# StanfordASL/pmpc

Hardware: AMD Instinct MI355X
Metric: SCP iterations/sec (M particles x N horizon) (higher is better)
Workload: dtype f64; 1 GPU; quadrotor x12 u4 M=4096 N=50 Nc=1 box-u, full SCP iteration (on-device linearise + c_lqp_solve-equivalent + residual), BASELINE config D; timed window = SCP iterations 6..2477 from the cold start X_prev = x0, U_prev = U_ref (the active-set round count falls as the SCP loop converges, so the rate depends on the window); particles_per_gpu=4096, parallelism=particle-shard x1, scp_loop=library (pmpc_scp_loop_device), ipm_warm_start=True

## Files before the change

include/pmpc_abi.h:

```cpp
#ifndef PMPC_ABI_H
#define PMPC_ABI_H

#include <stddef.h>

#ifdef __cplusplus
extern "C" {
#endif


void c_lqp_solve(double *X_out, double *U_out, size_t xdim, size_t udim, size_t N, size_t M, long long Nc,
                 double *x0, double *f, double *fx, double *fu, double *X_prev, double *U_prev, double *Q,
                 double *R, double *X_ref, double *U_ref, double *lx, double *ux, double *lu, double *uu,
                 double reg_x, double reg_u, double *slew_reg, double *slew_reg0, double *slew_um1,
                 long long verbose);

void c_lcone_solve(double *X_out, double *U_out, size_t xdim, size_t udim, size_t N, size_t M, long long Nc,
                   double *x0, double *f, double *fx, double *fu, double *X_prev, double *U_prev, double *Q,
                   double *R, double *X_ref, double *U_ref, double *lx, double *ux, double *lu, double *uu,
                   double reg_x, double reg_u, double *slew_reg, double *slew_reg0, double *slew_um1,
                   long long verbose, double smooth_alpha, char *solver);

void pmpc_lqp_solve_host(double *X_out, double *U_out, size_t xdim, size_t udim, size_t N, size_t M, long long Nc,
                         double *x0, double *f, double *fx, double *fu, double *X_prev, double *U_prev, double *Q,
                         double *R, double *X_ref, double *U_ref, double *lx, double *ux, double *lu, double *uu,
                         double reg_x, double reg_u, double *slew_reg, double *slew_reg0, double *slew_um1,
                         long long verbose, unsigned rowmajor);
void pmpc_lcone_solve_host(double *X_out, double *U_out, size_t xdim, size_t udim, size_t N, size_t M, long long Nc,
                           double *x0, double *f, double *fx, double *fu, double *X_prev, double *U_prev, double *Q,
                           double *R, double *X_ref, double *U_ref, double *lx, double *ux, double *lu, double *uu,
                           double reg_x, double reg_u, double *slew_reg, double *slew_reg0, double *slew_um1,
                           long long verbose, double smooth_alpha, unsigned rowmajor, long long cone_k);
void pmpc_lcone_solve_host_ex(double *X_out, double *U_out, size_t xdim, size_t udim, size_t N, size_t M, long long Nc, double *x0, double *f,
                              double *fx, double *fu, double *X_prev, double *U_prev, double *Q, double *R, double *X_ref, double *U_ref, double *lx,
                              double *ux, double *lu, double *uu, double reg_x, double reg_u, double *slew_reg, double *slew_reg0, double *slew_um1,
                              long long verbose, double smooth_alpha, unsigned rowmajor, long long cone_k, int smooth_cstr, double smooth_beta);


#define PMPC_HAS_XBOUNDS 1u
#define PMPC_HAS_UBOUNDS 2u
#define PMPC_HAS_SLEW 4u
#define PMPC_HAS_SLEW0 8u
#define PMPC_FORCE_GENERIC 16u
#define PMPC_SYMMETRIC_COST 32u

#define PMPC_COLD_START 64u
#define PMPC_STATIC_CONS_BOUNDS 128u
#define PMPC_PREV_IS_LAST_SOLUTION 256u

#define PMPC_CONE_OBJECTIVE 1024u
#define PMPC_F32_MATRICES 512u

typedef struct pmpc_problem {
  size_t xdim, udim, N, M;
  long long Nc;
  unsigned flags;
  double reg_x, reg_u;
  const double *x0, *f, *fx, *fu, *X_prev, *U_prev, *Q, *R, *X_ref, *U_ref;
  const double *lx, *ux, *lu, *uu;
  const double *slew_reg, *slew_reg0, *slew_um1;
  double *X_out, *U_out;
  const double *weights;
  double barrier_mu;
  size_t soc_q;
  const double *soc_W, *soc_w0, *soc_v;
  double soc_v0;
  const double *soc_u_interior;
  size_t cone_count;
  const int *cone_sizes;
  const double *cone_A, *cone_c;
  int cone_per_stage;
  long long cone_k;
  int smooth_cstr;
  double smooth_beta;
} pmpc_problem;

typedef struct pmpc_info {
  int status;
  int ipm_iters;
  int structured_solves;
  int fast_path;
  double mu;
  double slack_res;
  double max_violation;
  int outer_solves;
  int active_set_rounds;
} pmpc_info;

typedef struct pmpc_ctx pmpc_ctx;

int pmpc_create(pmpc_ctx **ctx, int device);
void pmpc_destroy(pmpc_ctx *ctx);
int pmpc_set_option(pmpc_ctx *ctx, const char *key, double value);
int pmpc_get_option(pmpc_ctx *ctx, const char *key, double *value);
void *pmpc_stream(pmpc_ctx *ctx);
void pmpc_sync(pmpc_ctx *ctx);

int pmpc_lqp_solve_device(pmpc_ctx *ctx, const pmpc_problem *prob, pmpc_info *info, int verbose);

int pmpc_lcone_solve_device(pmpc_ctx *ctx, const pmpc_problem *prob, double smooth_alpha, pmpc_info *info, int verbose);

int pmpc_lsoc_solve_device(pmpc_ctx *ctx, const pmpc_problem *prob, pmpc_info *info, int verbose);

int pmpc_particle_costs_device(pmpc_ctx *ctx, const pmpc_problem *prob, const double *X, const double *U, double *J_out);

int pmpc_comm_unique_id(void *unique_id_128);
int pmpc_comm_init(pmpc_ctx *ctx, int rank, int world, const void *unique_id_128);
int pmpc_comm_init_mock(pmpc_ctx *ctx, int rank, int world, int group);
int pmpc_comm_rank(pmpc_ctx *ctx);
int pmpc_comm_world(pmpc_ctx *ctx);

int pmpc_linearize_device(pmpc_ctx *ctx, int model, size_t N, size_t M, const double *x0, const double *X_prev,
                          const double *U_prev, const double *params, double *f, double *fx, double *fu);

int pmpc_linearize_device_f32(pmpc_ctx *ctx, int model, size_t N, size_t M, const double *x0, const double *X_prev,
                              const double *U_prev, const double *params, double *f, float *fx, float *fu);

int pmpc_rollout_device(pmpc_ctx *ctx, int model, size_t N, size_t M, const double *x0, const double *U, const double *params, double *X);

int pmpc_shift_plan_device(pmpc_ctx *ctx, int model, size_t N, size_t M, size_t s, const double *X, const double *U,
                           const double *params, const double *U_tail, double *X_new, double *U_new, double *um1_new);

int pmpc_shift_active_set_device(pmpc_ctx *ctx, size_t N, size_t M, size_t udim, long long Nc, size_t s, const double *U,
                                 const double *U_tail, const int *act, const double *lo, const double *hi, double *U_new, int *act_new);

int pmpc_warm_shift_device(pmpc_ctx *ctx, size_t N, size_t M, size_t udim, long long Nc, size_t s, const double *U, const double *U_tail,
                           const double *lo, const double *hi, double *U_new, int *shifted);

int pmpc_warm_set_read_device(pmpc_ctx *ctx, int *act_out, size_t n);

int pmpc_linearize_compact_device(pmpc_ctx *ctx, int model, size_t N, size_t M, const double *x0, const double *X_prev,
                                  const double *U_prev, const double *params, double *f, double *jc);
int pmpc_expand_jac_device(pmpc_ctx *ctx, int model, size_t N, size_t M, const double *jc, double *fx, double *fu, int orient);
long long pmpc_jac_compact_doubles(int model, size_t N, size_t M);
int pmpc_jac_live_mask(int model, unsigned char *fx_mask, unsigned char *fu_mask);

int pmpc_as_sweep_variant(int sweep, int xdim, int udim, int M, int Nc, unsigned flags, const int *knobs, int *out);

int pmpc_as_sweep_launches(int sweep, unsigned long long *out, int n, int reset);
void pmpc_as_sweep_knobs(int *out);

int pmpc_scp_residual_device(pmpc_ctx *ctx, size_t xdim, size_t udim, size_t N, size_t M, const double *X, const double *X_prev,
                             const double *U, const double *U_prev, double *out);

int pmpc_scp_loop_device(pmpc_ctx *ctx, int model, const double *params, const pmpc_problem *p, double *f2, double *fx2, double *fu2,
                         int steps, int first_cold, double *res, pmpc_info *infos, int *last_in_out);

int pmpc_ref_shift_device(pmpc_ctx *ctx, size_t dim, size_t rows, const double *A, const double *c, const double *ref, double *out);
long long pmpc_ref_shift_bad_pivots(pmpc_ctx *ctx, int reset);

typedef struct pmpc_scp_cost {
  int kind;
  int K, pos_dim;
  int pos_idx[3];
  int per_stage;
  const double *centres, *sigma, *w;
} pmpc_scp_cost;
size_t pmpc_abi_scp_cost_size(void);

int pmpc_obstacle_cost_grad_device(pmpc_ctx *ctx, const pmpc_scp_cost *cost, size_t xdim, size_t N, size_t M, const double *X_prev,
                                   double *cx);
int pmpc_obstacle_ref_shift_device(pmpc_ctx *ctx, const pmpc_scp_cost *cost, size_t xdim, size_t N, size_t M, const double *X_prev,
                                   const double *Q, const double *X_ref, double *out);

int pmpc_scp_loop_device_cost(pmpc_ctx *ctx, int model, const double *params, const pmpc_problem *p, double *f2, double *fx2,
                              double *fu2, int steps, int first_cold, double *res, pmpc_info *infos, int *last_in_out,
                              const pmpc_scp_cost *cost);

typedef struct pmpc_scp_cstr {
  int kind;
  int K, pos_dim;
  int pos_idx[3];
  long long centre_stride_particle, centre_stride_stage;
  const double *centres, *radius;
} pmpc_scp_cstr;
size_t pmpc_abi_scp_cstr_size(void);

int pmpc_keepout_augment_device(pmpc_ctx *ctx, const pmpc_scp_cstr *cstr, size_t xdim, size_t udim, size_t N, size_t M,
                                const double *X_prev, const double *f, const double *fx, const double *fu, const double *X_ref,
                                double *f_aug, double *fx_aug, double *fu_aug, double *X_prev_aug, double *X_ref_aug, double *xu_aug);

int pmpc_keepout_strip_residual_device(pmpc_ctx *ctx, size_t xdim, int K, size_t udim, size_t N, size_t M, const double *X_aug, double *X,
                                       const double *X_prev, const double *U, const double *U_prev, double *out);

typedef struct pmpc_scp_aug {
  const double *Q, *x0, *lx;
  double *f[2], *fx[2], *fu[2], *X_prev[2], *X_ref[2], *xu[2];
  double *X_out;
} pmpc_scp_aug;
size_t pmpc_abi_scp_aug_size(void);

int pmpc_scp_loop_device_cstr(pmpc_ctx *ctx, int model, const double *params, const pmpc_problem *p, double *f2, double *fx2,
                              double *fu2, int steps, int first_cold, double *res, pmpc_info *infos, int *last_in_out,
                              const pmpc_scp_cost *cost, const pmpc_scp_cstr *cstr, const pmpc_scp_aug *aug);
void pmpc_scp_loop_follow_ups(unsigned long long *out2, int reset);

void pmpc_profile_enable(pmpc_ctx *ctx, int level);
void pmpc_profile_read(pmpc_ctx *ctx, double *ms4, long long *n4);
void pmpc_profile_read_partial(pmpc_ctx *ctx, double *ms, long long *n);
void pmpc_profile_read_all(pmpc_ctx *ctx, double *ms, long long *launches, int count);

void pmpc_restart_stats(pmpc_ctx *ctx, unsigned long long *out4, int reset);

const char *pmpc_version(void);
void pmpc_abi_struct_sizes(size_t *problem, size_t *info);

#ifdef __cplusplus
}
#endif
#endif
```

pmpc_amd/_lib.py:

```python
from __future__ import annotations

import ctypes
import os
from pathlib import Path

import numpy as np

_HERE = Path(__file__).resolve().parent
LIB_PATH = Path(os.environ["PMPC_HIP_LIB"]) if os.environ.get("PMPC_HIP_LIB") else _HERE / "libpmpc_hip.so"
_lib = None

c_dp = ctypes.POINTER(ctypes.c_double)

HAS_XBOUNDS, HAS_UBOUNDS, HAS_SLEW, HAS_SLEW0, FORCE_GENERIC, SYMMETRIC_COST, COLD_START, STATIC_CONS_BOUNDS, PREV_IS_LAST_SOLUTION, F32_MATRICES, CONE_OBJECTIVE = 1, 2, 4, 8, 16, 32, 64, 128, 256, 512, 1024

ABI_SYMBOLS = [
    "c_lqp_solve", "c_lcone_solve", "pmpc_lqp_solve_host", "pmpc_lcone_solve_host", "pmpc_create", "pmpc_destroy", "pmpc_stream", "pmpc_sync", "pmpc_lqp_solve_device",
    "pmpc_comm_unique_id", "pmpc_comm_init", "pmpc_comm_rank", "pmpc_comm_world", "pmpc_linearize_device",
    "pmpc_profile_enable", "pmpc_profile_read", "pmpc_version", "pmpc_lcone_solve_device", "pmpc_particle_costs_device", "pmpc_lsoc_solve_device", "pmpc_comm_init_mock",
    "pmpc_scp_residual_device", "pmpc_profile_read_partial", "pmpc_profile_read_all", "pmpc_scp_loop_device", "pmpc_linearize_device_f32",
    "pmpc_set_option", "pmpc_get_option", "pmpc_abi_struct_sizes", "pmpc_lcone_solve_host_ex", "pmpc_restart_stats",
    "pmpc_linearize_compact_device", "pmpc_expand_jac_device", "pmpc_jac_compact_doubles", "pmpc_jac_live_mask",
    "pmpc_as_sweep_variant", "pmpc_as_sweep_launches", "pmpc_as_sweep_knobs",
    "pmpc_ref_shift_device", "pmpc_ref_shift_bad_pivots", "pmpc_obstacle_cost_grad_device", "pmpc_obstacle_ref_shift_device",
    "pmpc_scp_loop_device_cost", "pmpc_abi_scp_cost_size",
    "pmpc_rollout_device", "pmpc_shift_plan_device",
    "pmpc_keepout_augment_device", "pmpc_abi_scp_cstr_size",
    "pmpc_keepout_strip_residual_device", "pmpc_scp_loop_device_cstr", "pmpc_abi_scp_aug_size", "pmpc_scp_loop_follow_ups",
    "pmpc_shift_active_set_device", "pmpc_warm_shift_device", "pmpc_warm_set_read_device",
]


class PmpcProblem(ctypes.Structure):
    _fields_ = (
        [(k, ctypes.c_size_t) for k in ("xdim", "udim", "N", "M")]
        + [("Nc", ctypes.c_longlong), ("flags", ctypes.c_uint), ("reg_x", ctypes.c_double), ("reg_u", ctypes.c_double)]
        + [(k, ctypes.c_void_p) for k in ("x0", "f", "fx", "fu", "X_prev", "U_prev", "Q", "R", "X_ref", "U_ref",
                                          "lx", "ux", "lu", "uu", "slew_reg", "slew_reg0", "slew_um1", "X_out", "U_out", "weights")]
        + [("barrier_mu", ctypes.c_double), ("soc_q", ctypes.c_size_t), ("soc_W", ctypes.c_void_p), ("soc_w0", ctypes.c_void_p),
           ("soc_v", ctypes.c_void_p), ("soc_v0", ctypes.c_double), ("soc_u_interior", ctypes.c_void_p),
           ("cone_count", ctypes.c_size_t), ("cone_sizes", ctypes.POINTER(ctypes.c_int)), ("cone_A", ctypes.c_void_p), ("cone_c", ctypes.c_void_p),
           ("cone_per_stage", ctypes.c_int), ("cone_k", ctypes.c_longlong), ("smooth_cstr", ctypes.c_int), ("smooth_beta", ctypes.c_double)]
    )


class PmpcInfo(ctypes.Structure):
    _fields_ = [("status", ctypes.c_int), ("ipm_iters", ctypes.c_int), ("structured_solves", ctypes.c_int),
                ("fast_path", ctypes.c_int), ("mu", ctypes.c_double), ("slack_res", ctypes.c_double),
                ("max_violation", ctypes.c_double), ("outer_solves", ctypes.c_int), ("active_set_rounds", ctypes.c_int)]


class PmpcScpCost(ctypes.Structure):
    _fields_ = [("kind", ctypes.c_int), ("K", ctypes.c_int), ("pos_dim", ctypes.c_int), ("pos_idx", ctypes.c_int * 3), ("per_stage", ctypes.c_int),
                ("centres", ctypes.c_void_p), ("sigma", ctypes.c_void_p), ("w", ctypes.c_void_p)]


class PmpcScpCstr(ctypes.Structure):
    _fields_ = [("kind", ctypes.c_int), ("K", ctypes.c_int), ("pos_dim", ctypes.c_int), ("pos_idx", ctypes.c_int * 3),
                ("centre_stride_particle", ctypes.c_longlong), ("centre_stride_stage", ctypes.c_longlong),
                ("centres", ctypes.c_void_p), ("radius", ctypes.c_void_p)]


class PmpcScpAug(ctypes.Structure):
    _fields_ = ([(k, ctypes.c_void_p) for k in ("Q", "x0", "lx")] + [(k, ctypes.c_void_p * 2) for k in ("f", "fx", "fu", "X_prev", "X_ref", "xu")]
                + [("X_out", ctypes.c_void_p)])


def load():
    global _lib
    if _lib is not None:
        return _lib
    if not LIB_PATH.exists():
        raise ImportError(
            f"{LIB_PATH} is missing: build the HIP extension first (python -c 'import __graft_entry__ as g; g.build()' "
            "or make -C pmpc_amd/csrc). pmpc_amd has no CPU fallback.")
    lib = ctypes.CDLL(str(LIB_PATH), mode=ctypes.RTLD_GLOBAL)
    sz, ll, dbl, vp = ctypes.c_size_t, ctypes.c_longlong, ctypes.c_double, ctypes.c_void_p
    common = [c_dp, c_dp, sz, sz, sz, sz, ll] + [c_dp] * 14 + [dbl, dbl] + [c_dp] * 3 + [ll]
    lib.c_lqp_solve.argtypes = common
    lib.c_lqp_solve.restype = None
    lib.c_lcone_solve.argtypes = common + [dbl, ctypes.c_char_p]
    lib.c_lcone_solve.restype = None
    lib.pmpc_lqp_solve_host.argtypes = common + [ctypes.c_uint]
    lib.pmpc_lqp_solve_host.restype = None
    lib.pmpc_lcone_solve_host.argtypes = common + [dbl, ctypes.c_uint, ll]
    lib.pmpc_lcone_solve_host.restype = None
    lib.pmpc_lcone_solve_host_ex.argtypes = common + [dbl, ctypes.c_uint, ll, ctypes.c_int, dbl]
    lib.pmpc_lcone_solve_host_ex.restype = None
    lib.pmpc_create.argtypes = [ctypes.POINTER(vp), ctypes.c_int]
    lib.pmpc_create.restype = ctypes.c_int
    lib.pmpc_destroy.argtypes = [vp]
    lib.pmpc_destroy.restype = None
    lib.pmpc_set_option.argtypes = [vp, ctypes.c_char_p, ctypes.c_double]
    lib.pmpc_set_option.restype = ctypes.c_int
    lib.pmpc_get_option.argtypes = [vp, ctypes.c_char_p, c_dp]
    lib.pmpc_get_option.restype = ctypes.c_int
    lib.pmpc_stream.argtypes = [vp]
    lib.pmpc_stream.restype = vp
    lib.pmpc_sync.argtypes = [vp]
    lib.pmpc_sync.restype = None
    lib.pmpc_lqp_solve_device.argtypes = [vp, ctypes.POINTER(PmpcProblem), ctypes.POINTER(PmpcInfo), ctypes.c_int]
    lib.pmpc_lqp_solve_device.restype = ctypes.c_int
    lib.pmpc_lcone_solve_device.argtypes = [vp, ctypes.POINTER(PmpcProblem), dbl, ctypes.POINTER(PmpcInfo), ctypes.c_int]
    lib.pmpc_lcone_solve_device.restype = ctypes.c_int
    lib.pmpc_lsoc_solve_device.argtypes = [vp, ctypes.POINTER(PmpcProblem), ctypes.POINTER(PmpcInfo), ctypes.c_int]
    lib.pmpc_lsoc_solve_device.restype = ctypes.c_int
    lib.pmpc_particle_costs_device.argtypes = [vp, ctypes.POINTER(PmpcProblem), vp, vp, vp]
    lib.pmpc_particle_costs_device.restype = ctypes.c_int
    lib.pmpc_comm_unique_id.argtypes = [vp]
    lib.pmpc_comm_unique_id.restype = ctypes.c_int
    lib.pmpc_comm_init.argtypes = [vp, ctypes.c_int, ctypes.c_int, vp]
    lib.pmpc_comm_init.restype = ctypes.c_int
# ... 7 lines not shown
    lib.pmpc_linearize_device.restype = ctypes.c_int
    lib.pmpc_linearize_device_f32.argtypes = [vp, ctypes.c_int, sz, sz] + [vp] * 7
    lib.pmpc_linearize_device_f32.restype = ctypes.c_int
    if hasattr(lib, "pmpc_jac_live_mask"):
        lib.pmpc_linearize_compact_device.argtypes = [vp, ctypes.c_int, sz, sz] + [vp] * 6
        lib.pmpc_linearize_compact_device.restype = ctypes.c_int
        lib.pmpc_expand_jac_device.argtypes = [vp, ctypes.c_int, sz, sz, vp, vp, vp, ctypes.c_int]
        lib.pmpc_expand_jac_device.restype = ctypes.c_int
        lib.pmpc_jac_compact_doubles.argtypes = [ctypes.c_int, sz, sz]
        lib.pmpc_jac_compact_doubles.restype = ctypes.c_longlong
        lib.pmpc_jac_live_mask.argtypes = [ctypes.c_int, vp, vp]
        lib.pmpc_jac_live_mask.restype = ctypes.c_int
    if hasattr(lib, "pmpc_as_sweep_variant"):
        lib.pmpc_as_sweep_variant.argtypes = [ctypes.c_int] * 5 + [ctypes.c_uint, ctypes.POINTER(ctypes.c_int), ctypes.POINTER(ctypes.c_int)]
        lib.pmpc_as_sweep_variant.restype = ctypes.c_int
    if hasattr(lib, "pmpc_as_sweep_launches"):
        lib.pmpc_as_sweep_launches.argtypes = [ctypes.c_int, ctypes.POINTER(ctypes.c_ulonglong), ctypes.c_int, ctypes.c_int]
        lib.pmpc_as_sweep_launches.restype = ctypes.c_int
        lib.pmpc_as_sweep_knobs.argtypes = [ctypes.POINTER(ctypes.c_int)]
        lib.pmpc_as_sweep_knobs.restype = None
    lib.pmpc_scp_residual_device.argtypes = [vp, sz, sz, sz, sz] + [vp] * 5
    lib.pmpc_scp_residual_device.restype = ctypes.c_int
    lib.pmpc_profile_enable.argtypes = [vp, ctypes.c_int]
    lib.pmpc_profile_enable.restype = None
    lib.pmpc_profile_read.argtypes = [vp, c_dp, ctypes.POINTER(ctypes.c_longlong)]
    lib.pmpc_profile_read.restype = None
    lib.pmpc_profile_read_partial.argtypes = [vp, ctypes.POINTER(ctypes.c_double), ctypes.POINTER(ctypes.c_longlong)]
    lib.pmpc_profile_read_partial.restype = None
    lib.pmpc_restart_stats.argtypes = [vp, ctypes.POINTER(ctypes.c_ulonglong), ctypes.c_int]
    lib.pmpc_restart_stats.restype = None
    lib.pmpc_profile_read_all.argtypes = [vp, c_dp, ctypes.POINTER(ctypes.c_longlong), ctypes.c_int]
    lib.pmpc_profile_read_all.restype = None
    lib.pmpc_scp_loop_device.argtypes = [vp, ctypes.c_int, vp, ctypes.POINTER(PmpcProblem), vp, vp, vp, ctypes.c_int, ctypes.c_int, vp,
                                         ctypes.POINTER(PmpcInfo), ctypes.POINTER(ctypes.c_int)]
    lib.pmpc_scp_loop_device.restype = ctypes.c_int
    if hasattr(lib, "pmpc_scp_loop_device_cost"):
        lib.pmpc_ref_shift_device.argtypes = [vp, sz, sz, vp, vp, vp, vp]
        lib.pmpc_ref_shift_device.restype = ctypes.c_int
        lib.pmpc_ref_shift_bad_pivots.argtypes = [vp, ctypes.c_int]
        lib.pmpc_ref_shift_bad_pivots.restype = ctypes.c_longlong
        lib.pmpc_obstacle_cost_grad_device.argtypes = [vp, ctypes.POINTER(PmpcScpCost), sz, sz, sz, vp, vp]
        lib.pmpc_obstacle_cost_grad_device.restype = ctypes.c_int
        lib.pmpc_obstacle_ref_shift_device.argtypes = [vp, ctypes.POINTER(PmpcScpCost), sz, sz, sz, vp, vp, vp, vp]
        lib.pmpc_obstacle_ref_shift_device.restype = ctypes.c_int
        lib.pmpc_scp_loop_device_cost.argtypes = lib.pmpc_scp_loop_device.argtypes + [ctypes.POINTER(PmpcScpCost)]
        lib.pmpc_scp_loop_device_cost.restype = ctypes.c_int
        lib.pmpc_abi_scp_cost_size.argtypes = []
        lib.pmpc_abi_scp_cost_size.restype = sz
        if lib.pmpc_abi_scp_cost_size() != ctypes.sizeof(PmpcScpCost):
            raise ImportError(f"{LIB_PATH} and pmpc_amd/_lib.py disagree on pmpc_scp_cost: library {lib.pmpc_abi_scp_cost_size()} bytes, "
                              f"binding {ctypes.sizeof(PmpcScpCost)}: rebuild the library")
    if hasattr(lib, "pmpc_shift_plan_device"):
        lib.pmpc_rollout_device.argtypes = [vp, ctypes.c_int, sz, sz, vp, vp, vp, vp]
        lib.pmpc_rollout_device.restype = ctypes.c_int
        lib.pmpc_shift_plan_device.argtypes = [vp, ctypes.c_int, sz, sz, sz] + [vp] * 7
        lib.pmpc_shift_plan_device.restype = ctypes.c_int
    if hasattr(lib, "pmpc_keepout_augment_device"):
        lib.pmpc_keepout_augment_device.argtypes = [vp, ctypes.POINTER(PmpcScpCstr), sz, sz, sz, sz] + [vp] * 11
        lib.pmpc_keepout_augment_device.restype = ctypes.c_int
        lib.pmpc_abi_scp_cstr_size.argtypes = []
        lib.pmpc_abi_scp_cstr_size.restype = sz
        if lib.pmpc_abi_scp_cstr_size() != ctypes.sizeof(PmpcScpCstr):
            raise ImportError(f"{LIB_PATH} and pmpc_amd/_lib.py disagree on pmpc_scp_cstr: library {lib.pmpc_abi_scp_cstr_size()} bytes, "
                              f"binding {ctypes.sizeof(PmpcScpCstr)}: rebuild the library")
    if hasattr(lib, "pmpc_scp_loop_device_cstr"):
        lib.pmpc_keepout_strip_residual_device.argtypes = [vp, sz, ctypes.c_int, sz, sz, sz] + [vp] * 6
        lib.pmpc_keepout_strip_residual_device.restype = ctypes.c_int
        lib.pmpc_scp_loop_device_cstr.argtypes = lib.pmpc_scp_loop_device_cost.argtypes + [ctypes.POINTER(PmpcScpCstr), ctypes.POINTER(PmpcScpAug)]
        lib.pmpc_scp_loop_device_cstr.restype = ctypes.c_int
        lib.pmpc_scp_loop_follow_ups.argtypes = [ctypes.POINTER(ctypes.c_ulonglong), ctypes.c_int]
        lib.pmpc_scp_loop_follow_ups.restype = None
        lib.pmpc_abi_scp_aug_size.argtypes = []
        lib.pmpc_abi_scp_aug_size.restype = sz
        if lib.pmpc_abi_scp_aug_size() != ctypes.sizeof(PmpcScpAug):
            raise ImportError(f"{LIB_PATH} and pmpc_amd/_lib.py disagree on pmpc_scp_aug: library {lib.pmpc_abi_scp_aug_size()} bytes, "
                              f"binding {ctypes.sizeof(PmpcScpAug)}: rebuild the library")
    if hasattr(lib, "pmpc_warm_shift_device"):
        lib.pmpc_shift_active_set_device.argtypes = [vp, sz, sz, sz, ll, sz] + [vp] * 7
        lib.pmpc_shift_active_set_device.restype = ctypes.c_int
        lib.pmpc_warm_shift_device.argtypes = [vp, sz, sz, sz, ll, sz] + [vp] * 5 + [ctypes.POINTER(ctypes.c_int)]
        lib.pmpc_warm_shift_device.restype = ctypes.c_int
        lib.pmpc_warm_set_read_device.argtypes = [vp, vp, sz]
        lib.pmpc_warm_set_read_device.restype = ctypes.c_int
    lib.pmpc_version.argtypes = []
    lib.pmpc_version.restype = ctypes.c_char_p
    if not hasattr(lib, "pmpc_abi_struct_sizes"):
        raise ImportError(f"{LIB_PATH} predates this binding (no pmpc_abi_struct_sizes): rebuild it (make -C pmpc_amd/csrc)")
    lib.pmpc_abi_struct_sizes.argtypes = [ctypes.POINTER(sz), ctypes.POINTER(sz)]
    lib.pmpc_abi_struct_sizes.restype = None
    sp, si = sz(0), sz(0)
    lib.pmpc_abi_struct_sizes(ctypes.byref(sp), ctypes.byref(si))
    if (sp.value, si.value) != (ctypes.sizeof(PmpcProblem), ctypes.sizeof(PmpcInfo)):
        raise ImportError(f"{LIB_PATH} ({lib.pmpc_version().decode()}) and pmpc_amd/_lib.py disagree on the ABI structs: library "
                          f"{sp.value}/{si.value} bytes, binding {ctypes.sizeof(PmpcProblem)}/{ctypes.sizeof(PmpcInfo)}: rebuild the library")
    _lib = lib
    return lib


def jac_live_mask(model: int, x: int, u: int):
    lib = load()
    mx, mu = np.zeros(x * x, dtype=np.uint8), np.zeros(x * u, dtype=np.uint8)
    got = lib.pmpc_jac_live_mask(int(model), mx.ctypes.data, mu.ctypes.data)
    if got < 0:
        raise ValueError(f"model {model} is not a built-in model")
    if got != 100 * x + u:
        raise ValueError(f"model {model}: compact records are for dims {got // 100} x {got % 100}, not {x} x {u}")
    return mx.reshape(x, x).T.astype(bool), mu.reshape(u, x).T.astype(bool)


AS_SWEEP_FLAGS = ("defect", "as_settled_in", "mat32", "cone_H", "xb_D", "as_uraw", "as_T")


def as_sweep_variant(sweep: str, x: int, u: int, M: int, Nc: int, flags: int, knobs=None):
    lib = load()
    out = (ctypes.c_int * 8)()
    kn = (ctypes.c_int * 3)(*knobs) if knobs is not None else None
    got = lib.pmpc_as_sweep_variant({"bwd": 0, "fwd": 1}[sweep], x, u, M, Nc, flags, kn, out)
    if got < 0:
        raise ValueError(f"({x}, {u}) is not a compiled pair of the active-set sweeps")
    return tuple(out[:5]), bool(got), tuple(bool(v) for v in out[5:8])


def as_sweep_code(sweep: str, variant) -> int:
    a, b, c, d, e = (int(v) for v in variant)
    if sweep == "bwd":
        return a + 3 * (b + 2 * (c + 2 * (d + 3 * e)))
    return a + 2 * b + 4 * c + 8 * d + 16 * e


def as_sweep_launches(sweep: str, reset: bool = False):
    lib = load()
    sw = {"bwd": 0, "fwd": 1}[sweep]
    n = lib.pmpc_as_sweep_launches(sw, None, 0, 0)
    out = (ctypes.c_ulonglong * n)()
    lib.pmpc_as_sweep_launches(sw, out, n, int(reset))
    return [int(v) for v in out]


def scp_loop_follow_ups(reset: bool = False):
    out = (ctypes.c_ulonglong * 2)()
    load().pmpc_scp_loop_follow_ups(out, int(reset))
    return int(out[0]), int(out[1])


def as_sweep_knobs():
    out = (ctypes.c_int * 3)()
    load().pmpc_as_sweep_knobs(out)
    return tuple(out)


def dptr(a: np.ndarray):
    assert a.dtype == np.float64 and a.flags["C_CONTIGUOUS"]
    return a.ctypes.data_as(c_dp)
```

pmpc_amd/csrc/kernels_as.hip:

```cpp
#include <atomic>
#include <type_traits>

#include "fast_common.h"
#include "as_ctl_dev.h"
#include "as_variant.h"
#include "../../include/pmpc_abi.h"
#include "jac_compact.h"

#ifdef PMPC_STAGE_TIMELINE
#define PMPC_TL_STAMPS 10
__device__ unsigned long long pmpc_tl[3][128][PMPC_TL_STAMPS];
#define TL_DECL(kind) unsigned long long tl_[PMPC_TL_STAMPS] = {}; const int tl_kind = (kind); const bool tl_on = blockIdx.x == gridDim.x / 2
#define TL(k) do { __builtin_amdgcn_sched_barrier(0); tl_[k] = __builtin_amdgcn_s_memtime(); __builtin_amdgcn_sched_barrier(0); } while (0)
#define TL_FLUSH(j) do { if (tl_on && threadIdx.x == 0 && (j) < 128) { for (int k_ = 0; k_ < PMPC_TL_STAMPS; k_++) pmpc_tl[tl_kind][j][k_] = tl_[k_]; } } while (0)
#else
#define TL_DECL(kind)
#define TL(k)
#define TL_FLUSH(j)
#endif

#ifndef PMPC_AS_LEAN_WAVES
#define PMPC_AS_LEAN_WAVES 4
#endif
#ifndef PMPC_AS_DEEP_WAVES
// ... 5 lines not shown

namespace {

template <int XD, int UD, int MODE, bool SKIP, bool DEFECT, int EX = 0, class MT = double>
__global__ void __launch_bounds__(64, MODE == 2 ? 2 : (MODE == 1 ? PMPC_AS_DEEP_WAVES : PMPC_AS_LEAN_WAVES)) k_bwd_as(LQArgs a) {
  constexpr bool CONE = EX == 1, XBOX = EX == 2;
  typedef Lane<XD, UD> LT;
  constexpr int KS = LT::KS, XP = LT::XP;
  constexpr bool PADX = (XD != XP);
  constexpr long long D8 = sizeof(double);
  constexpr bool DEEP = MODE != 0, SCHOL = !DEEP;
  constexpr long long MB = sizeof(MT);
  if (a.done && *a.done) return;
  const int lane = threadIdx.x;
  const int N = a.N, Nc = a.Nc, i = a.as_perm ? __builtin_amdgcn_readfirstlane(a.as_perm[blockIdx.x]) : (int)blockIdx.x;
  if (SKIP && a.as_settled_in[i]) {
    const int nc = Nc * UD;
    if (lane < nc) {
      const double *H = a.Hc_part + (size_t)i * nc * nc;
      double acc = 0.0;
      for (int cc = 0; cc < nc; cc++) acc = fma(H[(lane < cc ? lane : cc) + nc * (lane < cc ? cc : lane)], a.as_delta[cc], acc);
      a.gc_part[(size_t)i * nc + lane] += acc;
    }
    return;
  }
  const LT L(lane);
  const int g = L.g, c = L.c;
  const size_t pbase = (size_t)i * N;
  const bool own0 = (i == 0 && a.owner);
  const bool gu = g < UD;
  const double *Z = a.zeros;
  const double pwt = a.pw ? a.pw[i] : 1.0;
  const double regx = pwt * a.reg_x, regu = pwt * a.reg_u;
  const double *Xb = DEFECT ? a.X_prev : a.Xb, *Ub = DEFECT ? a.U_prev : a.Ub;
  constexpr int CKS = 64 * KS + 32;
  int jtop = N - 1, ck_k = 0;
  if (SKIP && a.as_ck) {
    const int jh = a.as_jhi[i];
    const int lo = jh > Nc ? jh : (Nc > 1 ? Nc : 1);
    const int k = lo <= PMPC_AS_CK_FIRST ? 0 : 32 - __builtin_clz((unsigned)(lo - 1) >> PMPC_AS_CK_LOG);
    if (k < a.ck_slots) { ck_k = __builtin_amdgcn_readfirstlane(k + 1); jtop = PMPC_AS_CK_FIRST << (ck_k - 1); }
    if (lane == 0 && a.ck_stat) {
      atomicAdd(a.ck_stat + (ck_k ? 0 : 2), 1ull);
      atomicAdd(a.ck_stat + (ck_k ? 1 : 3), (unsigned long long)(jtop + 1));
    }
  }
  const double *ck_ = a.as_ck ? ubase(a.as_ck, (long long)i * a.ck_slots * (long long)(CKS * sizeof(double))) : nullptr;

  const bool fF = L.cxv || L.cu;
  const MT *pF = L.cxv ? (const MT *)a.fx + (pbase + jtop) * (XD * XD) + XD * L.oc + L.row0
                       : (L.cu ? (const MT *)a.fu + (pbase + jtop) * (XD * UD) + XD * L.cb + L.row0 : (const MT *)Z);
  int sF = fF ? -(int)MB * (L.cxv ? XD * XD : XD * UD) : 0;
  typedef typename jacc::SpecFor<XD, UD>::list JSpecs;
  if constexpr (JSpecs::COUNT > 0 && std::is_same<MT, double>::value) {
    if (a.jac_compact) {
      const jacc::LaneSel js = jacc::select(JSpecs{}, a.jac_compact, lane);
      const int m = js.bwd;
      if (m != jacc::NONE) {
        pF = m >= 0 ? (const MT *)a.fx + (pbase + jtop) * js.rec + m : (const MT *)a.fx + (size_t)a.M * N * js.rec + (size_t)i * js.pool + (-1 - m);
        sF = m >= 0 ? -(int)MB * js.rec : 0;
      }
    }
  }
  const unsigned lQ = (unsigned)((L.cxv ? XD * L.oc + L.row0 : 0) * MB);
  const double pwt_x = L.cxv ? pwt : 0.0;
  const bool fR = L.cu && gu;
  const unsigned lR = (unsigned)((fR ? g + UD * L.cb : 0) * MB), lRd = (unsigned)((fR ? g + UD * L.cb : 0) * D8);
  const unsigned lxr = (unsigned)(L.row0 * D8), lxc = (unsigned)((L.cxv ? L.oc : 0) * D8);
  const unsigned lug = (unsigned)((gu ? g : 0) * D8);
  const double regx_c = L.cxv ? regx : 0.0;
  const bool umask = L.cu && g == L.cb;
  const double umask_d = umask ? 1.0 : 0.0;
  const bool diag_x = L.cxv && ((c & 3) == g);
  bool dmask[KS];
#pragma unroll
  for (int r = 0; r < KS; r++) dmask[r] = diag_x && (c >> 2) == r;
  const long long px = (long long)(pbase * XD) * D8, pu = (long long)(pbase * UD) * D8;
  const double *Xb_ = ubase(Xb, px), *Xr_ = ubase(a.X_ref, px), *Xp_ = ubase(a.X_prev, px), *f_ = ubase(a.f, px);
  const double *kff_ = ubase(a.kff, pu);
  const void *Q_ = ubase_v(a.Q, (long long)(pbase * (XD * XD)) * MB), *R_ = ubase_v(a.R, (long long)(pbase * (UD * UD)) * MB);
  const void *K_ = ubase_v(a.K, (long long)(pbase * 64) * MB);
  auto xoff = [&](int jj) { return (long long)(jj * (int)(XD * D8)); };
  auto uoff = [&](int jj) { return (long long)(jj * (int)(UD * D8)); };
  auto ld_Q = [&](int jj, double *dst) {
    const void *q = ubase_v(Q_, (long long)(jj * (int)(XD * XD * MB)));
#pragma unroll
    for (int r = 0; r < KS; r++) {
      const bool rv = !PADX || (L.row0 + r < XD);
      const double v = ldom<MT>(q, rv ? lQ + r * (unsigned)MB : 0u);
      dst[r] = rv ? v : 0.0;
    }
  };
  auto ld_xm = [&](int jj, double *dst) {
    const double *xb = ubase(Xb_, xoff(jj)), *xr = ubase(Xr_, xoff(jj));
#pragma unroll
    for (int r = 0; r < KS; r++) {
      const bool rv = !PADX || (L.row0 + r < XD);
      const unsigned o = rv ? lxr + r * 8u : 0u;
      const double v = pwt * (ldo(xb, o) - ldo(xr, o));
      dst[r] = rv ? v : 0.0;
    }
  };
  auto ld_gx = [&](int jj) -> double {
    if (DEFECT) return 0.0;
    return regx_c * (ldo(ubase(Xb_, xoff(jj)), lxc) - ldo(ubase(Xp_, xoff(jj)), lxc));
  };
  const char *pC = (const char *)Z;
  int sC = 0;
  if (gu && c == XP) { pC = (const char *)(Ub + (pbase + jtop) * UD + g); sC = -UD * (int)D8; }
  else if (gu && c == XP + 1) { pC = (const char *)(a.U_ref + (pbase + jtop) * UD + g); sC = -UD * (int)D8; }
  else if (gu && c == XP + 2) { pC = (const char *)(a.as_act + (pbase + jtop) * UD + g); sC = -UD * (int)sizeof(int); }
  else if (CONE && gu && c == XP + 3) { pC = (const char *)(a.cone_g + (pbase + jtop) * UD + g); sC = -UD * (int)D8; }
  else if (!DEFECT && g < 2 && 15 - XP - c >= 0 && 15 - XP - c < UD) {
    pC = (const char *)((g == 0 ? Ub : a.U_prev) + (pbase + jtop) * UD + (15 - XP - c));
    sC = -UD * (int)D8;
  }
  const double regu_s = (L.cu && g < 2) ? (g == 0 ? regu : -regu) : 0.0;
  auto ld_R = [&](int jj) -> double {
    const double v = ldom<MT>(ubase_v(R_, (long long)(jj * (int)(UD * UD * MB))), lR);
    return fR ? v : 0.0;
  };
  const double *CH_ = CONE ? ubase(a.cone_H, (long long)(pbase * (UD * UD)) * D8) : Z;
  auto ld_CH = [&](int jj) -> double {
    const double v = ldo(ubase(CH_, (long long)(jj * (int)(UD * UD * D8))), lRd);
    return fR ? v : 0.0;
  };
  const bool frec = (L.cxv || L.cu) && gu;
  const unsigned lrec = (unsigned)(lane * MB);
  auto st_rec = [&](int jj, double v) {
    gstom<MT>(ubase_v(K_, (long long)(jj * (int)(64 * MB))), lrec, v);
  };

  struct PipeCone { double ch; };
  struct PipeXbox { double xd, xg; };
  struct PipeNone {};
  struct Pipe : std::conditional_t<CONE, PipeCone, std::conditional_t<XBOX, PipeXbox, PipeNone>> { double F[KS], R, ctl, f, Q[KS], xb, xr, xp; };
  const double *XD_ = XBOX ? ubase(a.xb_D, px) : Z, *XG_ = XBOX ? ubase(a.xb_g, px) : Z;
  int jF = jtop;
  auto fetch_early = [&](int jj, Pipe &q) {
    if (jj < jF) { pF = (const MT *)((const char *)pF + sF); pC += sC; jF = jj; }
#pragma unroll
    for (int r = 0; r < KS; r++) q.F[r] = (!PADX || L.row0 + r < XD || (const void *)pF == (const void *)Z) ? gldm<MT>(pF + r) : 0.0;
    q.R = ld_R(jj);
    q.ctl = gld(pC);
    if (DEFECT) q.f = ldo(ubase(f_, xoff(jj)), lxc);
    if constexpr (CONE) q.ch = ld_CH(jj);
  };
  auto fetch_late = [&](int jj, int jbelow, Pipe &q) {
    ld_Q(jbelow, q.Q);
    q.xb = ldo(ubase(Xb_, xoff(jbelow)), lxc);
    q.xr = ldo(ubase(Xr_, xoff(jbelow)), lxc);
    if (!DEFECT) q.xp = ldo(ubase(Xp_, xoff(jbelow)), lxc);
    if constexpr (XBOX) {
      q.xd = ldo(ubase(XD_, xoff(jbelow)), lxc);
      q.xg = ldo(ubase(XG_, xoff(jbelow)), lxc);
    }
  };

  double S[KS], s_row[KS], s_col;
  bool bad = false;
  TL_DECL(SKIP ? 1 : 0);
  if (SKIP && ck_k > 0) {
    const double *ck = ubase(ck_, (long long)(ck_k - 1) * (long long)(CKS * D8));
#pragma unroll
    for (int r = 0; r < KS; r++) S[r] = ldo(ck, (unsigned)((lane + 64 * r) * D8));
    const double s_ck = ldo(ck, (unsigned)(64 * KS * D8) + lxc), x_ck = ldo(ck, (unsigned)((64 * KS + 16) * D8) + lxc);
    const double dx_col = L.cxv ? ldo(ubase(Xb_, xoff(jtop)), lxc) - x_ck : 0.0;
    double dx_row[KS], part = 0.0;
    col_to_row<KS>(dx_col, g, dx_row);
#pragma unroll
    for (int r = 0; r < KS; r++) part = fma(S[r], dx_row[r], part);
    part = grp_allsum(part);
    s_col = L.cxv ? s_ck + part : 0.0;
    col_to_row<KS>(s_col, g, s_row);
  } else
  {
    double Q0[KS], xm0[KS], part = 0.0;
    ld_Q(N - 1, Q0);
    ld_xm(N - 1, xm0);
#pragma unroll
    for (int r = 0; r < KS; r++) {
      part = fma(Q0[r], xm0[r], part);
      S[r] = fma(pwt_x, Q0[r], dmask[r] ? regx : 0.0);
    }
    part = grp_allsum(part);
    if constexpr (XBOX) {
      const double d0 = ldo(ubase(XD_, xoff(N - 1)), lxc);
      part += ldo(ubase(XG_, xoff(N - 1)), lxc);
#pragma unroll
      for (int r = 0; r < KS; r++) S[r] += dmask[r] ? d0 : 0.0;
    }
    s_col = L.cxv ? part + ld_gx(N - 1) : 0.0;
    col_to_row<KS>(s_col, g, s_row);
  }
  double xb_carry = DEFECT ? ldo(ubase(Xb_, xoff(N - 1)), lxc) : 0.0;

  auto stage = [&](auto main_tag, const int j, const Pipe &cur, Pipe &nxt) {
    constexpr bool MAIN = decltype(main_tag)::value;
    TL(0);
    if (MAIN && ck_ && (j & (j - 1)) == 0 && j >= PMPC_AS_CK_FIRST) {
      const double *ck = ubase(ck_, (long long)(__builtin_ctz((unsigned)j) - PMPC_AS_CK_LOG) * (long long)(CKS * D8));
#pragma unroll
      for (int r = 0; r < KS; r++) gsto(ck, (unsigned)((lane + 64 * r) * D8), S[r]);
      const double xj = DEFECT ? xb_carry : ldo(ubase(Xb_, xoff(j)), lxc);
      if (g == 0 && L.cxv) {
        gsto(ck, (unsigned)(64 * KS * D8) + lxc, s_col);
        gsto(ck, (unsigned)((64 * KS + 16) * D8) + lxc, xj);
      }
    }
    const bool cons = MAIN ? false : j < Nc;
    const bool below = MAIN ? true : j > 0;
    double Fr[KS], Qc[KS], xm_row[KS], gx_c, Du_c;
#pragma unroll
    for (int r = 0; r < KS; r++) Fr[r] = (!MAIN && j == 0 && L.cxv) ? 0.0 : cur.F[r];
    const double Rc = cur.R;
    const double um_g = pwt * (dpp_d<0x00>(cur.ctl) - dpp_d<0x55>(cur.ctl));
    const int act_g = __builtin_amdgcn_mov_dpp(__double2loint(cur.ctl), 0xAA, 0xF, 0xF, true);
    Du_c = (umask && act_g) ? a.as_big : 0.0;
    const double gu_c0 = DEFECT ? 0.0 : regu_s * dpp_d<0x140>(cur.ctl);
    const bool cone_here = CONE && (MAIN || !cons || own0);
    double gu_c = gu_c0;
    if constexpr (CONE) gu_c = fma(dpp_d<0xFF>(cur.ctl), cone_here ? umask_d : 0.0, gu_c0);
    double Hcone = 0.0;
    if constexpr (CONE) Hcone = cone_here ? cur.ch : 0.0;
    const double df_c = (DEFECT && L.cxv) ? cur.f - xb_carry : 0.0;
    if (DEFECT) xb_carry = cur.xb;
    gx_c = DEFECT ? 0.0 : regx_c * (cur.xb - cur.xp);
    if constexpr (XBOX) gx_c += cur.xg;
    col_to_row<KS>(pwt_x * (cur.xb - cur.xr), g, xm_row);
#pragma unroll
    for (int r = 0; r < KS; r++) Qc[r] = cur.Q[r];
    auto late_pf = [&]() { if (below) fetch_late(j - 1, j >= 2 ? j - 2 : 0, nxt); };
    TL(1);
    if (MODE == 1) late_pf();
// ... 119 lines not shown
      stage(std::true_type{}, j - 2, P2, P2);
      __builtin_amdgcn_sched_barrier(0);
    }
    for (; j >= 0; j--) {
      fetch(j - 2, P2);
      if (j >= jmin) stage(std::true_type{}, j, P0, P0);
      else stage(std::false_type{}, j, P0, P0);
      P0 = P1;
      P1 = P2;
    }
  } else {
    Pipe A, B;
    fetch_early(jtop, A);
    fetch_late(jtop, jtop >= 1 ? jtop - 1 : 0, A);
    for (; j >= jmin; j--) {
      stage(std::true_type{}, j, A, B);
      A = B;
    }
    if (j >= jmin) {
      stage(std::true_type{}, j, A, B);
      A = B;
      j--;
    }
    for (; j >= 0; j--) {
      stage(std::false_type{}, j, A, B);
      A = B;
    }
  }
  if (bad && lane == 0) *a.fail = 2;
}

template <int XD, int UD, bool DEFECT, bool PF2, bool CONE = false, class MT = double, bool SENS = false>
__global__ void __launch_bounds__(64, 4) k_fwd_as(LQArgs a) {
  typedef Lane<XD, UD> LT;
  constexpr int KS = LT::KS;
  constexpr bool PADX = (XD != LT::XP);
  constexpr long long D8 = sizeof(double);
  if (a.done && *a.done) return;
  const int lane = threadIdx.x;
  const LT L(lane);
  const int N = a.N, Nc = a.Nc, i = a.as_perm ? __builtin_amdgcn_readfirstlane(a.as_perm[blockIdx.x]) : (int)blockIdx.x, g = L.g, c = L.c;
  const size_t pbase = (size_t)i * N;
  const bool gu = g < UD;
  const double *Z = a.zeros;
  constexpr int MB = (int)sizeof(MT);
  const char *pA = (const char *)Z, *pB = (const char *)Z;
  int sAr = 0, sAj = 0, sBj = 0;
  if (L.cxv) {
    pA = (const char *)((const MT *)a.fx + pbase * (XD * XD) + (size_t)XD * (KS * g) + L.oc);
    sAr = XD * MB; sAj = XD * XD * MB;
    if (gu) { pB = (const char *)((const MT *)a.fu + pbase * (XD * UD) + (size_t)XD * g + L.oc); sBj = XD * UD * MB; }
  } else if (L.cu) {
    pA = (const char *)((const MT *)a.K + pbase * 64 + 16 * L.cb + g);
    sAr = 4 * MB; sAj = 64 * MB;
  }
  typedef typename jacc::SpecFor<XD, UD>::list JSpecs;
  if constexpr (JSpecs::COUNT > 0 && std::is_same<MT, double>::value) {
    if (a.jac_compact && L.cxv) {
      const jacc::LaneSel js = jacc::select(JSpecs{}, a.jac_compact, lane);
      const double *rec = a.fx + pbase * js.rec, *pool = a.fx + (size_t)a.M * N * js.rec + (size_t)i * js.pool;
      const int mA = js.fwdA, mB = js.fwdB;
      pA = (const char *)(mA >= 0 ? rec + mA : pool + (-1 - mA));
      sAr = MB; sAj = mA >= 0 ? js.rec * MB : 0;
      if (gu) { pB = (const char *)(mB >= 0 ? rec + mB : pool + (-1 - mB)); sBj = mB >= 0 ? js.rec * MB : 0; }
    }
  }
  bool vA[KS];
#pragma unroll
  for (int r = 0; r < KS; r++) vA[r] = !L.cxv || !PADX || (KS * g + r < XD);
  const double *Xb = DEFECT ? a.X_prev : a.Xb, *Ub = DEFECT ? a.U_prev : a.Ub;
  const double pwi = a.pw ? a.pw[i] : 1.0;
  const double tol_l = (a.as_ctl ? a.as_ctl->tol_l : a.as_tol_l) * pwi;
  const unsigned lug = (unsigned)((gu ? g : 0) * D8);
  const bool own_x = c < KS && (!PADX || L.row0 + c < XD);
  const unsigned lx1 = own_x ? (unsigned)((L.row0 + c) * D8) : 0u;
  const long long px = (long long)(pbase * XD) * D8, pu = (long long)(pbase * UD) * D8;
  const double *Xb_ = ubase(Xb, px), *f_ = ubase(a.f, px), *Xo_ = ubase(a.Xo, px);
  const double *act_ = ubase((const double *)a.as_act, pu >> 1);
  const double *T_ = SENS ? ubase(a.as_T, (long long)(pbase * 64) * D8) : Z;
  const unsigned lT = (unsigned)((((c - 4) & 3) * 16 + 4 * g) * D8);
  auto xoff = [&](int jj) { return (long long)(jj * (int)(XD * D8)); };
  auto uoff = [&](int jj) { return (long long)(jj * (int)(UD * D8)); };
  const char *pG = (const char *)Z;
  int sG = 0;
  if (gu && c < 4) {
    const double *arr = c == 0 ? Ub : (c == 1 ? a.kff : (c == 2 ? a.as_lo : a.as_hi));
    pG = (const char *)(arr + pbase * UD + g);
    sG = UD * (int)D8;
  } else if (gu && c == 7) {
    pG = (const char *)(a.as_act + pbase * UD + g);
    sG = UD * (int)sizeof(int);
  }
  char *pS = (char *)((c == 1 ? a.kff : ((CONE && c == 2) ? a.as_uraw : a.Uo)) + pbase * UD + (gu ? g : 0));
  const bool st_lane = gu && c < (CONE ? 3 : 2);
  const bool store_u = (c == 0) && gu;
  struct Pipe { double T[KS + 1], grp, xb, f; };
  int jF = 0;
  auto fetch = [&](int jj, Pipe &q) {
    if (jj > jF) { pA += sAj; pB += sBj; pG += sG; jF = jj; }
#pragma unroll
    for (int r = 0; r < KS; r++) {
      const double t = gldm<MT>(pA + (vA[r] ? r * sAr : 0));
      q.T[r] = vA[r] ? t : 0.0;
    }
    q.T[KS] = gldm<MT>(pB);
    q.grp = gld(pG);
    q.xb = ldo(ubase(Xb_, xoff(jj)), lx1);
    if (DEFECT) q.f = ldo(ubase(f_, xoff(jj)), lx1);
  };

  double V[KS];
#pragma unroll
  for (int r = 0; r < KS; r++) V[r] = 0.0;
  int nrel = 0, nadd = 0, nbad = 0;
  int jh = -1;
  double vworst = 0.0;
  double dcap = 0.0;
  const bool elem = SENS && !DEFECT && a.as_settled_in && a.as_settled_in[i];
  TL_DECL(2);
  double dcons = 0.0;
  bool frozen = false;
  if (a.cons_G) {
    constexpr int nH = UD * UD, E = nH + UD;
    double a0 = 0.0, a1 = 0.0, a2 = 0.0, a3 = 0.0;
    if (lane < E) {
      const double *src = lane < nH ? a.cons_tH + lane : a.cons_tg + (lane - nH);
      const int stride = lane < nH ? nH : UD;
      int k = 0;
      for (; k + 3 < a.cons_G; k += 4) {
        a0 += src[(size_t)k * stride];
        a1 += src[(size_t)(k + 1) * stride];
        a2 += src[(size_t)(k + 2) * stride];
        a3 += src[(size_t)(k + 3) * stride];
      }
      for (; k < a.cons_G; k++) a0 += src[(size_t)k * stride];
    }
    const double acc = (a0 + a1) + (a2 + a3);
    double Lm[UD][UD], y[UD];
    bool cbad = false;
#pragma unroll
    for (int q = 0; q < UD; q++) {
      double d = readlane_d(acc, q + UD * q);
#pragma unroll
      for (int k = 0; k < q; k++) d -= Lm[q][k] * Lm[q][k];
      cbad |= !(d > 0.0);
      d = sqrt(cbad ? 1.0 : d);
      Lm[q][q] = d;
#pragma unroll
      for (int p = q + 1; p < UD; p++) {
        double v = readlane_d(acc, q + UD * p);
#pragma unroll
        for (int k = 0; k < q; k++) v -= Lm[p][k] * Lm[q][k];
        Lm[p][q] = v / d;
      }
    }
#pragma unroll
    for (int p = 0; p < UD; p++) {
      double v = -readlane_d(acc, nH + p);
#pragma unroll
      for (int k = 0; k < p; k++) v -= Lm[p][k] * y[k];
      y[p] = v / Lm[p][p];
    }
#pragma unroll
    for (int p = UD - 1; p >= 0; p--) {
      double v = y[p];
#pragma unroll
      for (int k = p + 1; k < UD; k++) v -= Lm[k][p] * y[k];
      y[p] = v / Lm[p][p];
    }
    if (CONE && a.as_freeze_tol > 0.0) {
      const int *act0 = a.as_act + pbase * UD;
      const double *ub0 = Ub + pbase * UD;
      double ym = 0.0;
      bool asks_release = false;
#pragma unroll
      for (int p = 0; p < UD; p++) {
        if (act0[p] == 0) ym = fmax(ym, fabs(y[p]) / fmax(1.0, fabs(ub0[p])));
        else asks_release |= (act0[p] == 1 ? -a.as_big * y[p] : a.as_big * y[p]) < -tol_l;
      }
      frozen = ym <= a.as_freeze_tol && !asks_release;
      if (frozen) {
#pragma unroll
// ... 56 lines not shown
    nrel += (cnt_here && release) ? 1 : 0;
    nadd += (cnt_here && (vlo || vhi)) ? 1 : 0;
    jh = (cnt_here && (release || vlo || vhi)) ? j : jh;
    {
      const double pv = (vlo ? loc - zt : (vhi ? zt - hic : 0.0)) * __builtin_amdgcn_rcp(fmax(1.0, fabs(vlo ? loc : hic)));
      const double dv = release ? -lam * inv_dual : 0.0;
      vworst = fmax(vworst, cnt_here ? fmax(pv, dv) : 0.0);
    }
    TL(3);
    const double du_q = dpp_d<0x00>(dug);
    if (SENS && !MAIN && j < Nc) dcap = dug;
    const double knew = actc ? -draw : 0.0;
    if (MAIN || j >= Nc) {
      const double k1 = dpp_d<0x00>(knew);
      const double z1 = CONE ? dpp_d<0x00>(zt) : 0.0;
      if (st_lane) gst(pS, (c == 0) ? unew : ((CONE && c == 2) ? z1 : k1));
    } else {
      const double z1 = CONE ? dpp_d<0x00>(zt) : 0.0;
      if (store_u || (CONE && gu && c == 2)) gst(pS, (c == 0) ? unew : z1);
      if (store_u && i == 0) a.as_delta[j * UD + g] = dug;
    }
    pS += UD * (int)D8;
    if (store_u) gsto_i(ubase(act_, uoff(j) >> 1), lug >> 1, anew);
    TL(4);
    D[KS] = 0.0;
    double bop = (c < 4 && gu) ? du_q : 0.0;
    if (SENS) {
      const bool sc = c >= 4 && c < 4 + UD && gu;
      const double bs = (!MAIN && j < Nc) ? ((g == c - 4) ? 1.0 : 0.0) : -raw;
      bop = sc ? bs : bop;
    }
    D = mfma(cur.T[KS], bop, D);
    if (SENS) {
      if (c >= 4 && c < 4 + UD) {
        typedef double v2dd __attribute__((ext_vector_type(2)));
        const v2dd lo2 = {D[0], KS > 1 ? D[KS > 1 ? 1 : 0] : 0.0}, hi2 = {KS > 2 ? D[KS > 2 ? 2 : 0] : 0.0, gu ? bop : 0.0};
        __attribute__((address_space(1))) char *t = (__attribute__((address_space(1))) char *)(unsigned long long)ubase(T_, (long long)(j * (int)(64 * D8))) + lT;
        *(v2dd __attribute__((address_space(1))) *)t = lo2;
        *(v2dd __attribute__((address_space(1))) *)(t + 16) = hi2;
      }
    }
    if (DEFECT) {
      const double dfo = own_x ? cur.f - cur.xb : 0.0;
      D[0] += dpp_d<0x00>(dfo);
      if (KS > 1) D[1] += dpp_d<0x55>(dfo);
      if (KS > 2) D[2] += dpp_d<0xAA>(dfo);
    }
    if (own_x) {
      double mine = D[0];
#pragma unroll
      for (int r = 1; r < KS; r++) mine = (c == r) ? D[r] : mine;
      gsto(ubase(Xo_, xoff(j)), lx1, cur.xb + mine);
    }
#pragma unroll
    for (int r = 0; r < KS; r++) V[r] = (c < (SENS ? 4 + UD : 4)) ? D[r] : 0.0;
    TL(5);
    TL_FLUSH(j);
  };

  int nrel_e = 0, nadd_e = 0, nbad_e = 0, jh_e = -1;
  auto settled_update = [&](int j0) {
    double dl[UD];
#pragma unroll
    for (int k = 0; k < UD; k++) dl[k] = readlane_d(dcap, 16 * k);
    const int s16 = lane & 15, q4 = lane >> 4, gs = s16 >> 2, rs = s16 & 3;
    const bool is_x = rs < KS && KS * gs + rs < XD, is_u = rs == 3 && gs < UD;
    const size_t xo = (size_t)(is_x ? KS * gs + rs : 0), uo = (size_t)(is_u ? gs : 0);
    constexpr int SB = 4;
    for (int j4 = j0; j4 < N; j4 += 4 * SB) {
      double dv[SB], xv[SB], ub[SB], kf[SB], lo[SB], hi[SB];
      int act[SB];
#pragma unroll
      for (int q = 0; q < SB; q++) {
        const int jj = j4 + 4 * q + q4, jc = jj < N ? jj : N - 1;
        const double *t = a.as_T + (pbase + jc) * 64 + s16;
        double acc = 0.0;
#pragma unroll
        for (int k = 0; k < UD; k++) acc = fma(gld(t + 16 * k), dl[k], acc);
        dv[q] = acc;
        xv[q] = is_x ? gld(Xb + (pbase + jc) * XD + xo) : 0.0;
        const size_t e = (pbase + jc) * UD + uo;
        ub[q] = is_u ? gld(Ub + e) : 0.0;
        kf[q] = is_u ? gld(a.kff + e) : 0.0;
        lo[q] = is_u ? gld(a.as_lo + e) : 0.0;
        hi[q] = is_u ? gld(a.as_hi + e) : 0.0;
        act[q] = is_u ? a.as_act[e] : 0;
      }
#pragma unroll
      for (int q = 0; q < SB; q++) {
        const int jj = j4 + 4 * q + q4;
        const bool live = jj < N;
        if (is_x && live) gst(a.Xo + (pbase + jj) * XD + xo, xv[q] + dv[q]);
        if (is_u && live) {
          const size_t e = (pbase + jj) * UD + uo;
          if (act[q] == 0) {
            const double zt = ub[q] + dv[q];
            const bool vlo = zt < lo[q] - a.as_tol_p * fmax(1.0, fabs(lo[q])), vhi = !vlo && zt > hi[q] + a.as_tol_p * fmax(1.0, fabs(hi[q]));
            nadd_e += (vlo || vhi) ? 1 : 0;
            nbad_e |= !(zt == zt) ? 1 : 0;
            gst(a.Uo + e, zt);
            if (CONE) gst(a.as_uraw + e, zt);
          } else {
            const double kn = kf[q] - dv[q];
            const double lam = act[q] == 1 ? a.as_big * kn : -a.as_big * kn;
            const bool release = lam < -tol_l;
            nrel_e += release ? 1 : 0;
            jh_e = (release && jj > jh_e) ? jj : jh_e;
            nbad_e |= !(kn == kn) ? 1 : 0;
            gst(a.kff + e, kn);
            if (release) a.as_act[e] = 0;
            if (a.Uo != Ub) gst(a.Uo + e, ub[q]);
            if (CONE) gst(a.as_uraw + e, ub[q] + dv[q]);
          }
        }
      }
    }
  };

  auto finish = [&]() {
    double r = grp_allsum((double)nrel), d = grp_allsum((double)nadd), b = grp_allsum((double)nbad);
    if (SENS && elem) {
      r += grp_allsum(row_allsum((double)nrel_e)); d += grp_allsum(row_allsum((double)nadd_e)); b += grp_allsum(row_allsum((double)nbad_e));
      int m = jh_e;
#pragma unroll
      for (int o = 32; o > 0; o >>= 1) { const int v = __shfl_xor(m, o, 64); m = v > m ? v : m; }
      jh = m > jh ? m : jh;
    }
    if (a.as_viol) {
      double p01, p23, q0, q1;
      swap32_d(vworst, p01, p23);
      const double m = fmax(p01, p23);
      swap16_d(m, q0, q1);
      if (lane == 0) a.as_viol[i] = fmax(q0, q1);
    }
    if (a.as_jhi) {
      int m = jh;
#pragma unroll
      for (int k = 1; k < 4; k++) { const int o = __builtin_amdgcn_readlane(jh, 16 * k); m = o > m ? o : m; }
      if (lane == 0) a.as_jhi[i] = m;
    }
    if (lane == 0) {
      a.as_cnt[3 * i + 0] = (int)r;
      a.as_cnt[3 * i + 1] = (int)d;
      a.as_cnt[3 * i + 2] = b > 0.0 ? 1 : 0;
      if (a.as_settled_out) a.as_settled_out[i] = (r == 0.0 && d == 0.0 && !(b > 0.0)) ? 1 : 0;
      if (CONE) a.as_open[i] = 0;
    }
  };

  const int jmin = Nc > 1 ? Nc : 1;
  auto clampN = [&](int jj) { return jj < N ? jj : N - 1; };
  int j = 0;
  if constexpr (SENS && !DEFECT) if (elem) {
    Pipe P;
    fetch(0, P);
    stage(std::false_type{}, 0, P);
    settled_update(1);
    finish();
    return;
  }
  if (PF2) {
    Pipe P0, P1, P2;
    fetch(0, P0);
    fetch(clampN(1), P1);
    for (; j < jmin && j < N; j++) {
      fetch(clampN(j + 2), P2);
      stage(std::false_type{}, j, P0);
      P0 = P1;
      P1 = P2;
    }
    for (; j + 2 < N; j += 3) {
      fetch(clampN(j + 2), P2);
      stage(std::true_type{}, j, P0);
      fetch(clampN(j + 3), P0);
      stage(std::true_type{}, j + 1, P1);
      fetch(clampN(j + 4), P1);
      stage(std::true_type{}, j + 2, P2);
    }
    if (j < N) { stage(std::true_type{}, j, P0); j++; }
    if (j < N) { stage(std::true_type{}, j, P1); j++; }
  } else {
    Pipe A, B;
    fetch(0, A);
    for (; j < jmin && j < N; j++) {
      fetch(clampN(j + 1), B);
      stage(std::false_type{}, j, A);
      A = B;
    }
    for (; j < N; j++) {
      fetch(clampN(j + 1), B);
      stage(std::true_type{}, j, A);
      A = B;
    }
  }
  finish();
}

__global__ void k_as_begin(AsCtl *ctl, int *fail, int max_rounds, double dual_scale, int stall_limit) {
  if (threadIdx.x == 0) {
    *fail = 0;
    AsCtl h = {};
    h.max_rounds = max_rounds;
    h.stall_limit = stall_limit;
    h.last_changes = 0x7fffffff;
    h.dual_scale = dual_scale;
    h.tol_l = dual_scale * 1e-11;
    *ctl = h;
  }
}

__global__ void __launch_bounds__(1024) k_as_ctl(AsCtl *ctl, const int *cnt_part, int M, const int *fail, int reduce, int decide, int last_of_batch,
                                                 AsCtl *mirror, unsigned long long *mirror_seq, unsigned long long seq, double *tail, const double *viol,
                                                 const int *open_part) {
  as_ctl_block(ctl, cnt_part, M, fail, reduce, decide, last_of_batch, mirror, mirror_seq, seq, tail, viol, open_part);
}

__global__ void __launch_bounds__(1024) k_as_perm(const int *settled, int M, int *perm, const int *done) {
  if (done && *done) return;
  as_perm_block(settled, M, perm);
}

template <class F>
void lift(bool v, F &&f) {
  if (v) f(std::true_type{}); else f(std::false_type{});
}
template <class F>
void lift3(int v, F &&f) {
  if (v == 0) f(std::integral_constant<int, 0>{}); else if (v == 1) f(std::integral_constant<int, 1>{}); else f(std::integral_constant<int, 2>{});
}
[[noreturn]] void no_such_variant(const char *sweep, int x, int u) {
  fprintf(stderr, "pmpc_hip: %s: the selected variant is not compiled for xdim %d, udim %d (as_variant.h)\n", sweep, x, u);
  throw PmpcHipError{-1, sweep, __FILE__, __LINE__};
}
const AsSweepKnobs &as_sweep_knobs() {
  static const AsSweepKnobs k = {getenv("PMPC_AS_DEEP2_MAXM") ? atoi(getenv("PMPC_AS_DEEP2_MAXM")) : PMPC_AS_DEEP2_MAXM,
                                 getenv("PMPC_AS_DEEP_MAXM") ? atoi(getenv("PMPC_AS_DEEP_MAXM")) : PMPC_AS_DEEP_WAVES * 1024,
                                 getenv("PMPC_AS_FWD_PF2_MAXM") ? atoi(getenv("PMPC_AS_FWD_PF2_MAXM")) : (1 << 30)};
  return k;
}
std::atomic<unsigned long long> as_bwd_launches[AS_BWD_CODES], as_fwd_launches[AS_FWD_CODES];

template <int XD, int UD>
void launch_bwd_as_t(const LQArgs &a, hipStream_t s) {
  const BwdAsVariant v = select_bwd_as(a.M, a.defect, a.as_settled_in, a.mat32, a.cone_H, a.xb_D, as_sweep_knobs());
  bool launched = false;
  lift3(v.mode, [&](auto MODE) { lift(v.skip, [&](auto SKIP) { lift(v.defect, [&](auto DEFECT) { lift3(v.ex, [&](auto EX) { lift(v.f32, [&](auto F32) {
    if constexpr (bwd_as_compiled(BwdAsVariant{MODE, SKIP, DEFECT, EX, F32}, XD, UD)) {
      hipLaunchKernelGGL((k_bwd_as<XD, UD, MODE, SKIP, DEFECT, EX, std::conditional_t<F32, float, double>>), dim3(a.M), dim3(64), 0, s, a);
      as_bwd_launches[bwd_as_code(v)].fetch_add(1, std::memory_order_relaxed);
      launched = true;
    }
  }); }); }); }); });
  if (!launched) no_such_variant("factor sweep of an active-set round", XD, UD);
}
template <int XD, int UD>
void launch_fwd_as_t(const LQArgs &a, hipStream_t s) {
  const FwdAsVariant v = select_fwd_as(a.M, a.Nc, a.defect, a.mat32, a.as_uraw, a.as_T, as_sweep_knobs());
  bool launched = false;
  lift(v.defect, [&](auto DEFECT) { lift(v.pf2, [&](auto PF2) { lift(v.cone, [&](auto CONE) { lift(v.f32, [&](auto F32) { lift(v.sens, [&](auto SENS) {
    if constexpr (fwd_as_compiled(FwdAsVariant{DEFECT, PF2, CONE, F32, SENS}, XD, UD)) {
      hipLaunchKernelGGL((k_fwd_as<XD, UD, DEFECT, PF2, CONE, std::conditional_t<F32, float, double>, SENS>), dim3(a.M), dim3(64), 0, s, a);
      as_fwd_launches[fwd_as_code(v)].fetch_add(1, std::memory_order_relaxed);
      launched = true;
    }
  }); }); }); }); });
  if (!launched) no_such_variant("forward sweep of an active-set round", XD, UD);
}

}

#ifdef PMPC_STAGE_TIMELINE
extern "C" int pmpc_debug_timeline_read(unsigned long long *out) {
  return (int)hipMemcpyFromSymbol(out, HIP_SYMBOL(pmpc_tl), sizeof(unsigned long long) * 3 * 128 * PMPC_TL_STAMPS);
}
#endif
static bool as_dims_compiled(int x, int u) {
#define X(xd, ud) if (x == xd && u == ud) return true;
  PMPC_FAST_DIMS(X)
#undef X
  return false;
}
bool f32_as_dims_supported(int x, int u) { return as_dims_compiled(x, u) && as_f32_dims(x, u); }
bool xbox_as_dims_supported(int x, int u) { return as_dims_compiled(x, u) && as_xbox_dims(x, u); }
bool cone_as_dims_supported(int x, int u) { return as_dims_compiled(x, u) && as_cone_dims(x, u); }
int pmpc_as_sweep_variant(int sweep, int xdim, int udim, int M, int Nc, unsigned flags, const int *knobs, int *out) {
  if ((sweep != 0 && sweep != 1) || !as_dims_compiled(xdim, udim) || !out) return -1;
  const AsSweepKnobs k = knobs ? AsSweepKnobs{knobs[0], knobs[1], knobs[2]} : AsSweepKnobs{PMPC_AS_DEEP2_MAXM, PMPC_AS_DEEP_WAVES * 1024, 1 << 30};
  const bool defect = flags & 1, settled_in = flags & 2, mat32 = flags & 4, cone_H = flags & 8, xb_D = flags & 16, as_uraw = flags & 32, as_T = flags & 64;
  out[5] = f32_as_dims_supported(xdim, udim); out[6] = cone_as_dims_supported(xdim, udim); out[7] = xbox_as_dims_supported(xdim, udim);
  if (sweep == 0) {
    const BwdAsVariant v = select_bwd_as(M, defect, settled_in, mat32, cone_H, xb_D, k);
    out[0] = v.mode; out[1] = v.skip; out[2] = v.defect; out[3] = v.ex; out[4] = v.f32;
    return bwd_as_compiled(v, xdim, udim);
  }
  const FwdAsVariant v = select_fwd_as(M, Nc, defect, mat32, as_uraw, as_T, k);
  out[0] = v.defect; out[1] = v.pf2; out[2] = v.cone; out[3] = v.f32; out[4] = v.sens;
  return fwd_as_compiled(v, xdim, udim);
}
int pmpc_as_sweep_launches(int sweep, unsigned long long *out, int n, int reset) {
  if (sweep != 0 && sweep != 1) return -1;
  std::atomic<unsigned long long> *t = sweep == 0 ? as_bwd_launches : as_fwd_launches;
  const int codes = sweep == 0 ? AS_BWD_CODES : AS_FWD_CODES;
  for (int c = 0; c < codes; c++) {
    const unsigned long long v = reset ? t[c].exchange(0, std::memory_order_relaxed) : t[c].load(std::memory_order_relaxed);
    if (out && c < n) out[c] = v;
  }
  return codes;
}
void pmpc_as_sweep_knobs(int *out) {
  const AsSweepKnobs &k = as_sweep_knobs();
  out[0] = k.deep2_maxm; out[1] = k.deep_maxm; out[2] = k.fwd_pf2_maxm;
}
void launch_bwd_as(const LQArgs &a, hipStream_t s) {
#define X(xd, ud) if (a.x == xd && a.u == ud) { launch_bwd_as_t<xd, ud>(a, s); return; }
  PMPC_FAST_DIMS(X)
#undef X
  no_such_variant("factor sweep of an active-set round", a.x, a.u);
}
void launch_fwd_as(const LQArgs &a, hipStream_t s) {
#define X(xd, ud) if (a.x == xd && a.u == ud) { launch_fwd_as_t<xd, ud>(a, s); return; }
  PMPC_FAST_DIMS(X)
#undef X
  no_such_variant("forward sweep of an active-set round", a.x, a.u);
}
void launch_as_ctl(AsCtl *ctl, const int *cnt_part, int M, const int *fail, int reduce, int decide, int last_of_batch, AsCtl *mirror,
                   unsigned long long *mirror_seq, unsigned long long seq, hipStream_t s, double *tail, const double *viol, const int *open_part) {
  hipLaunchKernelGGL(k_as_ctl, dim3(1), dim3(1024), 0, s, ctl, cnt_part, M, fail, reduce, decide, last_of_batch, mirror, mirror_seq, seq, tail, viol,
                     open_part);
}
void launch_as_perm(const int *settled, int M, int *perm, const int *done, hipStream_t s) {
  hipLaunchKernelGGL(k_as_perm, dim3(1), dim3(1024), 0, s, settled, M, perm, done);
}
void launch_as_begin(AsCtl *ctl, int *fail, int max_rounds, double dual_scale, hipStream_t s, int stall_limit) {
  hipLaunchKernelGGL(k_as_begin, dim3(1), dim3(64), 0, s, ctl, fail, max_rounds, dual_scale, stall_limit);
}
```

pmpc_amd/csrc/pmpc_dev.h:

```cpp
#pragma once
#include <hip/hip_runtime.h>
#include <cstdint>
#include <cstdio>
#include <cstdlib>

struct PmpcHipError {
  int code;
  const char *what, *file;
  int line;
};
#define HIP_CHECK(expr)                                                                       \
  do {                                                                                        \
    hipError_t _e = (expr);                                                                   \
    if (_e != hipSuccess) {                                                                   \
      fprintf(stderr, "pmpc_hip: HIP error %s at %s:%d (%s)\n", hipGetErrorString(_e), __FILE__, \
              __LINE__, #expr);                                                               \
      throw PmpcHipError{(int)_e, #expr, __FILE__, __LINE__};                                 \
    }                                                                                         \
  } while (0)
#define HIP_WARN(expr)                                                                        \
  do {                                                                                        \
    hipError_t _e = (expr);                                                                   \
    if (_e != hipSuccess)                                                                     \
      fprintf(stderr, "pmpc_hip: HIP error %s at %s:%d (%s)\n", hipGetErrorString(_e), __FILE__, __LINE__, #expr); \
  } while (0)

struct AsCtl {
  int done;
  int status;
  int round;
  int max_rounds, last_changes, stalls;
  int stall_limit;
  int open;
  int cnt[4];
  int hist[16][2];
  double tol_l;
  double dual_scale;
  double worst[16];
};

#ifndef PMPC_AS_CK_LOG
#define PMPC_AS_CK_LOG 2
#endif
#define PMPC_AS_CK_FIRST (1 << PMPC_AS_CK_LOG)

struct LQArgs {
  int x, u, N, M, Nc;
  int w;
  int n;
  double reg_x, reg_u;
  const double *pw;
  const double *cons_w;
  const double *f, *fx, *fu, *Q, *R, *X_prev, *U_prev, *X_ref, *U_ref;
  const double *slew, *slew0, *um1;
  const double *X, *U;
  const double *Dx, *Du, *wx, *wu;
  int du_full;
  double *xm, *xd, *um, *ud;
  const double *zeros;
  double *K;
  double *Hinv;
  double *kff;
  double *gc_part;
  double *Hc_part;
  int cost_lds;
  double *Hc_grp;
  double *scratch;
  const double *duc;
  double *dX, *dU;
  int *as_act;
  const double *as_lo, *as_hi;
  int *as_cnt;
  double *as_viol;
  const double *defect;
  const int *as_settled_in;
  int *as_settled_out;
  const int *as_perm;
  double *as_ck;
  int *as_jhi;
  int ck_slots;
  unsigned long long *ck_stat;
  double as_big, as_tol_p, as_tol_l;
  double as_freeze_tol;
  const double *Xb, *Ub;
  double *Xo, *Uo;
  double *as_delta;
  const AsCtl *as_ctl;
  const int *done;
  int as_merge;
  const double *cons_tH, *cons_tg;
  int cons_G;
  const double *cone_H, *cone_g;
  double *as_uraw;
  int *as_open;
  double *as_T;
  const double *xb_D, *xb_g;
  int mat32;
  int jac_compact;
  int owner;
  int any_slew;
  int sym_cost;
  int *fail;
};

struct Slab {
  long long count;
  int d, N, Nc;
  int is_u;
  int owner;
  const double *lo, *hi;
  double *z, *dz;
  const double *dz2;
  double *tl, *tu, *ll, *lu, *cl, *cu, *D, *w;
};

struct SlabEx {
  Slab s;
  int bounded;
  const double *ref, *prev;
  double *gm, *gd;
  double reg;
  const double *pw;
  long long per;
};

struct IpmScal {
  double comp_sum;
  double cnt;
  double muaff_sum;
  double pad0;
  double res_max;
  double viol_max;
  unsigned long long amin_bits;
  unsigned long long pad1;
  double mu, sigma, sigmu, alpha_aff, alpha, nu;
  int iter, status;
  double mu_target;
  double dev_max;
  double *part_dev;
};

#define PMPC_RED_BLOCKS 1024

size_t lq_generic_lds_bytes(const LQArgs &a);
void launch_rollout(const LQArgs &a, const double *U, double *X, hipStream_t s);
void launch_bwd_generic(const LQArgs &a, bool factor, hipStream_t s);
void launch_fwd_generic(const LQArgs &a, hipStream_t s);
void launch_reduce_particles_hg(const double *Hc_part, const double *gc_part, double *tmp, double *Hg, int M, int nc, hipStream_t s, int MH = -1);
void launch_reduce_particles(const double *src, double *tmp, double *dst, int M, int E, hipStream_t s);
struct AsCtlCall {
  AsCtl *ctl;
  const int *cnt_part;
  int M;
  const int *fail;
  AsCtl *mirror;
  unsigned long long *mirror_seq;
  unsigned long long seq;
  const double *viol;
  const int *open_part;
  const int *settled;
  int *perm;
};
int launch_cons_partials(const double *Hc_part, const double *gc_part, int M, int nc, double *tmp, const AsCtlCall &pend,
                         hipStream_t s);
void launch_cons_small(const double *Hc_part, const double *gc_part, int M, int nc, bool with_H, double *Hg, double *tmp, bool solve_now,
                       double *Lc, double *duc, int *fail, hipStream_t s);
void launch_cons_solve(double *Hc, double *Lc, const double *gc, double *duc, int nc, bool factor, int *fail,
                       hipStream_t s);
void launch_epi_check(const double *lam, const double *J, const double *user, int M, double cap, double *out, hipStream_t s, double *mirror = nullptr,
                      unsigned long long *mirror_seq = nullptr, unsigned long long seq = 0);
void launch_cons_scale(const double *Hc_part, const double *gc_part, const double *w, int M, int nc, bool with_H, double *outH, double *outg,
                       const int *as_act, double as_big, const double *Du, const double *wu, int u, int owner, hipStream_t s);

bool lq_fast_supported(const LQArgs &a);
void launch_bwd_fast(const LQArgs &a, bool factor, hipStream_t s);
void launch_fwd_fast(const LQArgs &a, hipStream_t s);
int cond_fast_groups(int M);
void launch_cond_fast(const LQArgs &a, hipStream_t s);
void launch_rollout_fast(const LQArgs &a, const double *U, double *X, hipStream_t s);
void launch_grad_prep(const LQArgs &a, hipStream_t s);
void launch_as_publish(int *counters, const int *fail, int *mirror_cnt, unsigned long long *mirror_seq, unsigned long long seq, hipStream_t s);
void launch_particle_cost(const LQArgs &a, const double *X, const double *U, double *J, hipStream_t s);

void launch_bwd_as(const LQArgs &a, hipStream_t s);
void launch_fwd_as(const LQArgs &a, hipStream_t s);
void launch_as_perm(const int *settled, int M, int *perm, const int *done, hipStream_t s);
void launch_as_begin(AsCtl *ctl, int *fail, int max_rounds, double dual_scale, hipStream_t s, int stall_limit = 2);
void launch_as_ctl(AsCtl *ctl, const int *cnt_part, int M, const int *fail, int reduce, int decide, int last_of_batch, AsCtl *mirror,
                   unsigned long long *mirror_seq, unsigned long long seq, hipStream_t s, double *tail = nullptr, const double *viol = nullptr,
                   const int *open_part = nullptr);

struct ConeArgs {
  int M, N, u, q, Nc, owner;
  const double *U, *Uraw;
  const double *A, *c;
  int ncones, qs[4], rows, per_stage;
  const double *R;
  int r32;
  double reg_u, rho_scale;
  double *z, *rec;
  double *H, *g;
  int *cnt, *settled, *open;
  int *jhi;
  const int *done;
  const AsCtl *ctl;
  int finish;
  double tol_step, tol_phi, dual_scale;
};
#define PMPC_CONE_REC 12
bool cone_as_supported(int u, int q);
bool cone_as_dims_supported(int x, int u);
void launch_cone_step(const ConeArgs &a, hipStream_t s);
void launch_cone_drop_redundant_lo(double *lo, const double *A, const double *c, int q, long long rows, int u, hipStream_t s);

struct XboxArgs {
  int M, N, x;
  const double *X;
  const double *lo, *hi;
  const double *Q, *pw;
  double reg_x, rho_scale;
  double *qmax;
  double *z;
  int *st;
  double *D, *g;
  int *cnt, *settled, *open;
  int *jhi;
  const int *done;
  const AsCtl *ctl;
  int finish;
  double tol, dual_scale;
  double z_tol;
  int keep_on_clamp;
  double act_frac;
  int ctrl_from;
};
bool xbox_as_dims_supported(int x, int u);
void launch_xbox_step(const XboxArgs &a, hipStream_t s);
void launch_xbox_from_ipm(const struct Slab &sx, int *st, double *z, hipStream_t s);

void launch_block_transpose(const double *in, double *out, int rows, int cols, long long n, hipStream_t s);
void launch_host_checks(const double *lx, const double *ux, long long nx, const double *lu, const double *uu, long long nu,
                        const double *Q, long long nq, int x, const double *R, long long nr, int u, int *flags, hipStream_t s);
void launch_axpy(double *y, const double *xv, double alpha, long long n, hipStream_t s);
void launch_fill(double *y, double v, long long n, hipStream_t s);
void launch_cons_bounds(double *lo, double *hi, int M, int N, int u, int Nc, hipStream_t s);
void launch_init_base(double *U, const double *U_prev, int M, int N, int u, int Nc, hipStream_t s);
void launch_violation(const Slab &sl, double *part_max, hipStream_t s);
void launch_violation_sum(const Slab &sl, const double *za, const double *zb, double *part_max, hipStream_t s);
void launch_ipm_clip(const Slab &sl, hipStream_t s);
void launch_as_setup(const Slab &sl, int from_ipm, int keep_base, int *act, double *ztry, double big, hipStream_t s);
void launch_as_check(const Slab &sl, int *act, const double *ztry, double big, double tol_p, double tol_l, int *counters,
                     unsigned long long *worst_bits, hipStream_t s);
void launch_as_accept_all(const Slab &sl, const int *act, const double *ztry, double *Uout, const double *xtry, const double *dx,
                          long long nx, double *Xws, double *Xout, hipStream_t s);
void launch_ipm_init_slack(const Slab &sl, double mu0, hipStream_t s, double thr_frac = 1e-2);
void launch_ipm_prepare(const Slab &sl, int corrector, const IpmScal *sc, double *part_sum, double *part_cnt,
                        double *part_max, hipStream_t s);
void launch_ipm_step(const Slab &sl, int corrector, IpmScal *sc, double *part_s1, double *part_s2, hipStream_t s);
void launch_ipm_advance(const SlabEx &X, const SlabEx &U, int do_update, const IpmScal *sc, double *part_sum, double *part_cnt,
                        double *part_max, hipStream_t s);
void launch_ipm_exchange(int phase, bool pack, bool unpack, IpmScal *sc, const int *fail, double *xch, int rank, int world,
                         const double *part_sum, const double *part_cnt, const double *part_max, int nblocks, hipStream_t s,
                         double mu_target = 0.0, double *part_dev = nullptr,
                         IpmScal *mirror = nullptr, unsigned long long *mirror_seq = nullptr, unsigned long long seq = 0);

struct SocArgs {
  int M, N, u, Nc, q, owner;
  const double *U, *dU, *dU2;
  int corr;
  double *cl, *cu, *cc;
  const double *lo, *hi;
  const double *W, *w0, *v;
  double v0, mu, sigmu;
// ... 56 lines not shown
```

pmpc_amd/csrc/solver.hip:

```cpp
#include <dlfcn.h>

#include "solver_internal.h"
#include "cost_lin.h"
#include "keepout.h"
#include <atomic>

namespace {

struct Rccl {
  void *h = nullptr;
  ncclResult_t (*GetUniqueId)(ncclUniqueId *) = nullptr;
  ncclResult_t (*CommInitRank)(ncclComm_t *, int, ncclUniqueId, int) = nullptr;
  ncclResult_t (*CommDestroy)(ncclComm_t) = nullptr;
  ncclResult_t (*AllReduce)(const void *, void *, size_t, ncclDataType_t, ncclRedOp_t, ncclComm_t, hipStream_t) = nullptr;
  ncclResult_t (*Broadcast)(const void *, void *, size_t, ncclDataType_t, int, ncclComm_t, hipStream_t) = nullptr;
  bool load() {
    if (h) return true;
    const char *names[] = {"librccl.so", "librccl.so.1", "/opt/rocm/lib/librccl.so"};
    for (const char *n : names)
      if ((h = dlopen(n, RTLD_NOW | RTLD_GLOBAL))) break;
    if (!h) return false;
    GetUniqueId = (decltype(GetUniqueId))dlsym(h, "ncclGetUniqueId");
    CommInitRank = (decltype(CommInitRank))dlsym(h, "ncclCommInitRank");
    CommDestroy = (decltype(CommDestroy))dlsym(h, "ncclCommDestroy");
// ... 129 lines not shown
  IpmScal *sc = (IpmScal *)w.sc.p;
  const int B2 = 2 * PMPC_RED_BLOCKS;
  c->seq++;
  if (!c->multi()) {
    launch_ipm_exchange(phase, true, true, sc, (const int *)w.fail.p, w.xch.d(), 0, 1, w.part_sum.d(), w.part_cnt.d(),
                        w.part_max.d(), B2, c->stream, 0.0, nullptr, &c->mirror_dev->sc, &c->mirror_dev->seq, c->seq);
    return;
  }
  launch_ipm_exchange(phase, true, false, sc, (const int *)w.fail.p, w.xch.d(), c->rank, c->world, w.part_sum.d(),
                      w.part_cnt.d(), w.part_max.d(), B2, c->stream);
  allreduce(c, w.xch.p, (size_t)c->world * 8, ncclFloat64, ncclSum);
  launch_ipm_exchange(phase, false, true, sc, (const int *)w.fail.p, w.xch.d(), c->rank, c->world, w.part_sum.d(),
                      w.part_cnt.d(), w.part_max.d(), B2, c->stream, 0.0, nullptr, &c->mirror_dev->sc, &c->mirror_dev->seq, c->seq);
}

void structured_solve(pmpc_ctx *c, LQArgs &a, bool factor, bool fast, bool prep_done) {
  hipStream_t s = c->stream;
  Workspace &w = c->ws;
  const int nc = a.Nc * a.u;
  if (fast && factor && !prep_done) launch_grad_prep(a, s);
  {
    ProfScope ps(c, factor ? ((fast && a.as_settled_in) ? 4 : 0) : 1);
    if (fast && a.as_act) launch_bwd_as(a, s);
    else if (fast) launch_bwd_fast(a, factor, s);
    else launch_bwd_generic(a, factor, s);
  }
  if (nc > 0) {
    ProfScope ps(c, 3);
    double *Hc = w.Hg.d(), *gc = w.Hg.d() + (size_t)nc * nc;
    const bool grouped = fast && factor && a.Nc > 1 && nc * nc + nc > 32 && !a.as_act && !a.as_settled_in && !a.cons_w && c->opt[OPT_COND_GROUPED] != 0.0;
    a.Hc_grp = nullptr;
    if (grouped) {
      w.Hc_grp.ensure((size_t)cond_fast_groups(a.M) * nc * nc * sizeof(double));
      a.Hc_grp = w.Hc_grp.d();
    }
    if (fast && factor) launch_cond_fast(a, s);
    const size_t tail = (a.as_merge && factor) ? 5 : 0;
    double *tl = Hc + (size_t)nc * nc + nc;
    auto merged_exchange = [&]() {
      if (a.as_merge == 2) launch_as_ctl(const_cast<AsCtl *>(a.as_ctl), a.as_cnt, a.M, (const int *)w.fail.p, 1, 0, 0, nullptr, nullptr, 0, s, tl, nullptr, a.as_open);
      else if (a.as_merge == 1) HIP_CHECK(hipMemsetAsync(tl, 0, 5 * sizeof(double), s));
      if (factor) allreduce(c, Hc, (size_t)nc * nc + nc + tail, ncclFloat64, ncclSum);
      else allreduce(c, gc, nc, ncclFloat64, ncclSum);
      if (a.as_merge == 2)
        launch_as_ctl(const_cast<AsCtl *>(a.as_ctl), nullptr, a.M, (const int *)w.fail.p, 0, 1, 0, &c->mirror_dev->ctl, &c->mirror_dev->as_seq, c->as_seq, s, tl);
    };
    const bool wave_solve = c->opt[OPT_AS_WAVE_CONS] != 0.0;
    a.cons_G = 0;
    const double *HcP = a.Hc_part, *gcP = a.gc_part;
    if (a.cons_w) {
      w.Hc_w.ensure((size_t)a.M * nc * nc * sizeof(double)); w.gc_w.ensure((size_t)a.M * nc * sizeof(double));
      launch_cons_scale(a.Hc_part, a.gc_part, a.cons_w, a.M, nc, factor, w.Hc_w.d(), w.gc_w.d(), a.as_act, a.as_big, a.as_act ? nullptr : a.Du,
                        a.as_act ? nullptr : a.wu, a.u, a.owner, s);
      HcP = factor ? w.Hc_w.d() : a.Hc_part; gcP = w.gc_w.d();
    }
    if (fast && a.as_act && factor && !c->multi() && a.Nc == 1 && wave_solve) {
      a.cons_G = launch_cons_partials(HcP, gcP, a.M, nc, w.red_tmp.d(), c->as_pend, s);
      c->as_pend.ctl = nullptr;
      a.cons_tH = w.red_tmp.d();
      a.cons_tg = w.red_tmp.d() + (size_t)64 * nc * nc;
    } else if (nc * nc + nc <= 32) {
      const bool solve_now = !c->multi();
      launch_cons_small(HcP, gcP, a.M, nc, factor, Hc, w.red_tmp.d(), solve_now, w.Lc.d(), w.duc.d(), (int *)w.fail.p, s);
      if (!solve_now) {
        merged_exchange();
        if (fast && a.as_act && factor && a.Nc == 1 && wave_solve) {
          a.cons_G = 1; a.cons_tH = Hc; a.cons_tg = gc;
        } else {
          launch_cons_solve(Hc, w.Lc.d(), gc, w.duc.d(), nc, factor, (int *)w.fail.p, s);
        }
      }
    } else {
      if (factor && grouped) launch_reduce_particles_hg(a.Hc_grp, gcP, w.red_tmp.d(), Hc, a.M, nc, s, cond_fast_groups(a.M));
      else if (factor) launch_reduce_particles_hg(HcP, gcP, w.red_tmp.d(), Hc, a.M, nc, s);
      else launch_reduce_particles(gcP, w.red_tmp.d(), gc, a.M, nc, s);
      merged_exchange();
      launch_cons_solve(Hc, w.Lc.d(), gc, w.duc.d(), nc, factor, (int *)w.fail.p, s);
    }
  }
  ProfScope ps(c, 2);
  if (fast && a.as_act) launch_fwd_as(a, s);
  else if (fast) launch_fwd_fast(a, s);
  else launch_fwd_generic(a, s);
}

int fail_after_error(pmpc_ctx *c, const pmpc_problem *p, pmpc_info *info) {
  Workspace &w = c->ws;
  w.as_key = w.warm_key = w.soc_key = w.cons_key = w.xb_block_key = w.su_key = -1;
  w.as_U_valid = false;
  w.xb_warm_backoff = w.xb_warm_fails = 0;
  c->cone_rw_key = -1;
  c->xb_ctrl_from = -1;
  c->as_pend.ctl = nullptr;
  c->staged.clear();
  (void)hipGetLastError();
  try {
    if (p && p->X_out && p->U_out) {
      const double nan = std::numeric_limits<double>::quiet_NaN();
      launch_fill(p->X_out, nan, (long long)p->M * p->N * p->xdim, c->stream);
      launch_fill(p->U_out, nan, (long long)p->M * p->N * p->udim, c->stream);
    }
    HIP_WARN(hipStreamSynchronize(c->stream));
  } catch (...) {
  }
  if (info) {
    memset(info, 0, sizeof(*info));
    info->status = 2;
  }
  return 2;
}

void fill_nan_outputs(pmpc_ctx *c, const pmpc_problem *p) {
  const double nan = std::numeric_limits<double>::quiet_NaN();
  launch_fill(p->X_out, nan, (long long)p->M * p->N * p->xdim, c->stream);
  launch_fill(p->U_out, nan, (long long)p->M * p->N * p->udim, c->stream);
  HIP_CHECK(hipStreamSynchronize(c->stream));
}

}

extern "C" {

const char *pmpc_version(void) { return "pmpc_hip 0.4 (gfx950)"; }
void pmpc_abi_struct_sizes(size_t *problem, size_t *info) { *problem = sizeof(pmpc_problem); *info = sizeof(pmpc_info); }
size_t pmpc_abi_scp_cost_size(void) { return sizeof(pmpc_scp_cost); }

int pmpc_create(pmpc_ctx **out, int device) {
  int ndev = 0;
  if (hipGetDeviceCount(&ndev) != hipSuccess || ndev <= device) {
    fprintf(stderr, "pmpc_hip: no HIP device %d available (found %d) — this library has no CPU path\n", device, ndev);
    return 1;
  }
  pmpc_ctx *c = new pmpc_ctx();
  c->device = device;
  for (int k = 0; k < OPT_COUNT; k++) {
    const char *e = getenv(kPmpcOptions[k].env);
    c->opt[k] = (e && *e) ? atof(e) : kPmpcOptions[k].dflt;
  }
  try {
    HIP_CHECK(hipSetDevice(device));
    HIP_CHECK(hipStreamCreateWithFlags(&c->stream, hipStreamNonBlocking));
    c->sc_host = (IpmScal *)calloc(1, sizeof(IpmScal));
    c->fail_host = (int *)calloc(1, sizeof(int));
    HIP_CHECK(hipHostMalloc((void **)&c->mirror, sizeof(pmpc_ctx::ScMirror), hipHostMallocMapped | hipHostMallocCoherent));
    memset(c->mirror, 0, sizeof(pmpc_ctx::ScMirror));
    HIP_CHECK(hipHostGetDevicePointer((void **)&c->mirror_dev, c->mirror, 0));
  } catch (const PmpcHipError &) {
    free(c->sc_host);
    free(c->fail_host);
    delete c;
    return 1;
  }
  *out = c;
  return 0;
}

int pmpc_set_option(pmpc_ctx *c, const char *key, double value) {
  if (!c || !key) return -1;
  for (int k = 0; k < OPT_COUNT; k++)
    if (!strcmp(key, kPmpcOptions[k].key)) {
      c->opt[k] = value;
      c->fp_key = -1;
      c->ws.as_key = c->ws.warm_key = c->cone_rw_key = c->cone_lam_key = c->ws.es_key = -1;
      return 0;
    }
  return -1;
// ... 332 lines not shown
static int solve_impl(pmpc_ctx *c, const pmpc_problem *p, pmpc_info *info, int verbose, bool soc) {
  try {
    int st = solve_impl_body(c, p, info, verbose, soc);
    if (st == PMPC_NEEDS_F64) {
      const pmpc_problem q = widened_f32_problem(c, p);
      if (verbose) printf("pmpc_hip: fp32-storage problem: widened for the fp64 kernels\n");
      st = solve_impl_body(c, &q, info, verbose, soc);
    }
    HIP_CHECK(hipGetLastError());
    return st;
  } catch (const PmpcHipError &) {
    return fail_after_error(c, p, info);
  }
}

int pmpc_lqp_solve_device(pmpc_ctx *c, const pmpc_problem *p, pmpc_info *info, int verbose) {
  return solve_impl(c, p, info, verbose, false);
}
int pmpc_lsoc_solve_device(pmpc_ctx *c, const pmpc_problem *p, pmpc_info *info, int verbose) {
  return solve_impl(c, p, info, verbose, true);
}

bool slew_increment_form_applies(const pmpc_ctx *c, const pmpc_problem *p, bool soc) {
  if (soc || !(p->flags & (PMPC_HAS_SLEW | PMPC_HAS_SLEW0)) || (p->flags & PMPC_FORCE_GENERIC) || !(p->flags & PMPC_SYMMETRIC_COST))
    return false;
  if (p->N < 2) return false;
  const bool with_boxes = c->opt[OPT_SLEW_INCREMENT_BOXES] != 0.0 && c->opt[OPT_XBOX_AS] != 0.0;
  if ((p->flags & (PMPC_HAS_XBOUNDS | PMPC_HAS_UBOUNDS)) && !(with_boxes && xbox_as_dims_supported((int)(p->xdim + p->udim), (int)p->udim))) return false;
  if ((p->flags & (PMPC_HAS_XBOUNDS | PMPC_HAS_UBOUNDS)) && p->barrier_mu > 0.0) return false;
  LQArgs t;
  memset(&t, 0, sizeof(t));
  t.x = (int)(p->xdim + p->udim); t.u = (int)p->udim; t.N = (int)p->N; t.M = (int)p->M; t.sym_cost = 1;
  return lq_fast_supported(t);
}

void build_slew_increment_problem(pmpc_ctx *c, const pmpc_problem *p, pmpc_problem &q, SlewAug &g) {
  HIP_CHECK(hipSetDevice(c->device));
  hipStream_t s = c->stream;
  Workspace &w = c->ws;
  const int x = (int)p->xdim, u = (int)p->udim, N = (int)p->N, M = (int)p->M, n = x + u;
  const int Nc = p->Nc < 0 ? N : (int)p->Nc;
  const bool has_xb = p->flags & PMPC_HAS_XBOUNDS, has_ub = p->flags & PMPC_HAS_UBOUNDS;
  const bool has_slew = p->flags & PMPC_HAS_SLEW, has_slew0 = p->flags & PMPC_HAS_SLEW0;
  const size_t rows = (size_t)M * N, D8 = sizeof(double);
  w.sa_f.ensure(rows * n * D8); w.sa_fx.ensure(rows * n * n * D8); w.sa_fu.ensure(rows * n * u * D8);
  w.sa_Xp.ensure(rows * n * D8); w.sa_Up.ensure(rows * u * D8); w.sa_Q.ensure(rows * n * n * D8); w.sa_R.ensure(rows * u * u * D8);
  w.sa_Xr.ensure(rows * n * D8); w.sa_Ur.ensure(rows * u * D8); w.sa_Xo.ensure(rows * n * D8); w.sa_Uo.ensure(rows * u * D8);
  const bool boxes = has_xb || has_ub;
  if (boxes) { w.sa_lo.ensure(rows * n * D8); w.sa_hi.ensure(rows * n * D8); }
  if (w.zslew.bytes < (size_t)M * D8 || w.zum1.bytes < (size_t)M * u * D8) {
    w.zslew.ensure((size_t)M * D8); w.zslew0.ensure((size_t)M * D8); w.zum1.ensure((size_t)M * u * D8);
    HIP_CHECK(hipMemsetAsync(w.zslew.p, 0, (size_t)M * D8, s));
    HIP_CHECK(hipMemsetAsync(w.zslew0.p, 0, (size_t)M * D8, s));
    HIP_CHECK(hipMemsetAsync(w.zum1.p, 0, (size_t)M * u * D8, s));
  }
  memset(&g, 0, sizeof(g));
  g.x = x; g.u = u; g.N = N; g.M = M; g.Nc = Nc; g.has_xb = has_xb; g.has_ub = has_ub;
  g.has_um1 = (has_slew0 && Nc >= 1) ? 1 : 0;
  const double reg = std::min(p->reg_x, p->reg_u);
  g.dx = p->reg_x - reg; g.du = p->reg_u - reg;
  g.f = p->f; g.fx = p->fx; g.fu = p->fu; g.Xp = p->X_prev; g.Up = p->U_prev; g.Q = p->Q; g.R = p->R; g.Xr = p->X_ref; g.Ur = p->U_ref;
  g.lx = p->lx; g.ux = p->ux; g.lu = p->lu; g.uu = p->uu;
  g.slew = has_slew ? p->slew_reg : w.zslew.d();
  g.slew0 = has_slew0 ? p->slew_reg0 : w.zslew0.d();
  g.um1 = has_slew0 ? p->slew_um1 : w.zum1.d();
  if (has_ub && Nc > 0) {
    const size_t nc = (size_t)Nc * u;
    w.sa_cl.ensure(nc * D8); w.sa_ch.ensure(nc * D8);
    HIP_CHECK(hipMemcpyAsync(w.sa_cl.p, p->lu, nc * D8, hipMemcpyDeviceToDevice, s));
    HIP_CHECK(hipMemcpyAsync(w.sa_ch.p, p->uu, nc * D8, hipMemcpyDeviceToDevice, s));
    if (c->multi()) {
      broadcast(c, w.sa_cl.p, nc, ncclFloat64, 0);
      broadcast(c, w.sa_ch.p, nc, ncclFloat64, 0);
    }
    g.cons_lo = w.sa_cl.d(); g.cons_hi = w.sa_ch.d();
  }
  g.af = w.sa_f.d(); g.afx = w.sa_fx.d(); g.afu = w.sa_fu.d(); g.aXp = w.sa_Xp.d(); g.aUp = w.sa_Up.d();
  g.aQ = w.sa_Q.d(); g.aR = w.sa_R.d(); g.aXr = w.sa_Xr.d(); g.aUr = w.sa_Ur.d();
  g.alo = boxes ? w.sa_lo.d() : nullptr; g.ahi = boxes ? w.sa_hi.d() : nullptr;
  launch_slew_augment(g, s);

  q = *p;
  q.xdim = (size_t)n;
  q.flags &= ~(PMPC_HAS_SLEW | PMPC_HAS_SLEW0 | PMPC_HAS_UBOUNDS | PMPC_HAS_XBOUNDS | PMPC_PREV_IS_LAST_SOLUTION | PMPC_STATIC_CONS_BOUNDS);
  if (boxes) q.flags |= PMPC_HAS_XBOUNDS;
  q.reg_x = reg;
  q.reg_u = 0.0;
  q.f = g.af; q.fx = g.afx; q.fu = g.afu; q.X_prev = g.aXp; q.U_prev = g.aUp; q.Q = g.aQ; q.R = g.aR; q.X_ref = g.aXr; q.U_ref = g.aUr;
  q.lx = g.alo; q.ux = g.ahi; q.lu = q.uu = nullptr;
  q.slew_reg = q.slew_reg0 = q.slew_um1 = nullptr;
  q.X_out = w.sa_Xo.d(); q.U_out = w.sa_Uo.d();
}

int solve_slew_increment_form(pmpc_ctx *c, const pmpc_problem *p, pmpc_info *info, int verbose) {
  hipStream_t s = c->stream;
  Workspace &w = c->ws;
  const int x = (int)p->xdim, u = (int)p->udim, N = (int)p->N, M = (int)p->M;
  const int Nc = p->Nc < 0 ? N : (int)p->Nc;
  const size_t rows = (size_t)M * N;
  pmpc_problem q;
  SlewAug g;
  build_slew_increment_problem(c, p, q, g);
  pmpc_info inf;
  memset(&inf, 0, sizeof(inf));
  c->xb_ctrl_from = x;
  int st;
  try {
    st = solve_impl_body(c, &q, &inf, verbose, false);
  } catch (...) {
    c->xb_ctrl_from = -1;
    throw;
  }
  c->xb_ctrl_from = -1;
  if (st == 0) launch_slew_split(w.sa_Xo.d(), w.sa_Uo.d(), p->X_out, p->U_out, (long long)rows, x, u, N, (M > 1 || c->multi()) ? Nc : 0, g.cons_lo, g.cons_hi, s);
  else fill_nan_outputs(c, p);
  if (info) *info = inf;
  return st;
}


static std::atomic<unsigned long long> g_follow_ups[2];
void pmpc_scp_loop_follow_ups(unsigned long long *out2, int reset) {
  for (int k = 0; k < 2; k++) {
    if (out2) out2[k] = g_follow_ups[k].load();
    if (reset) g_follow_ups[k].store(0);
  }
}
size_t pmpc_abi_scp_aug_size(void) { return sizeof(pmpc_scp_aug); }

int pmpc_scp_loop_device(pmpc_ctx *c, int model, const double *params, const pmpc_problem *p0, double *f2, double *fx2, double *fu2,
                         int steps, int first_cold, double *res, pmpc_info *infos, int *last_in_out) {
  return pmpc_scp_loop_device_cstr(c, model, params, p0, f2, fx2, fu2, steps, first_cold, res, infos, last_in_out, nullptr, nullptr, nullptr);
}
int pmpc_scp_loop_device_cost(pmpc_ctx *c, int model, const double *params, const pmpc_problem *p0, double *f2, double *fx2, double *fu2,
                              int steps, int first_cold, double *res, pmpc_info *infos, int *last_in_out, const pmpc_scp_cost *cost) {
  return pmpc_scp_loop_device_cstr(c, model, params, p0, f2, fx2, fu2, steps, first_cold, res, infos, last_in_out, cost, nullptr, nullptr);
}
static bool scp_aug_complete(const pmpc_scp_aug *g) {
  if (!g || !g->Q || !g->x0 || !g->lx || !g->X_out) return false;
  for (int k = 0; k < 2; k++)
    if (!g->f[k] || !g->fx[k] || !g->fu[k] || !g->X_prev[k] || !g->X_ref[k] || !g->xu[k]) return false;
  return true;
}
int pmpc_scp_loop_device_cstr(pmpc_ctx *c, int model, const double *params, const pmpc_problem *p0, double *f2, double *fx2, double *fu2,
                              int steps, int first_cold, double *res, pmpc_info *infos, int *last_in_out, const pmpc_scp_cost *cost,
                              const pmpc_scp_cstr *cstr, const pmpc_scp_aug *aug) {
  pmpc_problem p = *p0;
  const int x = (int)p0->xdim, u = (int)p0->udim, N = (int)p0->N, M = (int)p0->M;
  const bool with_cost = cost != nullptr && cost->kind != 0;
  double *Xr[2] = {nullptr, nullptr};
  unsigned *cost_bad = nullptr;
  auto shift = [&](int set, const double *X) {
    if (!with_cost) return;
    launch_obstacle_ref_shift(*cost, x, N, M, X, p0->Q, p0->X_ref, Xr[set], cost_bad, c->stream);
  };
  double *XA = const_cast<double *>(p0->X_prev), *UA = const_cast<double *>(p0->U_prev), *XB = p0->X_out, *UB = p0->U_out;
  double *F[2][3] = {{const_cast<double *>(p0->f), const_cast<double *>(p0->fx), const_cast<double *>(p0->fu)}, {f2, fx2, fu2}};
  const bool with_cstr = cstr != nullptr && cstr->kind != 0;
  const int K = with_cstr ? cstr->K : 0;
  auto augment = [&](int set, const double *X) {
    if (!with_cstr) return;
    launch_keepout_augment(*cstr, x, u, N, M, X, F[set][0], F[set][1], F[set][2], with_cost ? Xr[set] : p0->X_ref, aug->f[set], aug->fx[set], aug->fu[set], aug->X_prev[set],
                           aug->X_ref[set], aug->xu[set], c->stream);
  };
  const bool soc = p0->soc_u_interior != nullptr || p0->cone_count > 0;
  const bool cone_obj = (p0->flags & PMPC_CONE_OBJECTIVE) != 0;
  const int jac32 = (p0->flags & PMPC_F32_MATRICES) ? 1 : 0;
  static const bool lin_compact_env = !(getenv("PMPC_LIN_COMPACT") && atoi(getenv("PMPC_LIN_COMPACT")) == 0);
  const bool compact_ok = lin_compact_env && !with_cstr && !cone_obj && !jac32 && !c->multi() && p0->Nc >= 0 && p0->Nc <= 1 &&
                          jac_compact_dims(model, x, u) && (p0->flags & PMPC_SYMMETRIC_COST) &&
                          !(p0->flags & (PMPC_HAS_SLEW | PMPC_HAS_SLEW0 | PMPC_FORCE_GENERIC | PMPC_COLD_START)) &&
                          ((p0->flags & PMPC_HAS_UBOUNDS) || soc) && !(p0->barrier_mu > 0.0) && c->opt[OPT_AS_DEFECT] != 0.0 &&
                          c->opt[OPT_AS_WARM] != 0.0 && c->opt[OPT_POLISH_MU] > 0.0;
  bool compact_set[2] = {false, false};
  int done = 0, cur = 0;
  const bool cstr_refused = with_cstr && (!keepout_cstr_valid(cstr, x) || !keepout_strip_dims_valid(p0->xdim, K, p0->udim) || !scp_aug_complete(aug) || soc ||
                                          (p0->flags & (PMPC_HAS_SLEW | PMPC_HAS_SLEW0)) || jac32 || c->multi() || p0->smooth_cstr == 1);
  if (!model_known(model) || (with_cost && (jac32 || !obstacle_cost_valid(cost, x))) || cstr_refused) {
    if (infos && steps > 0) { memset(&infos[0], 0, sizeof(pmpc_info)); infos[0].status = 2; }
    if (last_in_out) *last_in_out = 0;
    return 0;
  }
  bool lin_ready = false;
  try {
    HIP_CHECK(hipSetDevice(c->device));
    HIP_CHECK(hipMemsetAsync(res, 0, (size_t)steps * sizeof(double), c->stream));
    if (with_cost) {
      for (DevBuf &b : c->ws.cost_ref) b.ensure((size_t)p0->M * p0->N * p0->xdim * sizeof(double));
      Xr[0] = c->ws.cost_ref[0].d(); Xr[1] = c->ws.cost_ref[1].d();
      cost_bad = cost_bad_counter(c);
    }
    for (; done < steps; done++) {
      double *Xp = (done & 1) ? XB : XA, *Up = (done & 1) ? UB : UA, *Xo = (done & 1) ? XA : XB, *Uo = (done & 1) ? UA : UB;
      if (!lin_ready) {
        ProfScope ps(c, 6);
        compact_set[cur] = compact_ok && (done > 0 || !first_cold);
        if (compact_set[cur])
          launch_linearize_compact(model, N, M, p0->x0, Xp, Up, params, F[cur][0], F[cur][1], nullptr, nullptr, nullptr, nullptr, 0, 0, nullptr, c->stream);
        else
          launch_linearize(model, N, M, p0->x0, Xp, Up, params, F[cur][0], F[cur][1], F[cur][2], c->stream, jac32);
        shift(cur, Xp);
        augment(cur, Xp);
      }
      p.f = F[cur][0]; p.fx = F[cur][1]; p.fu = F[cur][2];
      if (with_cost) p.X_ref = Xr[cur];
      c->jac_compact_fx = compact_set[cur] ? F[cur][1] : nullptr;
      c->jac_compact_model = model;
      p.X_prev = Xp; p.U_prev = Up; p.X_out = Xo; p.U_out = Uo;
      p.flags = p0->flags | PMPC_STATIC_CONS_BOUNDS;
      if (done > 0 || !first_cold) p.flags |= PMPC_PREV_IS_LAST_SOLUTION;
      else p.flags &= ~(unsigned)PMPC_PREV_IS_LAST_SOLUTION;
      if (with_cstr) {
        p.xdim = (size_t)(x + K);
        p.f = aug->f[cur]; p.fx = aug->fx[cur]; p.fu = aug->fu[cur]; p.X_prev = aug->X_prev[cur];
        p.X_ref = (with_cost || p0->X_ref) ? aug->X_ref[cur] : nullptr;
        p.Q = aug->Q; p.x0 = aug->x0; p.lx = aug->lx; p.ux = aug->xu[cur]; p.X_out = aug->X_out;
        p.flags = (p.flags | PMPC_HAS_XBOUNDS) & ~(unsigned)PMPC_PREV_IS_LAST_SOLUTION;
      }
      bool res_dirty = false;
      auto follow_up = [&, Xp, Up, Xo, Uo](bool with_next_lin) {
        const bool next = with_next_lin && done + 1 < steps;
        if (with_cstr) {
          {
            ProfScope ps(c, 7);
            launch_keepout_strip_residual(aug->X_out, Xo, Xp, Uo, Up, (long long)M * (long long)N, x, K, u, res + done, c->stream, res_dirty);
            res_dirty = true;
          }
          if (next) {
            ProfScope ps(c, 6);
            compact_set[cur ^ 1] = false;
            launch_linearize(model, N, M, p0->x0, Xo, Uo, params, F[cur ^ 1][0], F[cur ^ 1][1], F[cur ^ 1][2], c->stream, jac32);
            shift(cur ^ 1, Xo);
            augment(cur ^ 1, Xo);
          }
          return;
        }
        if (next && !res_dirty && !c->multi()) {
          ProfScope ps(c, 6);
          compact_set[cur ^ 1] = compact_ok;
          if (compact_ok)
            launch_linearize_compact(model, N, M, p0->x0, Xo, Uo, params, F[cur ^ 1][0], F[cur ^ 1][1], Xo, Xp, Uo, Up, x, u, res + done, c->stream);
          else
            launch_linearize_with_residual(model, N, M, p0->x0, Xo, Uo, params, F[cur ^ 1][0], F[cur ^ 1][1], F[cur ^ 1][2], Xo, Xp, Uo, Up, x, u,
                                           res + done, c->stream, jac32);
          shift(cur ^ 1, Xo);
          res_dirty = true;
          return;
        }
        {
          ProfScope ps(c, 7);
          launch_scp_residual(Xo, Xp, Uo, Up, (long long)M * (long long)N, x, u, res + done, c->stream, res_dirty);
          res_dirty = true;
        }
        if (c->multi()) allreduce(c, res + done, 1, ncclFloat64, ncclMax);
        if (next) {
          ProfScope ps(c, 6);
          compact_set[cur ^ 1] = compact_ok;
          if (compact_ok)
            launch_linearize_compact(model, N, M, p0->x0, Xo, Uo, params, F[cur ^ 1][0], F[cur ^ 1][1], nullptr, nullptr, nullptr, nullptr, 0, 0, nullptr, c->stream);
          else
            launch_linearize(model, N, M, p0->x0, Xo, Uo, params, F[cur ^ 1][0], F[cur ^ 1][1], F[cur ^ 1][2], c->stream, jac32);
          shift(cur ^ 1, Xo);
        }
      };
      c->spec_fired = c->spec_ok = false;
      c->post_batch = [&]() { follow_up(true); };
      pmpc_info inf;
      const int st = cone_obj ? lcone_body(c, &p, p.barrier_mu > 0.0 ? 1.0 / p.barrier_mu : std::numeric_limits<double>::quiet_NaN(), &inf, 0)
                              : solve_impl(c, &p, &inf, 0, soc);
      c->post_batch = nullptr;
      c->jac_compact_fx = nullptr;
      if (infos) infos[done] = inf;
      if (st != 0) {
        if (with_cstr) launch_fill(Xo, std::numeric_limits<double>::quiet_NaN(), (long long)M * N * x, c->stream);
        break;
      }
      if (c->spec_fired && c->spec_ok) {
        lin_ready = true;
        g_follow_ups[0]++;
      } else {
        follow_up(false);
        lin_ready = false;
        g_follow_ups[1]++;
      }
      cur ^= 1;
    }
    HIP_CHECK(hipGetLastError());
  } catch (const PmpcHipError &) {
    c->post_batch = nullptr;
    c->jac_compact_fx = nullptr;
    if (infos && done < steps) { memset(&infos[done], 0, sizeof(pmpc_info)); infos[done].status = 2; }
    fail_after_error(c, nullptr, nullptr);
    try {
      const double nan = std::numeric_limits<double>::quiet_NaN();
      const long long ex = (long long)M * N * x, eu = (long long)M * N * u;
      for (double *b : {XA, XB}) if (b) launch_fill(b, nan, ex, c->stream);
      for (double *b : {UA, UB}) if (b) launch_fill(b, nan, eu, c->stream);
      if (with_cstr) launch_fill(aug->X_out, nan, (long long)M * N * (x + K), c->stream);
      HIP_WARN(hipStreamSynchronize(c->stream));
    } catch (...) {
    }
  }
  if (last_in_out) *last_in_out = done & 1;
  return done;
}

}
```

pmpc_amd/csrc/solver_internal.h:

```cpp
#pragma once
#include <dlfcn.h>
#include <rccl/rccl.h>

#include <algorithm>
#include <chrono>
#include <cmath>
#include <condition_variable>
#include <cstring>
#include <functional>
#include <map>
#include <atomic>
#include <mutex>
#include <thread>
#include <limits>
#include <vector>

#include "../../include/pmpc_abi.h"
#include "pmpc_dev.h"

namespace pmpc_impl {

struct DevBuf {
  void *p = nullptr;
  size_t bytes = 0;
// ... 23 lines not shown
  DevBuf Hc_w, gc_w, cons_w, epi_lam, epi_out, epi_gath;
  DevBuf Hc_grp;
  DevBuf es_Dx, es_wx, es_Du, es_wu, es_xm, es_xd, es_um, es_ud, es_kff2, es_kff3, es_gc2, es_dots, es_coef, es_out2, es_Xt, es_Ut, es_U, es_zero;
  long long es_key = -1;
  DevBuf xch, zeros, zslew, zslew0, zum1, part_sum, part_cnt, part_max, sc, fail;
  DevBuf pw, Jc, Jg;
  DevBuf soc_zl, soc_zu, soc_zc, soc_dzl, soc_dzu, soc_dzc, soc_sl, soc_su, soc_sc, soc_dsl, soc_dsu, soc_dsc;
  DevBuf soc_cl, soc_cu, soc_cc;
  DevBuf soc_wU, soc_wzl, soc_wzu, soc_wzc;
  long long soc_key = -1;
  DevBuf Hadd, wu_soc;
  DevBuf cone_A, cone_c, cone_z, cone_rec, cone_uraw, as_open;
  DevBuf xb_qmax;
  DevBuf xb_z, xb_st, xb_D, xb_g;
  DevBuf jac_tmp;
  DevBuf cost_ref[2];
  DevBuf cost_bad;
  DevBuf m64[4];
  DevBuf warmU, warm_llu, warm_luu, warm_llx, warm_lux;
  DevBuf lateX, lateU;
  long long warm_key = -1;
  double warm_mu = 0.0;
  DevBuf as_perm;
  int as_perm_m = -1;
  DevBuf as_T;
  DevBuf as_ck, as_jhi, ck_stat;
  DevBuf as_act, as_cnt, as_cntp, as_settled, as_ctl, as_delta, as_viol;
  long long su_key = -1;
  const double *su_src_lo = nullptr, *su_src_hi = nullptr;
  bool as_U_valid = false;
  int as_pred_rounds = 3;
  DevBuf cons_lo, cons_hi;
  long long cons_key = -1;
  long long xb_block_key = -1;
  int xb_warm_backoff = 0, xb_warm_fails = 0;
  long long as_key = -1;
  double as_scale = 1.0;
  size_t as_count = 0;
  DevBuf as_act2;
  DevBuf part_dev;
  DevBuf sa_f, sa_fx, sa_fu, sa_Xp, sa_Up, sa_Q, sa_R, sa_Xr, sa_Ur, sa_lo, sa_hi, sa_Xo, sa_Uo, sa_cl, sa_ch;
  SlabBufs sx, su;
};


enum PmpcOpt {
  OPT_AS_WARM, OPT_AS_SKIP, OPT_AS_DEFECT, OPT_AS_COLD_ROUNDS, OPT_POLISH_MU, OPT_WARM_START, OPT_CONE_AS, OPT_CONE_COLD_ROUNDS, OPT_XBOX_AS,
  OPT_SLEW_INCREMENT_BOXES, OPT_AS_FUSE_CTL, OPT_AS_WAVE_CONS, OPT_HOST_REUSE, OPT_WARN_SLOW_PATH, OPT_CONE_RANK_MEMORY, OPT_CONE_EPIGRAPH, OPT_COND_GROUPED, OPT_AS_FREEZE_TOL, OPT_AS_CKPT, OPT_AS_SENS_MIN_M, OPT_AS_PERM_MIN_M, OPT_CONE_PATH, OPT_COUNT
};
}
using namespace pmpc_impl;

struct ProfCat {
  std::vector<std::pair<hipEvent_t, hipEvent_t>> pending, pool;
  double ms = 0.0;
  long long n = 0;
};

struct pmpc_ctx {
  double opt[OPT_COUNT];
  bool warned_slow_path = false;
  std::vector<double> cone_rw;
  long long cone_rw_key = -1;
  long long fp_key = -1;
  int fp_ok = -1;
  std::vector<double> cone_lam;
  long long cone_lam_key = -1;
  double cone_rho = 0.0;
  std::vector<double> cons_w_host, epi_lam_host;
  const double *cons_w_active = nullptr;
  int xb_ctrl_from = -1;
  AsCtlCall as_pend{};
  int prof = 0;
  double partial_ms = 0.0;
  long long partial_n = 0;
  double last_ms[8] = {0};
  long long last_n[8] = {0};
  ProfCat cat[8];
  int device = 0;
  hipStream_t stream = nullptr;
  Workspace ws;
  IpmScal *sc_host = nullptr;
  int *fail_host = nullptr;
  struct ScMirror { IpmScal sc; unsigned long long seq; int as_cnt[4]; unsigned long long as_seq; AsCtl ctl; double epi[4]; unsigned long long epi_seq; };
  ScMirror *mirror = nullptr, *mirror_dev = nullptr;
  unsigned long long seq = 0, as_seq = 0, epi_seq = 0;
  ncclComm_t comm = nullptr;
  bool mock_comm = false;
  int rank = 0, world = 1;
  bool single_rank_comm = false;
  bool multi() const { return world > 1 || single_rank_comm; }
  DevBuf stage[19], stage_t[4];
  void *pinned = nullptr;
  void *sm_pinned = nullptr;
  size_t sm_pinned_bytes = 0;
  size_t pinned_bytes = 0;
  struct StagedChunk { void *dst; size_t bytes, off; };
  std::vector<StagedChunk> staged;
  DevBuf host_flags;
  std::function<void()> post_batch;
  bool spec_fired = false, spec_ok = false;
  const double *jac_compact_fx = nullptr;
  int jac_compact_model = 0;
};

namespace pmpc_impl {

void allreduce(pmpc_ctx *c, void *buf, size_t n, ncclDataType_t dt, ncclRedOp_t op);
void broadcast(pmpc_ctx *c, void *buf, size_t n, ncclDataType_t dt, int root);

struct ProfScope {
  pmpc_ctx *c;
  int k;
  std::pair<hipEvent_t, hipEvent_t> ev;
  bool on;
  ProfScope(pmpc_ctx *c_, int k_) : c(c_), k(k_), on(c_->prof >= 2 || (c_->prof == 1 && k_ == 0)) {
    if (!on) return;
    ProfCat &pc = c->cat[k];
    if (pc.pool.empty()) {
      HIP_CHECK(hipEventCreate(&ev.first));
      HIP_CHECK(hipEventCreate(&ev.second));
    } else {
      ev = pc.pool.back();
      pc.pool.pop_back();
    }
    HIP_CHECK(hipEventRecord(ev.first, c->stream));
  }
  ~ProfScope() {
    if (!on) return;
    HIP_WARN(hipEventRecord(ev.second, c->stream));
    c->cat[k].pending.push_back(ev);
  }
};

template <class Pred>
bool spin_until(Pred ready, double limit_s = 2.0) {
  const auto t0 = std::chrono::steady_clock::now();
  for (;;) {
    for (int k = 0; k < 1024; k++) {
      if (ready()) return true;
      __builtin_ia32_pause();
    }
    if (std::chrono::duration<double>(std::chrono::steady_clock::now() - t0).count() > limit_s) return ready();
  }
}
void wait_published(pmpc_ctx *c, volatile unsigned long long *seq, unsigned long long want);
void read_scalars(pmpc_ctx *c);
void exchange(pmpc_ctx *c, int phase);
void structured_solve(pmpc_ctx *c, LQArgs &a, bool factor, bool fast, bool prep_done = false);
int fail_after_error(pmpc_ctx *c, const pmpc_problem *p, pmpc_info *info);
void fill_nan_outputs(pmpc_ctx *c, const pmpc_problem *p);

}

constexpr int PMPC_NEEDS_F64 = -7;

extern "C" {
pmpc_problem widened_f32_problem(pmpc_ctx *c, const pmpc_problem *p, bool jacobians = true);
void build_slew_increment_problem(pmpc_ctx *c, const pmpc_problem *p, pmpc_problem &q, SlewAug &g);
int lcone_body(pmpc_ctx *c, const pmpc_problem *p, double smooth_alpha, pmpc_info *info, int verbose);
int solve_impl_body(pmpc_ctx *c, const pmpc_problem *p, pmpc_info *info, int verbose, bool soc);
bool slew_increment_form_applies(const pmpc_ctx *c, const pmpc_problem *p, bool soc);
int solve_slew_increment_form(pmpc_ctx *c, const pmpc_problem *p, pmpc_info *info, int verbose);
}
```

pmpc_amd/csrc/solver_qp.hip:

```cpp
#include "solver_internal.h"

namespace {

constexpr int GO_ON = -1000;

struct AsAttempt {
  double dual_scale;
  int mode, max_rounds;
  LQArgs b;
  ConeArgs ca;
  XboxArgs xa;
  int *act;
  AsCtl *ctl;
  bool cone, xbox;
  bool refused;
  bool use_defect;
  AsCtl h;
  int round;
  int n_batches_at_hook;
};

class QpSolve {
 public:
  QpSolve(pmpc_ctx *c_, const pmpc_problem *p_, pmpc_info *info_, int verbose_, bool soc_)
// ... 461 lines not shown
    if (read_step(amax)) { status = 2; break; }
    const double alpha = std::min(1.0, 0.99 * amax);
    if (!(alpha > 0.0)) { status = 2; break; }
    launch_soc_update(sa, alpha, w.X.d(), w.dX.d(), w.dX2.d(), w.U.d(), (long long)nx, (long long)nu, (long long)ncz, s);
    newton++;
    sa.corr = 0; sa.sigmu = 0.0;
    nblk = launch_soc_prepare(sa, 1, w.part_sum.d(), w.part_cnt.d(), s);
    double mu_new;
    fl = measure(nblk, mu_new);
    if (fl) {
      status = (mu <= 1e2 * mu_tol) ? 0 : (fl == 3 ? 3 : 2);
      break;
    }
    if (verbose) printf("pmpc_hip: soc it %3d  mu %9.3e -> %9.3e  alpha_aff %6.4f  sigma %8.2e  alpha %6.4f\n", newton, mu, mu_new, a_aff, sigma, alpha);
    const bool stalled = alpha < 1e-3 && mu <= 1e2 * mu_tol;
    mu = mu_new;
    if (!remembered && !soc_warm_off && mu <= 0.5) {
      for (DevBuf *b : {&w.soc_wU, &w.soc_wzl, &w.soc_wzu}) b->ensure(nu * D8);
      w.soc_wzc.ensure(ncz * D8);
      HIP_CHECK(hipMemcpyAsync(w.soc_wU.p, w.U.p, nu * D8, hipMemcpyDeviceToDevice, s));
      HIP_CHECK(hipMemcpyAsync(w.soc_wzl.p, sa.zl, nu * D8, hipMemcpyDeviceToDevice, s));
      HIP_CHECK(hipMemcpyAsync(w.soc_wzu.p, sa.zu, nu * D8, hipMemcpyDeviceToDevice, s));
      HIP_CHECK(hipMemcpyAsync(w.soc_wzc.p, sa.zc, ncz * D8, hipMemcpyDeviceToDevice, s));
      w.soc_key = skey;
      remembered = true;
    }
    if (mu <= mu_tol || stalled) { status = 0; break; }
  }
  if (status != 0 && warm) {
    if (verbose) printf("pmpc_hip: stage cones: warm-started run failed (status %d), cold start\n", status);
    warm = false; remembered = false; status = 1; newton = 0;
    w.soc_key = -1;
    HIP_CHECK(hipMemsetAsync(w.fail.p, 0, sizeof(int), s));
    goto soc_restart;
  }
  inf.ipm_iters = newton;
  inf.mu = mu;
  if (verbose) printf("pmpc_hip: stage cones: status %d after %d Newton steps\n", status, newton);
  return (finish_now || status != 0) ? finish(status) : 0;
}

int QpSolve::equality_phase() {
  reset_scalars();
  equality_solve();
  if (has_xb) launch_violation(sx, w.part_max.d(), s);
  if (has_ub) launch_violation(su, w.part_max.d() + B, s);
  exchange(c, 1);
  read_scalars(c);
  inf.max_violation = c->sc_host->viol_max;
  if (*c->fail_host || !(c->sc_host->viol_max == c->sc_host->viol_max)) return 2;
  if (verbose) printf("pmpc_hip: equality-only optimum, max bound violation %.3e\n", c->sc_host->viol_max);
  if (!has_xb && !has_ub) return 0;
  if (c->sc_host->viol_max <= 0.0 && mu_target == 0.0) return 0;
  return 1;
}

int QpSolve::active_set_fast(double dual_scale, int mode, int max_rounds, int xb) {
  if (!(mode == 0 && as_defect_on && (p->flags & PMPC_PREV_IS_LAST_SOLUTION) && Nc <= 1)) densify();
  AsAttempt t = as_blocks(dual_scale, mode, max_rounds, xb);
  if (t.refused || !as_start(t)) return 1;
  as_rounds(t);
  return as_accept(t);
}

AsAttempt QpSolve::as_blocks(double dual_scale, int mode, int max_rounds, int xb) {
  AsAttempt t;
  memset(&t, 0, sizeof(t));
  t.dual_scale = dual_scale; t.mode = mode; t.max_rounds = max_rounds;
  LQArgs &b = t.b;
  ConeArgs &ca = t.ca;
  XboxArgs &xa = t.xa;
  const double big = 1e30, tol_p = 1e-13;
  w.as_act.ensure(nu * sizeof(int) + 8); w.as_cntp.ensure((size_t)M * 3 * sizeof(int)); w.as_settled.ensure((size_t)M * sizeof(int));
  w.as_ctl.ensure(sizeof(AsCtl)); w.as_delta.ensure((size_t)std::max(nc, 1) * D8);
  int *act = t.act = (int *)w.as_act.p;
  AsCtl *ctl = t.ctl = (AsCtl *)w.as_ctl.p;
  b = a;
  b.Dx = b.wx = b.Du = b.wu = nullptr; b.du_full = 0;
  b.as_act = act; b.as_lo = su.lo; b.as_hi = su.hi; b.as_cnt = (int *)w.as_cntp.p; b.as_big = big; b.as_tol_p = tol_p;
  b.as_settled_out = (int *)w.as_settled.p; b.as_delta = w.as_delta.d(); b.as_ctl = ctl; b.done = &ctl->done;
  w.as_viol.ensure((size_t)M * D8);
  b.as_viol = w.as_viol.d();
  b.Xb = p->X_out; b.Ub = p->U_out; b.Xo = p->X_out; b.Uo = p->U_out;
  {
    int slots = 0;
    if (c->opt[OPT_AS_CKPT] != 0.0 && as_skip_on && nc <= 32)
      while ((PMPC_AS_CK_FIRST << slots) <= N - 1) slots++;
    if (slots > 0) {
      const int ks = (x + 3) / 4;
      w.as_ck.ensure((size_t)M * slots * (64 * ks + 32) * D8);
      w.as_jhi.ensure((size_t)M * sizeof(int));
      if (w.ck_stat.ensure(4 * sizeof(unsigned long long))) HIP_CHECK(hipMemsetAsync(w.ck_stat.p, 0, 4 * sizeof(unsigned long long), s));
      b.as_ck = w.as_ck.d(); b.as_jhi = (int *)w.as_jhi.p; b.ck_slots = slots; b.ck_stat = (unsigned long long *)w.ck_stat.p;
    }
  }
  w.as_key = -1;
  const bool cone = t.cone = cone_as && (mode == 0 || mode == 3 || mode == 5);
  b.as_freeze_tol = (cone && Nc == 1) ? c->opt[OPT_AS_FREEZE_TOL] : 0.0;
  if (cone) {
    const int q = (int)p->soc_q;
    const size_t rows = (size_t)M * N;
    w.Hadd.ensure(nu * u * D8); w.wu_soc.ensure(nu * D8); w.cone_uraw.ensure(nu * D8); w.as_open.ensure((size_t)M * sizeof(int));
    const bool z_new = w.cone_z.ensure(rows * cone_rows * D8), rec_new = w.cone_rec.ensure(rows * std::max(ncones, 1) * PMPC_CONE_REC * D8);
    if (z_new || rec_new) w.as_key = -1;
    b.cone_H = w.Hadd.d(); b.cone_g = w.wu_soc.d(); b.as_uraw = w.cone_uraw.d(); b.as_open = (int *)w.as_open.p;
    ca.M = M; ca.N = N; ca.u = u; ca.q = q; ca.Nc = Nc; ca.owner = a.owner;
    ca.rows = cone_rows;
    if (ncones > 0) {
      ca.ncones = ncones; ca.per_stage = p->cone_per_stage ? 1 : 0;
      for (int k = 0; k < ncones; k++) ca.qs[k] = p->cone_sizes[k];
      ca.A = p->cone_A; ca.c = p->cone_c;
    } else {
      ca.ncones = 1; ca.qs[0] = q; ca.per_stage = 0;
      ca.A = w.cone_A.d(); ca.c = w.cone_c.d();
    }
    ca.R = p->R; ca.r32 = a.mat32; ca.reg_u = p->reg_u; ca.rho_scale = 1e7;
    ca.z = w.cone_z.d(); ca.rec = w.cone_rec.d(); ca.H = w.Hadd.d(); ca.g = w.wu_soc.d();
    ca.cnt = (int *)w.as_cntp.p; ca.settled = (int *)w.as_settled.p; ca.open = (int *)w.as_open.p; ca.done = &ctl->done; ca.ctl = ctl;
    ca.jhi = b.as_jhi;
    ca.tol_step = 1e-6; ca.tol_phi = 1e-9;
    ca.dual_scale = dual_scale;
  }
  const bool xbox = t.xbox = xbox_as && xb != 0;
  {
    const int min_m = (int)c->opt[OPT_AS_SENS_MIN_M];
    if (min_m > 0 && M >= min_m && as_skip_on && Nc == 1 && (mode != 0 || w.as_pred_rounds >= 2)) {
      w.as_T.ensure((size_t)M * N * 64 * D8);
      b.as_T = w.as_T.d();
    }
  }
  if (xbox) {
    w.as_open.ensure((size_t)M * sizeof(int)); w.xb_D.ensure(nx * D8); w.xb_g.ensure(nx * D8);
    const bool z_new = w.xb_z.ensure(nx * D8), st_new = w.xb_st.ensure(nx * sizeof(int));
    if ((z_new || st_new) && mode == 0) { t.refused = true; return t; }
    if (mode == 2 || xb == 2) {
      HIP_CHECK(hipMemsetAsync(w.xb_z.p, 0, nx * D8, s));
      HIP_CHECK(hipMemsetAsync(w.xb_st.p, 0, nx * sizeof(int), s));
    } else if (mode == 1) {
      launch_xbox_from_ipm(sx, (int *)w.xb_st.p, w.xb_z.d(), s);
    }
    b.xb_D = w.xb_D.d(); b.xb_g = w.xb_g.d(); b.as_open = (int *)w.as_open.p;
    xa.M = M; xa.N = N; xa.x = x; xa.lo = p->lx; xa.hi = p->ux; xa.Q = p->Q; xa.pw = p->weights; xa.reg_x = p->reg_x; xa.rho_scale = 1e7;
    w.xb_qmax.ensure((size_t)M * D8);
    xa.qmax = w.xb_qmax.d();
    xa.z = w.xb_z.d(); xa.st = (int *)w.xb_st.p; xa.D = w.xb_D.d(); xa.g = w.xb_g.d();
    xa.cnt = (int *)w.as_cntp.p; xa.settled = (int *)w.as_settled.p; xa.open = (int *)w.as_open.p; xa.done = &ctl->done; xa.ctl = ctl;
    xa.jhi = b.as_jhi;
    xa.tol = 1e-9; xa.dual_scale = dual_scale;
    xa.z_tol = 1e-3;
    xa.keep_on_clamp = 1;
    xa.act_frac = 0.5;
    xa.ctrl_from = c->xb_ctrl_from >= 0 ? c->xb_ctrl_from : x;
  }
  return t;
}

bool QpSolve::as_start(AsAttempt &t) {
  LQArgs &b = t.b;
  ConeArgs &ca = t.ca;
  XboxArgs &xa = t.xa;
  const int mode = t.mode, max_rounds = t.max_rounds;
  const double dual_scale = t.dual_scale, big = b.as_big;
  const bool cone = t.cone, xbox = t.xbox;
  int *act = t.act;
  AsCtl *ctl = t.ctl;
  launch_as_begin(ctl, (int *)w.fail.p, max_rounds, dual_scale, s, cone ? 8 : (xbox ? (c->xb_ctrl_from >= 0 ? 8 : (mode == 0 ? 6 : 3)) : 2));
// ... 646 lines not shown
```

pmpc_amd/device.py:

```python
from __future__ import annotations

import ctypes
from typing import Dict, Optional

import numpy as np
import torch

from . import _lib

MODEL_UNICYCLE, MODEL_QUADROTOR, MODEL_BICYCLE = 0, 1, 2


def _p(t: Optional[torch.Tensor], dtype=torch.float64):
    if t is None:
        return None
    assert t.is_cuda and t.dtype == dtype and t.is_contiguous(), (t.device, t.dtype, t.is_contiguous())
    return ctypes.c_void_p(t.data_ptr())


class _TorchF64:

    def __init__(self, device):
        self.device = device

    def asarray(self, a):
        return torch.as_tensor(a, dtype=torch.float64, device=self.device)


class DeviceSolver:

    def __init__(self, device: Optional[int] = None):
        if not torch.cuda.is_available():
            raise RuntimeError("pmpc_amd.DeviceSolver needs a HIP device: there is no CPU path")
        self.lib = _lib.load()
        self.device = torch.cuda.current_device() if device is None else int(device)
        h = ctypes.c_void_p()
        rc = self.lib.pmpc_create(ctypes.byref(h), self.device)
        if rc != 0:
            raise RuntimeError(f"pmpc_create failed ({rc})")
        self.h = h
        self.stream = torch.cuda.ExternalStream(self.lib.pmpc_stream(h), device=self.device)
        self.rank, self.world = 0, 1
        self.last_info: Dict[str, float] = {}

    def set_option(self, key: str, value: float) -> None:
        if self.lib.pmpc_set_option(self.h, key.encode(), float(value)) != 0:
            raise KeyError(f"pmpc_set_option: unknown option {key!r}")

    def get_option(self, key: str) -> float:
        v = ctypes.c_double()
        if self.lib.pmpc_get_option(self.h, key.encode(), ctypes.byref(v)) != 0:
            raise KeyError(f"pmpc_get_option: unknown option {key!r}")
        return v.value

    def close(self):
        if getattr(self, "h", None):
            self.lib.pmpc_destroy(self.h)
            self.h = None

    def __del__(self):
        try:
            self.close()
        except Exception:
            pass

    def init_comm(self):
        import torch.distributed as dist

        if not dist.is_initialized() or dist.get_world_size() == 1:
            return
        rank, world = dist.get_rank(), dist.get_world_size()
        uid = [None]
        if rank == 0:
            buf = ctypes.create_string_buffer(128)
            rc = self.lib.pmpc_comm_unique_id(ctypes.cast(buf, ctypes.c_void_p))
            if rc != 0:
                raise RuntimeError(f"pmpc_comm_unique_id failed ({rc})")
            uid[0] = bytes(buf.raw)
        dist.broadcast_object_list(uid, src=0)
        buf = ctypes.create_string_buffer(uid[0], 128)
        rc = self.lib.pmpc_comm_init(self.h, rank, world, ctypes.cast(buf, ctypes.c_void_p))
        if rc != 0:
            raise RuntimeError(f"pmpc_comm_init failed ({rc})")
        self.rank, self.world = rank, world

    def _before(self, on=True):
        if on:
            self.stream.wait_stream(torch.cuda.current_stream(self.device))

    def _after(self, on=True):
        if on:
            torch.cuda.current_stream(self.device).wait_stream(self.stream)

    def _problem(self, *, f, fx, fu, X_prev, U_prev, Q, R, X_ref, U_ref, reg_x, reg_u, Nc=-1, x0=None, lx=None, ux=None,
                 lu=None, uu=None, slew_reg=None, slew_reg0=None, slew_um1=None, X_out=None, U_out=None, weights=None,
                 barrier_mu=0.0, force_generic=False, symmetric_cost=False, cold_start=False, static_cons_bounds=False, prev_is_last_solution=False, soc_W=None, soc_w0=None,
                 soc_v=None, soc_v0=0.0, soc_u_interior=None, cone_k=0, cones=None, cone_objective=False, smooth_cstr="logbarrier", smooth_beta=1.0):
        M, N, x = f.shape
        u = U_prev.shape[-1]
        assert fx.shape == (M, N, x, x) and fu.shape == (M, N, u, x) and Q.shape == (M, N, x, x) and R.shape == (M, N, u, u)
        assert weights is None or weights.shape == (M,)
        if X_out is None:
            X_out = torch.empty((M, N, x), dtype=torch.float64, device=f.device)
        if U_out is None:
            U_out = torch.empty((M, N, u), dtype=torch.float64, device=f.device)
        flags = 0
        if lx is not None and ux is not None:
            flags |= _lib.HAS_XBOUNDS
        if lu is not None and uu is not None:
            flags |= _lib.HAS_UBOUNDS
        if slew_reg is not None:
            flags |= _lib.HAS_SLEW
        if slew_reg0 is not None and slew_um1 is not None:
            flags |= _lib.HAS_SLEW0
        if force_generic:
            flags |= _lib.FORCE_GENERIC
        if cold_start:
            flags |= _lib.COLD_START
        if static_cons_bounds:
            flags |= _lib.STATIC_CONS_BOUNDS
        if prev_is_last_solution:
            flags |= _lib.PREV_IS_LAST_SOLUTION
        if symmetric_cost:
            flags |= _lib.SYMMETRIC_COST
        if cone_objective:
            flags |= _lib.CONE_OBJECTIVE
        md = torch.float32 if fx.dtype == torch.float32 else torch.float64
        assert fx.dtype == fu.dtype == Q.dtype == R.dtype == md, "fx, fu, Q, R must share one dtype (float64, or float32 for the fp32-storage mode)"
        if md == torch.float32:
            flags |= _lib.F32_MATRICES
        prob = _lib.PmpcProblem(
            xdim=x, udim=u, N=N, M=M, Nc=int(Nc), flags=flags, reg_x=float(reg_x), reg_u=float(reg_u),
            x0=_p(x0), f=_p(f), fx=_p(fx, md), fu=_p(fu, md), X_prev=_p(X_prev), U_prev=_p(U_prev), Q=_p(Q, md), R=_p(R, md),
            X_ref=_p(X_ref), U_ref=_p(U_ref), lx=_p(lx), ux=_p(ux), lu=_p(lu), uu=_p(uu), slew_reg=_p(slew_reg),
            slew_reg0=_p(slew_reg0), slew_um1=_p(slew_um1), X_out=_p(X_out), U_out=_p(U_out), weights=_p(weights), barrier_mu=float(barrier_mu),
            soc_q=0 if soc_W is None else int(soc_W.shape[0]), soc_W=_p(soc_W), soc_w0=_p(soc_w0), soc_v=_p(soc_v), soc_v0=float(soc_v0),
            soc_u_interior=_p(soc_u_interior), cone_k=int(cone_k), smooth_cstr={"logbarrier": 0, "squareplus": 1}[smooth_cstr], smooth_beta=float(smooth_beta))
        if cones is not None:
            sizes = [int(v) for v in cones["sizes"]]
            rows = sum(sizes) + len(sizes)
            A, cvec = cones["A"], cones["c"]
            per_stage = A.dim() == 4
            assert A.shape == ((M, N, rows, u) if per_stage else (rows, u)) and cvec.shape == ((M, N, rows) if per_stage else (rows,)), (A.shape, cvec.shape)
            self._cone_sizes = (ctypes.c_int * len(sizes))(*sizes)
            prob.cone_count, prob.cone_sizes = len(sizes), ctypes.cast(self._cone_sizes, ctypes.POINTER(ctypes.c_int))
            prob.cone_A, prob.cone_c, prob.cone_per_stage = _p(A), _p(cvec), int(per_stage)
        return prob, X_out, U_out

    def _solve(self, entry, kw, verbose, wait_current_stream, *args):
        prob, X_out, U_out = self._problem(**kw)
        info = _lib.PmpcInfo()
        self._before(wait_current_stream)
        status = entry(self.h, ctypes.byref(prob), *args, ctypes.byref(info), int(verbose))
        self.last_info = {k: getattr(info, k) for k, _ in _lib.PmpcInfo._fields_}
        self._after(wait_current_stream)
        return X_out, U_out, status

    def lqp_solve(self, *, verbose=False, wait_current_stream=True, **kw):
        return self._solve(self.lib.pmpc_lqp_solve_device, kw, verbose, wait_current_stream)

    def lcone_solve(self, *, smooth_alpha=float("nan"), verbose=False, wait_current_stream=True, **kw):
        return self._solve(self.lib.pmpc_lcone_solve_device, kw, verbose, wait_current_stream, float(smooth_alpha))

    def lsoc_solve(self, *, verbose=False, wait_current_stream=True, **kw):
        return self._solve(self.lib.pmpc_lsoc_solve_device, kw, verbose, wait_current_stream)

    def particle_costs(self, X, U, **kw):
        prob, _, _ = self._problem(X_out=X, U_out=U, **kw)
        J = torch.empty((X.shape[0],), dtype=torch.float64, device=X.device)
        self.stream.wait_stream(torch.cuda.current_stream(self.device))
        self.lib.pmpc_particle_costs_device(self.h, ctypes.byref(prob), _p(X), _p(U), _p(J))
        self.sync()
        return J

    def linearize(self, model: int, x0, X_prev, U_prev, params, f=None, fx=None, fu=None, wait_current_stream=True):
        M, N, x = X_prev.shape
        u = U_prev.shape[-1]
        dev = X_prev.device
        f = torch.empty((M, N, x), dtype=torch.float64, device=dev) if f is None else f
        fx = torch.empty((M, N, x, x), dtype=torch.float64, device=dev) if fx is None else fx
        fu = torch.empty((M, N, u, x), dtype=torch.float64, device=dev) if fu is None else fu
        self._before(wait_current_stream)
        if fx.dtype == torch.float32:
            st = self.lib.pmpc_linearize_device_f32(self.h, int(model), N, M, _p(x0), _p(X_prev), _p(U_prev), _p(params), _p(f), _p(fx, torch.float32),
                                               _p(fu, torch.float32))
        else:
            st = self.lib.pmpc_linearize_device(self.h, int(model), N, M, _p(x0), _p(X_prev), _p(U_prev), _p(params), _p(f), _p(fx),
                                           _p(fu))
        self._after(wait_current_stream)
        if st != 0:
            raise RuntimeError(f"pmpc_linearize_device failed ({st}): model {model} is not a built-in model, or a HIP error")
        return f, fx, fu

    def rollout(self, model: int, x0, U, params, out=None, wait_current_stream=True):
        self._need("pmpc_rollout_device")
        M, N, _ = U.shape
        x = x0.shape[-1]
        assert x0.shape == (M, x), (x0.shape, U.shape)
        out = torch.empty((M, N, x), dtype=torch.float64, device=U.device) if out is None else out
        assert out.shape == (M, N, x)
        self._before(wait_current_stream)
        st = self.lib.pmpc_rollout_device(self.h, int(model), N, M, _p(x0), _p(U), _p(params), _p(out))
        self._after(wait_current_stream)
        if st != 0:
            raise RuntimeError(f"pmpc_rollout_device failed ({st}): model {model} is not a built-in model, an empty horizon, or a HIP error")
        return out

# ... 182 lines not shown
        self._before(wait_current_stream)
        st = self.lib.pmpc_keepout_augment_device(self.h, ctypes.byref(sc), x, u, N, M, _p(X_prev), _p(f), _p(fx), _p(fu), _p(X_ref), _p(out["f"]),
                                                  _p(out["fx"]), _p(out["fu"]), _p(out["X_prev"]), _p(out["X_ref"]), _p(out["xu"]))
        self._after(wait_current_stream)
        if st != 0:
            raise RuntimeError(f"pmpc_keepout_augment_device failed ({st})")
        if not wait_current_stream:
            self.sync()
        del keep
        return out

    def scp_residual(self, X, X_prev, U, U_prev, out=None, wait_current_stream=True):
        M, N, x = X.shape
        out = torch.empty((1,), dtype=torch.float64, device=X.device) if out is None else out
        self._before(wait_current_stream)
        self.lib.pmpc_scp_residual_device(self.h, x, U.shape[-1], N, M, _p(X), _p(X_prev), _p(U), _p(U_prev), _p(out))
        self._after(wait_current_stream)
        return out

    def strip_residual(self, X_aug, X, X_prev, U, U_prev, out=None, wait_current_stream=True):
        self._need("pmpc_keepout_strip_residual_device")
        M, N, x = X.shape
        K = X_aug.shape[-1] - x
        assert X_aug.shape == (M, N, x + K) and X_prev.shape == X.shape and U.shape == U_prev.shape and U.shape[:2] == (M, N)
        out = torch.empty((1,), dtype=torch.float64, device=X.device) if out is None else out
        self._before(wait_current_stream)
        st = self.lib.pmpc_keepout_strip_residual_device(self.h, x, K, U.shape[-1], N, M, _p(X_aug), _p(X), _p(X_prev), _p(U), _p(U_prev), _p(out))
        self._after(wait_current_stream)
        if st != 0:
            raise RuntimeError(f"pmpc_keepout_strip_residual_device failed ({st}): K outside 1 .. 4, x + K > 16, an empty array, or a HIP error")
        return out

    def scp_loop(self, model: int, params, steps: int, *, f2, fx2, fu2, first_cold=True, res=None, wait_current_stream=True, cost=None, cstr=None,
                 aug=None, **kw):
        if kw.pop("builtin_cstr", None) is not None:
            raise ValueError("scp_loop: builtin_cstr is not supported (the keep-out constraint enters the library loop as cstr=, a dict or the handle "
                             "of prepare_cstr, with aug=keepout_buffers(...); solve(..., device=..., builtin_cstr=...) carries it in the Python-driven loop)")
        prob, X_out, U_out = self._problem(**kw)
        res = torch.empty((steps,), dtype=torch.float64, device=f2.device) if res is None else res
        infos = (_lib.PmpcInfo * steps)()
        last = ctypes.c_int(0)
        M, N, x = kw["f"].shape
        if cost is not None:
            sc, keep = self._scp_cost(cost, N, x, f2.device)
        if cstr is not None:
            self._need("pmpc_scp_loop_device_cstr")
            if aug is None:
                raise ValueError("scp_loop(cstr=...) needs aug=keepout_buffers(problem, K): the augmented buffers, allocated once")
            own_cstr = not isinstance(cstr, tuple)
            cs, keep_cstr = self.prepare_cstr(cstr, M, N, x, f2.device)
            sets = aug["sets"]
            if aug["K"] != cs.K or len(sets) != 2 or aug["X_out"].shape != (M, N, x + cs.K):
                raise ValueError(f"scp_loop(cstr=...): aug is not keepout_buffers(problem, K={cs.K}, sets=2) of this problem")
            two = lambda k: (ctypes.c_void_p * 2)(_p(sets[0][k]), _p(sets[1][k]))
            ab = _lib.PmpcScpAug(Q=_p(aug["Qa"]), x0=_p(aug["x0"]), lx=_p(aug["lx"]), f=two("f"), fx=two("fx"), fu=two("fu"), X_prev=two("X_prev"),
                                 X_ref=two("X_ref"), xu=two("xu"), X_out=_p(aug["X_out"]))
        self._before(wait_current_stream)
        jd = kw["fx"].dtype
        head = (self.h, int(model), _p(params), ctypes.byref(prob), _p(f2), _p(fx2, jd), _p(fu2, jd), int(steps), int(bool(first_cold)), _p(res), infos,
                ctypes.byref(last))
        if cstr is not None:
            done = self.lib.pmpc_scp_loop_device_cstr(*head, ctypes.byref(sc) if cost is not None else None, ctypes.byref(cs), ctypes.byref(ab))
            if cost is not None or own_cstr:
                self.sync()
            del keep_cstr
        elif cost is None:
            done = self.lib.pmpc_scp_loop_device(*head)
        else:
            done = self.lib.pmpc_scp_loop_device_cost(*head, ctypes.byref(sc))
            self.sync()
        if cost is not None:
            del keep
        self._after(wait_current_stream)
        if cost is not None:
            self.check_bad_pivots("scp_loop(cost=...): Q")
        out = [{k: getattr(infos[i], k) for k, _ in _lib.PmpcInfo._fields_} for i in range(min(done + 1, steps))]
        if out:
            self.last_info = out[min(done, steps) - 1] if done > 0 else out[0]
        return res, out, bool(last.value), done

    def sync(self):
        self.lib.pmpc_sync(self.h)

    def profile(self, level):
        self.lib.pmpc_profile_enable(self.h, int(level))

    def profile_read(self):
        ms = (ctypes.c_double * 4)()
        n = (ctypes.c_longlong * 4)()
        self.lib.pmpc_profile_read(self.h, ms, n)
        names = ("bwd_factor", "bwd_vec", "fwd", "consensus")
        out = {k: (ms[i], n[i]) for i, k in enumerate(names)}
        pms, pn = ctypes.c_double(), ctypes.c_longlong()
        self.lib.pmpc_profile_read_partial(self.h, ctypes.byref(pms), ctypes.byref(pn))
        out["bwd_factor_partial"] = (pms.value, pn.value)
        ms8, n8 = (ctypes.c_double * 8)(), (ctypes.c_longlong * 8)()
        self.lib.pmpc_profile_read_all(self.h, ms8, n8, 8)
        for k, name in ((5, "as_bookkeeping"), (6, "linearize"), (7, "scp_residual")):
            out[name] = (ms8[k], n8[k])
        return out

    def restart_stats(self, reset: bool = True):
        out = (ctypes.c_ulonglong * 4)()
        self.lib.pmpc_restart_stats(self.h, out, 1 if reset else 0)
        return dict(restarted=int(out[0]), restarted_stages=int(out[1]), full=int(out[2]), full_stages=int(out[3]))


def to_device_problem(prob: dict, device="cuda"):
    t = lambda a: torch.as_tensor(np.ascontiguousarray(a), dtype=torch.float64, device=device)
    tm = lambda a: torch.as_tensor(np.ascontiguousarray(np.swapaxes(a, -1, -2)), dtype=torch.float64, device=device)
    out = dict(x0=t(prob["x0"]), Q=tm(prob["Q"]), R=tm(prob["R"]), X_ref=t(prob["X_ref"]), U_ref=t(prob["U_ref"]),
               X_prev=t(prob["X_prev"]), U_prev=t(prob["U_prev"]), params=t(prob["params"]))
    for k_src, k_dst in (("u_l", "lu"), ("u_u", "uu"), ("x_l", "lx"), ("x_u", "ux")):
        if prob.get(k_src) is not None:
            out[k_dst] = t(prob[k_src])
    return out
```

pmpc_amd/device_problem.py:

```python
from __future__ import annotations

import math
from dataclasses import dataclass
from typing import Any, Dict, Optional

import numpy as np
import torch

from .dynamics import model_id

_CONE_SOLVERS = ("ecos", "gurobi", "mosek", "cosmo")


@dataclass
class DeviceProblem:
    M: int
    N: int
    xdim: int
    udim: int
    single: bool
    Q: torch.Tensor
    R: torch.Tensor
    Qa: torch.Tensor
    Ra: torch.Tensor
    sym: bool
    x0: Optional[torch.Tensor]
    X_ref: torch.Tensor
    U_ref: torch.Tensor
    X_prev: torch.Tensor
    U_prev: torch.Tensor
    lx: Optional[torch.Tensor]
    ux: Optional[torch.Tensor]
    lu: Optional[torch.Tensor]
    uu: Optional[torch.Tensor]
    reg_x: float
    reg_u: float
    Nc: int
    cone: bool
    smooth_alpha: float
    solver_verbose: bool
    slew: Optional[torch.Tensor]
    slew_reg0: Optional[torch.Tensor]
    slew0: Optional[torch.Tensor]
    um1: Optional[torch.Tensor]
    soc_kw: Dict[str, Any]
    model: Optional[int]
    params: Optional[torch.Tensor]

    def solve_kw(self) -> Dict[str, Any]:
        return dict(Q=self.Qa, R=self.Ra, reg_x=self.reg_x, reg_u=self.reg_u, Nc=self.Nc, x0=self.x0, lx=self.lx, ux=self.ux, lu=self.lu,
                    uu=self.uu, slew_reg=self.slew, symmetric_cost=self.sym)


def _stage_cone(soc, settings, T, M, N, xdim, udim, Nc) -> Dict[str, Any]:
    if soc is None and settings.get("extra_cstrs"):
        from .extra_cstrs import stage_soc_from_extra_cstrs

        tuples = list(settings["extra_cstrs"])
        if len(tuples) != 1:
            raise ValueError("one extra_cstrs tuple (the stage-wise second-order cone) is supported")
        soc = stage_soc_from_extra_cstrs(tuples[0], M, N, xdim, udim, Nc)
        if "soc_u_interior" not in settings:
            raise ValueError("solver_settings['soc_u_interior'] (a control strictly inside the boxes and the cone) is required")
        soc["u_interior"] = settings["soc_u_interior"]
    if soc is None:
        return {}
    return dict(soc_W=T(soc["W"]).reshape(-1, udim).contiguous(), soc_w0=T(soc["w0"]).reshape(-1).contiguous(),
                soc_v=T(soc["v"]).reshape(udim).contiguous(), soc_v0=float(soc.get("v0", 0.0)),
                soc_u_interior=T(soc["u_interior"]).reshape(udim).contiguous())


def build_problem(Q, R, x0=None, X_ref=None, U_ref=None, X_prev=None, U_prev=None, x_l=None, x_u=None, u_l=None, u_u=None,
                  reg_x: float = 1e0, reg_u: float = 1e-2, slew_rate: Optional[float] = None, u0_slew=None,
                  solver_settings: Optional[Dict[str, Any]] = None, soc: Optional[Dict[str, Any]] = None, builtin_model=None, params=None,
                  device="cuda", own_copies: bool = False, need_sym: Optional[str] = None) -> DeviceProblem:
    dev = torch.device(device)
    T = lambda z: None if z is None else torch.as_tensor(np.asarray(z) if not torch.is_tensor(z) else z, dtype=torch.float64, device=dev)
    Q, R, x0 = T(Q), T(R), T(x0)
    single = x0 is not None and x0.ndim == 1
    if single:
        assert Q.ndim == 3 and R.ndim == 3
        Q, R, x0 = Q[None], R[None], x0[None]
    M, N, xdim, udim = Q.shape[0], Q.shape[1], Q.shape[-1], R.shape[-1]
    own = (lambda t: t.clone()) if own_copies else (lambda t: t)
    vec = lambda z, d: own(T(z).reshape(M, N, d).contiguous())
    X_ref = torch.zeros((M, N, xdim), dtype=torch.float64, device=dev) if X_ref is None else vec(X_ref, xdim)
    U_ref = torch.zeros((M, N, udim), dtype=torch.float64, device=dev) if U_ref is None else vec(U_ref, udim)
    X_prev = X_ref.clone() if X_prev is None else T(X_prev).reshape(M, N, xdim).contiguous().clone()
    U_prev = U_ref.clone() if U_prev is None else T(U_prev).reshape(M, N, udim).contiguous().clone()
    has = lambda z: z is not None and (z.numel() if torch.is_tensor(z) else np.size(z)) > 0
    lx, ux = (vec(x_l, xdim), vec(x_u, xdim)) if has(x_l) and has(x_u) else (None, None)
    lu, uu = (vec(u_l, udim), vec(u_u, udim)) if has(u_l) and has(u_u) else (None, None)
    Qa, Ra = Q.transpose(-1, -2).contiguous(), R.transpose(-1, -2).contiguous()
    sym = bool(torch.equal(Qa, Q) and torch.equal(Ra, R))
    if need_sym is not None and not sym:
        raise ValueError(f"{need_sym} symmetric Q and R blocks (the reference shift is a Cholesky solve with them)")
    settings = dict(solver_settings or {})
    cone = str(settings.get("solver", "ecos")).lower() in _CONE_SOLVERS or "smooth_cstr" in settings or "smooth_alpha" in settings
    Nc = int(settings.get("Nc", -1))
    full = lambda v: torch.full((M,), float(v), dtype=torch.float64, device=dev)
    slew = full(slew_rate) if slew_rate is not None and float(slew_rate) != 0.0 else None
    slew_reg0 = full(settings["slew_reg"]) if "slew_reg" in settings else None
    um1 = T(u0_slew).reshape(-1, udim).expand(M, udim).contiguous() if slew_reg0 is not None and u0_slew is not None else None
    model = model_id(builtin_model) if builtin_model is not None else None
    if model is not None:
        assert params is not None, "builtin_model needs `params` (M, 3) unicycle / (M, 4) quadrotor / (M, 2) bicycle"
        params = own(T(params).reshape(M, -1).contiguous())
    return DeviceProblem(M=M, N=N, xdim=xdim, udim=udim, single=single, Q=Q, R=R, Qa=Qa, Ra=Ra, sym=sym,
                         x0=None if x0 is None else x0.contiguous(), X_ref=X_ref, U_ref=U_ref, X_prev=X_prev, U_prev=U_prev, lx=lx, ux=ux,
                         lu=lu, uu=uu, reg_x=float(reg_x), reg_u=float(reg_u), Nc=Nc, cone=cone,
                         smooth_alpha=float(settings.get("smooth_alpha", math.nan)), solver_verbose=bool(settings.get("verbose", False)),
                         slew=slew, slew_reg0=slew_reg0, slew0=slew_reg0 if um1 is not None else None, um1=um1,
                         soc_kw=_stage_cone(soc, settings, T, M, N, xdim, udim, Nc), model=model, params=params if model is not None else None)


def keepout_static(p: DeviceProblem, K: int) -> Dict[str, torch.Tensor]:
    M, N, xdim, xd = p.M, p.N, p.xdim, p.xdim + K
    mk = lambda *shape, fill: torch.full(shape, fill, dtype=torch.float64, device=p.Qa.device)
    lx, xu = mk(M, N, xd, fill=-math.inf), mk(M, N, xd, fill=math.inf)
    if p.lx is not None:
        lx[..., :xdim] = torch.where(torch.isnan(p.lx), torch.full_like(p.lx, -math.inf), p.lx)
        xu[..., :xdim] = torch.where(torch.isnan(p.ux), torch.full_like(p.ux, math.inf), p.ux)
    Qa = mk(M, N, xd, xd, fill=0.0)
    Qa[..., :xdim, :xdim] = p.Qa
    Qa[..., torch.arange(xdim, xd), torch.arange(xdim, xd)] = -p.reg_x
    x0 = mk(M, xd, fill=0.0)
    x0[:, :xdim] = p.x0
    return dict(Qa=Qa, x0=x0, lx=lx, xu=xu)


def keepout_buffers(p: DeviceProblem, K: int, sets: int = 2) -> Dict[str, Any]:
    M, N, u, xd = p.M, p.N, p.udim, p.xdim + K
    static = keepout_static(p, K)
    mk = lambda *shape: torch.empty(shape, dtype=torch.float64, device=p.Qa.device)
    one = lambda k: dict(f=mk(M, N, xd), fx=mk(M, N, xd, xd), fu=mk(M, N, u, xd), X_prev=mk(M, N, xd), X_ref=mk(M, N, xd),
                         xu=static["xu"] if k == 0 else static["xu"].clone())
    return dict(Qa=static["Qa"], x0=static["x0"], lx=static["lx"], sets=[one(k) for k in range(int(sets))], X_out=mk(M, N, xd), K=int(K))
```

Before: 2988 SCP iterations/s.

## Broadcast stage-invariant Q, R, refs and bounds with zero stride in active-set sweeps

Adds detection of per-particle arrays (Q, R, X_ref, U_ref, lu, uu) that are identical across horizon stages, either promised by the caller, computed in Python, or found by a device kernel at loop start. The active-set backward and forward sweeps then read these arrays with a zero per-stage stride, so every stage reuses the first stage's block instead of streaming N copies. The goal is less global memory traffic in the bandwidth-bound sweeps. In exchange it adds a detection kernel and a host poll, plus extra pointer-identity bookkeeping that has to hold for results to stay correct.

```diff
diff --git a/include/pmpc_abi.h b/include/pmpc_abi.h
--- a/include/pmpc_abi.h
+++ b/include/pmpc_abi.h
@@ -45,6 +45,14 @@
 
 #define PMPC_COLD_START 64u
 #define PMPC_STATIC_CONS_BOUNDS 128u
+#define PMPC_STAGE_INV_SHIFT 11
+#define PMPC_STAGE_INV_Q 2048u
+#define PMPC_STAGE_INV_R 4096u
+#define PMPC_STAGE_INV_XREF 8192u
+#define PMPC_STAGE_INV_UREF 16384u
+#define PMPC_STAGE_INV_LU 32768u
+#define PMPC_STAGE_INV_UU 65536u
+#define PMPC_STAGE_INV_ALL 129024u
 #define PMPC_PREV_IS_LAST_SOLUTION 256u
 
 #define PMPC_CONE_OBJECTIVE 1024u
@@ -193,6 +201,8 @@
                               double *fu2, int steps, int first_cold, double *res, pmpc_info *infos, int *last_in_out,
                               const pmpc_scp_cost *cost, const pmpc_scp_cstr *cstr, const pmpc_scp_aug *aug);
 void pmpc_scp_loop_follow_ups(unsigned long long *out2, int reset);
+unsigned pmpc_stage_inv_last(pmpc_ctx *ctx);
+
 
 void pmpc_profile_enable(pmpc_ctx *ctx, int level);
 void pmpc_profile_read(pmpc_ctx *ctx, double *ms4, long long *n4);
diff --git a/pmpc_amd/_lib.py b/pmpc_amd/_lib.py
--- a/pmpc_amd/_lib.py
+++ b/pmpc_amd/_lib.py
@@ -13,6 +13,10 @@
 c_dp = ctypes.POINTER(ctypes.c_double)
 
 HAS_XBOUNDS, HAS_UBOUNDS, HAS_SLEW, HAS_SLEW0, FORCE_GENERIC, SYMMETRIC_COST, COLD_START, STATIC_CONS_BOUNDS, PREV_IS_LAST_SOLUTION, F32_MATRICES, CONE_OBJECTIVE = 1, 2, 4, 8, 16, 32, 64, 128, 256, 512, 1024
+
+STAGE_INV_SHIFT = 11
+STAGE_INV = {"Q": 1 << 11, "R": 1 << 12, "X_ref": 1 << 13, "U_ref": 1 << 14, "lu": 1 << 15, "uu": 1 << 16}
+STAGE_INV_ALL = sum(STAGE_INV.values())
 
 ABI_SYMBOLS = [
     "c_lqp_solve", "c_lcone_solve", "pmpc_lqp_solve_host", "pmpc_lcone_solve_host", "pmpc_create", "pmpc_destroy", "pmpc_stream", "pmpc_sync", "pmpc_lqp_solve_device",
@@ -28,6 +32,7 @@
     "pmpc_keepout_augment_device", "pmpc_abi_scp_cstr_size",
     "pmpc_keepout_strip_residual_device", "pmpc_scp_loop_device_cstr", "pmpc_abi_scp_aug_size", "pmpc_scp_loop_follow_ups",
     "pmpc_shift_active_set_device", "pmpc_warm_shift_device", "pmpc_warm_set_read_device",
+    "pmpc_stage_inv_last",
 ]
 
 
@@ -201,6 +206,9 @@
         lib.pmpc_warm_shift_device.restype = ctypes.c_int
         lib.pmpc_warm_set_read_device.argtypes = [vp, vp, sz]
         lib.pmpc_warm_set_read_device.restype = ctypes.c_int
+    if hasattr(lib, "pmpc_stage_inv_last"):
+        lib.pmpc_stage_inv_last.argtypes = [vp]
+        lib.pmpc_stage_inv_last.restype = ctypes.c_uint
     lib.pmpc_version.argtypes = []
     lib.pmpc_version.restype = ctypes.c_char_p
     if not hasattr(lib, "pmpc_abi_struct_sizes"):
@@ -262,6 +270,21 @@
     return int(out[0]), int(out[1])
 
 
+def stage_inv_flags(promise) -> int:
+    if promise is None or promise == "detect":
+        return 0
+    if isinstance(promise, (int, np.integer)):
+        if not 0 <= int(promise) < 64:
+            raise ValueError(f"stage_inv: a mask of six bits, got {promise}")
+        return int(promise) << STAGE_INV_SHIFT
+    bits = 0
+    for name in promise:
+        if name not in STAGE_INV:
+            raise ValueError(f"stage_inv: unknown array {name!r} (one of {sorted(STAGE_INV)})")
+        bits |= STAGE_INV[name]
+    return bits
+
+
 def as_sweep_knobs():
     out = (ctypes.c_int * 3)()
     load().pmpc_as_sweep_knobs(out)
diff --git a/pmpc_amd/csrc/kernels_as.hip b/pmpc_amd/csrc/kernels_as.hip
--- a/pmpc_amd/csrc/kernels_as.hip
+++ b/pmpc_amd/csrc/kernels_as.hip
@@ -111,8 +111,9 @@
   const void *K_ = ubase_v(a.K, (long long)(pbase * 64) * MB);
   auto xoff = [&](int jj) { return (long long)(jj * (int)(XD * D8)); };
   auto uoff = [&](int jj) { return (long long)(jj * (int)(UD * D8)); };
+  auto xroff = [&](int jj) { return (long long)(jj * a.sj_Xr); };
   auto ld_Q = [&](int jj, double *dst) {
-    const void *q = ubase_v(Q_, (long long)(jj * (int)(XD * XD * MB)));
+    const void *q = ubase_v(Q_, (long long)(jj * a.sj_Q));
 #pragma unroll
     for (int r = 0; r < KS; r++) {
       const bool rv = !PADX || (L.row0 + r < XD);
@@ -121,7 +122,7 @@
     }
   };
   auto ld_xm = [&](int jj, double *dst) {
-    const double *xb = ubase(Xb_, xoff(jj)), *xr = ubase(Xr_, xoff(jj));
+    const double *xb = ubase(Xb_, xoff(jj)), *xr = ubase(Xr_, xroff(jj));
 #pragma unroll
     for (int r = 0; r < KS; r++) {
       const bool rv = !PADX || (L.row0 + r < XD);
@@ -137,7 +138,7 @@
   const char *pC = (const char *)Z;
   int sC = 0;
   if (gu && c == XP) { pC = (const char *)(Ub + (pbase + jtop) * UD + g); sC = -UD * (int)D8; }
-  else if (gu && c == XP + 1) { pC = (const char *)(a.U_ref + (pbase + jtop) * UD + g); sC = -UD * (int)D8; }
+  else if (gu && c == XP + 1) { pC = (const char *)(a.U_ref + pbase * UD + g) + (long long)jtop * a.sj_Ur; sC = -a.sj_Ur; }
   else if (gu && c == XP + 2) { pC = (const char *)(a.as_act + (pbase + jtop) * UD + g); sC = -UD * (int)sizeof(int); }
   else if (CONE && gu && c == XP + 3) { pC = (const char *)(a.cone_g + (pbase + jtop) * UD + g); sC = -UD * (int)D8; }
   else if (!DEFECT && g < 2 && 15 - XP - c >= 0 && 15 - XP - c < UD) {
@@ -146,7 +147,7 @@
   }
   const double regu_s = (L.cu && g < 2) ? (g == 0 ? regu : -regu) : 0.0;
   auto ld_R = [&](int jj) -> double {
-    const double v = ldom<MT>(ubase_v(R_, (long long)(jj * (int)(UD * UD * MB))), lR);
+    const double v = ldom<MT>(ubase_v(R_, (long long)(jj * a.sj_R)), lR);
     return fR ? v : 0.0;
   };
   const double *CH_ = CONE ? ubase(a.cone_H, (long long)(pbase * (UD * UD)) * D8) : Z;
@@ -178,7 +179,7 @@
   auto fetch_late = [&](int jj, int jbelow, Pipe &q) {
     ld_Q(jbelow, q.Q);
     q.xb = ldo(ubase(Xb_, xoff(jbelow)), lxc);
-    q.xr = ldo(ubase(Xr_, xoff(jbelow)), lxc);
+    q.xr = ldo(ubase(Xr_, xroff(jbelow)), lxc);
     if (!DEFECT) q.xp = ldo(ubase(Xp_, xoff(jbelow)), lxc);
     if constexpr (XBOX) {
       q.xd = ldo(ubase(XD_, xoff(jbelow)), lxc);
@@ -464,11 +465,12 @@
   auto xoff = [&](int jj) { return (long long)(jj * (int)(XD * D8)); };
   auto uoff = [&](int jj) { return (long long)(jj * (int)(UD * D8)); };
   const char *pG = (const char *)Z;
-  int sG = 0;
+  int sG = 0, sGc = 0;
   if (gu && c < 4) {
     const double *arr = c == 0 ? Ub : (c == 1 ? a.kff : (c == 2 ? a.as_lo : a.as_hi));
     pG = (const char *)(arr + pbase * UD + g);
-    sG = UD * (int)D8;
+    sG = c == 2 ? a.sj_lo : (c == 3 ? a.sj_hi : UD * (int)D8);
+    sGc = UD * (int)D8 - sG;
   } else if (gu && c == 7) {
     pG = (const char *)(a.as_act + pbase * UD + g);
     sG = UD * (int)sizeof(int);
@@ -478,8 +480,8 @@
   const bool store_u = (c == 0) && gu;
   struct Pipe { double T[KS + 1], grp, xb, f; };
   int jF = 0;
-  auto fetch = [&](int jj, Pipe &q) {
-    if (jj > jF) { pA += sAj; pB += sBj; pG += sG; jF = jj; }
+  auto fetch = [&](int jj, Pipe &q, auto free_tag) {
+    if (jj > jF) { pA += sAj; pB += sBj; pG += (decltype(free_tag)::value || jj > Nc) ? sG : sG + sGc; jF = jj; }
 #pragma unroll
     for (int r = 0; r < KS; r++) {
       const double t = gldm<MT>(pA + (vA[r] ? r * sAr : 0));
@@ -702,8 +704,8 @@
         const size_t e = (pbase + jc) * UD + uo;
         ub[q] = is_u ? gld(Ub + e) : 0.0;
         kf[q] = is_u ? gld(a.kff + e) : 0.0;
-        lo[q] = is_u ? gld(a.as_lo + e) : 0.0;
-        hi[q] = is_u ? gld(a.as_hi + e) : 0.0;
+        lo[q] = is_u ? gld((const double *)((const char *)(a.as_lo + (pbase + 1) * UD + uo) + (long long)(jc - 1) * a.sj_lo)) : 0.0;
+        hi[q] = is_u ? gld((const double *)((const char *)(a.as_hi + (pbase + 1) * UD + uo) + (long long)(jc - 1) * a.sj_hi)) : 0.0;
         act[q] = is_u ? a.as_act[e] : 0;
       }
 #pragma unroll
@@ -773,7 +775,7 @@
   int j = 0;
   if constexpr (SENS && !DEFECT) if (elem) {
     Pipe P;
-    fetch(0, P);
+    fetch(0, P, std::false_type{});
     stage(std::false_type{}, 0, P);
     settled_update(1);
     finish();
@@ -781,34 +783,34 @@
   }
   if (PF2) {
     Pipe P0, P1, P2;
-    fetch(0, P0);
-    fetch(clampN(1), P1);
+    fetch(0, P0, std::false_type{});
+    fetch(clampN(1), P1, std::false_type{});
     for (; j < jmin && j < N; j++) {
-      fetch(clampN(j + 2), P2);
+      fetch(clampN(j + 2), P2, std::false_type{});
       stage(std::false_type{}, j, P0);
       P0 = P1;
       P1 = P2;
     }
     for (; j + 2 < N; j += 3) {
-      fetch(clampN(j + 2), P2);
+      fetch(clampN(j + 2), P2, std::true_type{});
       stage(std::true_type{}, j, P0);
-      fetch(clampN(j + 3), P0);
+      fetch(clampN(j + 3), P0, std::true_type{});
       stage(std::true_type{}, j + 1, P1);
-      fetch(clampN(j + 4), P1);
+      fetch(clampN(j + 4), P1, std::true_type{});
       stage(std::true_type{}, j + 2, P2);
     }
     if (j < N) { stage(std::true_type{}, j, P0); j++; }
     if (j < N) { stage(std::true_type{}, j, P1); j++; }
   } else {
     Pipe A, B;
-    fetch(0, A);
+    fetch(0, A, std::false_type{});
     for (; j < jmin && j < N; j++) {
-      fetch(clampN(j + 1), B);
+      fetch(clampN(j + 1), B, std::false_type{});
       stage(std::false_type{}, j, A);
       A = B;
     }
     for (; j < N; j++) {
-      fetch(clampN(j + 1), B);
+      fetch(clampN(j + 1), B, std::true_type{});
       stage(std::true_type{}, j, A);
       A = B;
     }
@@ -859,6 +861,19 @@
   return k;
 }
 std::atomic<unsigned long long> as_bwd_launches[AS_BWD_CODES], as_fwd_launches[AS_FWD_CODES];
+
+LQArgs with_stage_strides(const LQArgs &a0) {
+  LQArgs a = a0;
+  const int MB = a.mat32 ? (int)sizeof(float) : (int)sizeof(double), D8 = (int)sizeof(double);
+  auto st = [&](unsigned bit, int dense) { return (a.stage_inv & bit) ? 0 : dense; };
+  a.sj_Q = st(PMPC_STAGE_INV_Q >> PMPC_STAGE_INV_SHIFT, a.x * a.x * MB);
+  a.sj_R = st(PMPC_STAGE_INV_R >> PMPC_STAGE_INV_SHIFT, a.u * a.u * MB);
+  a.sj_Xr = st(PMPC_STAGE_INV_XREF >> PMPC_STAGE_INV_SHIFT, a.x * D8);
+  a.sj_Ur = st(PMPC_STAGE_INV_UREF >> PMPC_STAGE_INV_SHIFT, a.u * D8);
+  a.sj_lo = st(PMPC_STAGE_INV_LU >> PMPC_STAGE_INV_SHIFT, a.u * D8);
+  a.sj_hi = st(PMPC_STAGE_INV_UU >> PMPC_STAGE_INV_SHIFT, a.u * D8);
+  return a;
+}
 
 template <int XD, int UD>
 void launch_bwd_as_t(const LQArgs &a, hipStream_t s) {
@@ -931,13 +946,15 @@
   const AsSweepKnobs &k = as_sweep_knobs();
   out[0] = k.deep2_maxm; out[1] = k.deep_maxm; out[2] = k.fwd_pf2_maxm;
 }
-void launch_bwd_as(const LQArgs &a, hipStream_t s) {
+void launch_bwd_as(const LQArgs &a0, hipStream_t s) {
+  const LQArgs a = with_stage_strides(a0);
 #define X(xd, ud) if (a.x == xd && a.u == ud) { launch_bwd_as_t<xd, ud>(a, s); return; }
   PMPC_FAST_DIMS(X)
 #undef X
   no_such_variant("factor sweep of an active-set round", a.x, a.u);
 }
-void launch_fwd_as(const LQArgs &a, hipStream_t s) {
+void launch_fwd_as(const LQArgs &a0, hipStream_t s) {
+  const LQArgs a = with_stage_strides(a0);
 #define X(xd, ud) if (a.x == xd && a.u == ud) { launch_fwd_as_t<xd, ud>(a, s); return; }
   PMPC_FAST_DIMS(X)
 #undef X
diff --git a/pmpc_amd/csrc/pmpc_dev.h b/pmpc_amd/csrc/pmpc_dev.h
--- a/pmpc_amd/csrc/pmpc_dev.h
+++ b/pmpc_amd/csrc/pmpc_dev.h
@@ -97,6 +97,8 @@
   const double *xb_D, *xb_g;
   int mat32;
   int jac_compact;
+  unsigned stage_inv;
+  int sj_Q, sj_R, sj_Xr, sj_Ur, sj_lo, sj_hi;
   int owner;
   int any_slew;
   int sym_cost;
@@ -189,6 +191,13 @@
 void launch_as_ctl(AsCtl *ctl, const int *cnt_part, int M, const int *fail, int reduce, int decide, int last_of_batch, AsCtl *mirror,
                    unsigned long long *mirror_seq, unsigned long long seq, hipStream_t s, double *tail = nullptr, const double *viol = nullptr,
                    const int *open_part = nullptr);
+
+struct StageInvArgs {
+  const void *arr[6];
+  int block_bytes[6];
+  int N, M;
+};
+void launch_stage_inv_detect(const StageInvArgs &g, unsigned *flag, unsigned long long *mirror, unsigned long long seq, hipStream_t s);
 
 struct ConeArgs {
   int M, N, u, q, Nc, owner;
diff --git a/pmpc_amd/csrc/solver.hip b/pmpc_amd/csrc/solver.hip
--- a/pmpc_amd/csrc/solver.hip
+++ b/pmpc_amd/csrc/solver.hip
@@ -235,6 +235,11 @@
   if (fast && a.as_act) launch_fwd_as(a, s);
   else if (fast) launch_fwd_fast(a, s);
   else launch_fwd_generic(a, s);
+}
+
+bool stage_inv_enabled() {
+  static const bool on = !(getenv("PMPC_STAGE_INV") && atoi(getenv("PMPC_STAGE_INV")) == 0);
+  return on;
 }
 
 int fail_after_error(pmpc_ctx *c, const pmpc_problem *p, pmpc_info *info) {
@@ -733,7 +738,7 @@
 
   q = *p;
   q.xdim = (size_t)n;
-  q.flags &= ~(PMPC_HAS_SLEW | PMPC_HAS_SLEW0 | PMPC_HAS_UBOUNDS | PMPC_HAS_XBOUNDS | PMPC_PREV_IS_LAST_SOLUTION | PMPC_STATIC_CONS_BOUNDS);
+  q.flags &= ~(PMPC_HAS_SLEW | PMPC_HAS_SLEW0 | PMPC_HAS_UBOUNDS | PMPC_HAS_XBOUNDS | PMPC_PREV_IS_LAST_SOLUTION | PMPC_STATIC_CONS_BOUNDS | PMPC_STAGE_INV_ALL);
   if (boxes) q.flags |= PMPC_HAS_XBOUNDS;
   q.reg_x = reg;
   q.reg_u = 0.0;
@@ -779,6 +784,50 @@
 }
 size_t pmpc_abi_scp_aug_size(void) { return sizeof(pmpc_scp_aug); }
 
+static void stage_inv_begin(pmpc_ctx *c, const pmpc_problem *p0, bool eligible, bool with_cost, int steps) {
+  c->sinv_mask = c->sinv_last = c->sinv_cand = 0;
+  c->sinv_pending = 0;
+  if (!eligible || !stage_inv_enabled() || steps <= 0) return;
+  const bool f32 = (p0->flags & PMPC_F32_MATRICES) != 0, has_ub = (p0->flags & PMPC_HAS_UBOUNDS) != 0;
+  const int x = (int)p0->xdim, u = (int)p0->udim, N = (int)p0->N, M = (int)p0->M, MB = f32 ? 4 : 8;
+  StageInvArgs g;
+  memset(&g, 0, sizeof(g));
+  const void *arr[6] = {p0->Q, p0->R, with_cost ? nullptr : p0->X_ref, p0->U_ref, has_ub ? p0->lu : nullptr, has_ub ? p0->uu : nullptr};
+  const int bb[6] = {x * x * MB, u * u * MB, x * 8, u * 8, u * 8, u * 8};
+  unsigned cand = 0;
+  for (int k = 0; k < 6; k++) {
+    g.arr[k] = arr[k]; g.block_bytes[k] = bb[k]; c->sinv_ptr[k] = arr[k];
+    if (arr[k]) cand |= 1u << k;
+  }
+  g.N = N; g.M = M;
+  c->sinv_cand = cand;
+  const unsigned promise = (p0->flags & PMPC_STAGE_INV_ALL) >> PMPC_STAGE_INV_SHIFT;
+  if (promise) {
+    c->sinv_last = promise & cand;
+    return;
+  }
+  if (!cand) return;
+  c->sinv_flag.ensure(sizeof(unsigned));
+  c->sinv_pending = ++c->sinv_seq;
+  launch_stage_inv_detect(g, (unsigned *)c->sinv_flag.p, &c->mirror_dev->stage_inv, c->sinv_pending, c->stream);
+}
+static void stage_inv_poll(pmpc_ctx *c) {
+  if (!c->sinv_pending) return;
+  const unsigned long long v = *(volatile unsigned long long *)&c->mirror->stage_inv;
+  if ((v >> 8) != c->sinv_pending) return;
+  c->sinv_pending = 0;
+  c->sinv_mask = c->sinv_last = (unsigned)(v & 63u) & c->sinv_cand;
+}
+unsigned pmpc_stage_inv_last(pmpc_ctx *c) {
+  if (!c) return 0;
+  if (c->sinv_pending) {
+    HIP_WARN(hipStreamSynchronize(c->stream));
+    stage_inv_poll(c);
+    c->sinv_mask = 0;
+  }
+  return c->sinv_last;
+}
+
 int pmpc_scp_loop_device(pmpc_ctx *c, int model, const double *params, const pmpc_problem *p0, double *f2, double *fx2, double *fu2,
                          int steps, int first_cold, double *res, pmpc_info *infos, int *last_in_out) {
   return pmpc_scp_loop_device_cstr(c, model, params, p0, f2, fx2, fu2, steps, first_cold, res, infos, last_in_out, nullptr, nullptr, nullptr);
@@ -798,6 +847,8 @@
                               const pmpc_scp_cstr *cstr, const pmpc_scp_aug *aug) {
   pmpc_problem p = *p0;
   const int x = (int)p0->xdim, u = (int)p0->udim, N = (int)p0->N, M = (int)p0->M;
+  c->sinv_mask = c->sinv_last = 0;
+  c->sinv_pending = 0;
   const bool with_cost = cost != nullptr && cost->kind != 0;
   double *Xr[2] = {nullptr, nullptr};
   unsigned *cost_bad = nullptr;
@@ -841,6 +892,7 @@
       Xr[0] = c->ws.cost_ref[0].d(); Xr[1] = c->ws.cost_ref[1].d();
       cost_bad = cost_bad_counter(c);
     }
+    stage_inv_begin(c, p0, !with_cstr && !c->multi() && !cone_obj && !(p0->flags & (PMPC_HAS_SLEW | PMPC_HAS_SLEW0 | PMPC_FORCE_GENERIC)), with_cost, steps);
     for (; done < steps; done++) {
       double *Xp = (done & 1) ? XB : XA, *Up = (done & 1) ? UB : UA, *Xo = (done & 1) ? XA : XB, *Uo = (done & 1) ? UA : UB;
       if (!lin_ready) {
@@ -859,6 +911,8 @@
       c->jac_compact_model = model;
       p.X_prev = Xp; p.U_prev = Up; p.X_out = Xo; p.U_out = Uo;
       p.flags = p0->flags | PMPC_STATIC_CONS_BOUNDS;
+      if (with_cost) p.flags &= ~(unsigned)PMPC_STAGE_INV_XREF;
+      if (with_cstr) p.flags &= ~(unsigned)PMPC_STAGE_INV_ALL;
       if (done > 0 || !first_cold) p.flags |= PMPC_PREV_IS_LAST_SOLUTION;
       else p.flags &= ~(unsigned)PMPC_PREV_IS_LAST_SOLUTION;
       if (with_cstr) {
@@ -921,6 +975,7 @@
                               : solve_impl(c, &p, &inf, 0, soc);
       c->post_batch = nullptr;
       c->jac_compact_fx = nullptr;
+      stage_inv_poll(c);
       if (infos) infos[done] = inf;
       if (st != 0) {
         if (with_cstr) launch_fill(Xo, std::numeric_limits<double>::quiet_NaN(), (long long)M * N * x, c->stream);
@@ -937,9 +992,11 @@
       cur ^= 1;
     }
     HIP_CHECK(hipGetLastError());
+    c->sinv_mask = 0;
   } catch (const PmpcHipError &) {
     c->post_batch = nullptr;
     c->jac_compact_fx = nullptr;
+    c->sinv_mask = 0;
     if (infos && done < steps) { memset(&infos[done], 0, sizeof(pmpc_info)); infos[done].status = 2; }
     fail_after_error(c, nullptr, nullptr);
     try {
diff --git a/pmpc_amd/csrc/solver_internal.h b/pmpc_amd/csrc/solver_internal.h
--- a/pmpc_amd/csrc/solver_internal.h
+++ b/pmpc_amd/csrc/solver_internal.h
@@ -129,7 +129,7 @@
   Workspace ws;
   IpmScal *sc_host = nullptr;
   int *fail_host = nullptr;
-  struct ScMirror { IpmScal sc; unsigned long long seq; int as_cnt[4]; unsigned long long as_seq; AsCtl ctl; double epi[4]; unsigned long long epi_seq; };
+  struct ScMirror { IpmScal sc; unsigned long long seq; int as_cnt[4]; unsigned long long as_seq; AsCtl ctl; double epi[4]; unsigned long long epi_seq; unsigned long long stage_inv; };
   ScMirror *mirror = nullptr, *mirror_dev = nullptr;
   unsigned long long seq = 0, as_seq = 0, epi_seq = 0;
   ncclComm_t comm = nullptr;
@@ -149,6 +149,10 @@
   bool spec_fired = false, spec_ok = false;
   const double *jac_compact_fx = nullptr;
   int jac_compact_model = 0;
+  unsigned sinv_mask = 0, sinv_last = 0, sinv_cand = 0;
+  const void *sinv_ptr[6] = {nullptr, nullptr, nullptr, nullptr, nullptr, nullptr};
+  unsigned long long sinv_seq = 0, sinv_pending = 0;
+  DevBuf sinv_flag;
 };
 
 namespace pmpc_impl {
@@ -195,6 +199,7 @@
 void read_scalars(pmpc_ctx *c);
 void exchange(pmpc_ctx *c, int phase);
 void structured_solve(pmpc_ctx *c, LQArgs &a, bool factor, bool fast, bool prep_done = false);
+bool stage_inv_enabled();
 int fail_after_error(pmpc_ctx *c, const pmpc_problem *p, pmpc_info *info);
 void fill_nan_outputs(pmpc_ctx *c, const pmpc_problem *p);
 
diff --git a/pmpc_amd/csrc/solver_qp.hip b/pmpc_amd/csrc/solver_qp.hip
--- a/pmpc_amd/csrc/solver_qp.hip
+++ b/pmpc_amd/csrc/solver_qp.hip
@@ -567,6 +567,18 @@
   w.as_viol.ensure((size_t)M * D8);
   b.as_viol = w.as_viol.d();
   b.Xb = p->X_out; b.Ub = p->U_out; b.Xo = p->X_out; b.Uo = p->U_out;
+  {
+    unsigned inv = 0;
+    if (stage_inv_enabled() && !c->multi()) {
+      inv = (p->flags & PMPC_STAGE_INV_ALL) >> PMPC_STAGE_INV_SHIFT;
+      const void *arr[6] = {p->Q, p->R, p->X_ref, p->U_ref, p->lu, p->uu};
+      for (int k = 0; k < 6; k++)
+        if ((c->sinv_mask >> k & 1u) && arr[k] && arr[k] == c->sinv_ptr[k]) inv |= 1u << k;
+      const bool boxes_as_given = has_ub && !soc && (su.lo == p->lu || (su.lo == w.su.lo.d() && w.su_src_lo == p->lu && w.su_src_hi == p->uu && w.su_key != -1));
+      if (!boxes_as_given) inv &= ~48u;
+    }
+    b.stage_inv = inv;
+  }
   {
     int slots = 0;
     if (c->opt[OPT_AS_CKPT] != 0.0 && as_skip_on && nc <= 32)
diff --git a/pmpc_amd/csrc/stage_inv.hip b/pmpc_amd/csrc/stage_inv.hip
--- /dev/null
+++ b/pmpc_amd/csrc/stage_inv.hip
@@ -0,0 +1,46 @@
+#include "pmpc_dev.h"
+
+namespace {
+
+template <class W>
+__device__ unsigned slab_differs(const void *arr, const void *ref_block, int block_bytes, int N, size_t particle) {
+  const int bw = block_bytes / (int)sizeof(W);
+  const W *slab = (const W *)arr + particle * (size_t)N * bw, *ref = (const W *)ref_block;
+  unsigned bad = 0;
+  const int total = N * bw;
+  for (int t = bw + (int)threadIdx.x; t < total; t += (int)blockDim.x) bad |= (slab[t] != ref[t % bw]) ? 1u : 0u;
+  return bad;
+}
+
+__global__ void __launch_bounds__(256) k_stage_inv(StageInvArgs g, unsigned *flag) {
+  const size_t i = blockIdx.x;
+  unsigned bad = 0;
+#pragma unroll
+  for (int k = 0; k < 6; k++) {
+    if (!g.arr[k]) continue;
+    const int bb = g.block_bytes[k];
+    const char *ref = (const char *)g.arr[k] + i * (size_t)g.N * bb;
+    unsigned d;
+    if (bb % 8 == 0 && (unsigned long long)g.arr[k] % 8 == 0) d = slab_differs<unsigned long long>(g.arr[k], ref, bb, g.N, i);
+    else d = slab_differs<unsigned>(g.arr[k], ref, bb, g.N, i);
+    bad |= d << k;
+  }
+#pragma unroll
+  for (int o = 32; o > 0; o >>= 1) bad |= __shfl_xor(bad, o, 64);
+  if ((threadIdx.x & 63) == 0 && bad) atomicAnd(flag, ~bad);
+}
+
+__global__ void k_stage_inv_publish(const unsigned *flag, unsigned long long *mirror, unsigned long long seq) {
+  if (threadIdx.x == 0) *(volatile unsigned long long *)mirror = (seq << 8) | (unsigned long long)(*flag & 63u);
+}
+
+}
+
+void launch_stage_inv_detect(const StageInvArgs &g, unsigned *flag, unsigned long long *mirror, unsigned long long seq, hipStream_t s) {
+  unsigned cand = 0;
+  for (int k = 0; k < 6; k++)
+    if (g.arr[k]) cand |= 1u << k;
+  HIP_CHECK(hipMemsetD32Async((hipDeviceptr_t)flag, (int)cand, 1, s));
+  if (cand && g.M > 0 && g.N > 1) hipLaunchKernelGGL(k_stage_inv, dim3(g.M), dim3(256), 0, s, g, flag);
+  hipLaunchKernelGGL(k_stage_inv_publish, dim3(1), dim3(64), 0, s, flag, mirror, seq);
+}
diff --git a/pmpc_amd/device.py b/pmpc_amd/device.py
--- a/pmpc_amd/device.py
+++ b/pmpc_amd/device.py
@@ -95,7 +95,7 @@
     def _problem(self, *, f, fx, fu, X_prev, U_prev, Q, R, X_ref, U_ref, reg_x, reg_u, Nc=-1, x0=None, lx=None, ux=None,
                  lu=None, uu=None, slew_reg=None, slew_reg0=None, slew_um1=None, X_out=None, U_out=None, weights=None,
                  barrier_mu=0.0, force_generic=False, symmetric_cost=False, cold_start=False, static_cons_bounds=False, prev_is_last_solution=False, soc_W=None, soc_w0=None,
-                 soc_v=None, soc_v0=0.0, soc_u_interior=None, cone_k=0, cones=None, cone_objective=False, smooth_cstr="logbarrier", smooth_beta=1.0):
+                 soc_v=None, soc_v0=0.0, soc_u_interior=None, cone_k=0, cones=None, cone_objective=False, smooth_cstr="logbarrier", smooth_beta=1.0, stage_inv=None):
         M, N, x = f.shape
         u = U_prev.shape[-1]
         assert fx.shape == (M, N, x, x) and fu.shape == (M, N, u, x) and Q.shape == (M, N, x, x) and R.shape == (M, N, u, u)
@@ -123,6 +123,7 @@
             flags |= _lib.PREV_IS_LAST_SOLUTION
         if symmetric_cost:
             flags |= _lib.SYMMETRIC_COST
+        flags |= _lib.stage_inv_flags(stage_inv)
         if cone_objective:
             flags |= _lib.CONE_OBJECTIVE
         md = torch.float32 if fx.dtype == torch.float32 else torch.float64
@@ -471,6 +472,10 @@
     def sync(self):
         self.lib.pmpc_sync(self.h)
 
+    def stage_inv_last(self) -> int:
+        self._need("pmpc_stage_inv_last")
+        return int(self.lib.pmpc_stage_inv_last(self.h))
+
     def profile(self, level):
         self.lib.pmpc_profile_enable(self.h, int(level))
 
diff --git a/pmpc_amd/device_problem.py b/pmpc_amd/device_problem.py
--- a/pmpc_amd/device_problem.py
+++ b/pmpc_amd/device_problem.py
@@ -46,10 +46,25 @@
     soc_kw: Dict[str, Any]
     model: Optional[int]
     params: Optional[torch.Tensor]
+    stage_inv: int = 0
 
     def solve_kw(self) -> Dict[str, Any]:
         return dict(Q=self.Qa, R=self.Ra, reg_x=self.reg_x, reg_u=self.reg_u, Nc=self.Nc, x0=self.x0, lx=self.lx, ux=self.ux, lu=self.lu,
-                    uu=self.uu, slew_reg=self.slew, symmetric_cost=self.sym)
+                    uu=self.uu, slew_reg=self.slew, symmetric_cost=self.sym, stage_inv=self.stage_inv)
+
+
+def stage_invariant_mask(Qa, Ra, lu, uu) -> int:
+    def bits(t):
+        t = t.contiguous()
+        return t.view(torch.int32 if t.dtype == torch.float32 else torch.int64).reshape(t.shape[0], t.shape[1], -1)
+
+    def same(t):
+        if t is None:
+            return False
+        b = bits(t)
+        return bool(torch.equal(b, b[:, :1].expand_as(b)))
+
+    return (1 if same(Qa) else 0) | (2 if same(Ra) else 0) | (16 if same(lu) else 0) | (32 if same(uu) else 0)
 
 
 def _stage_cone(soc, settings, T, M, N, xdim, udim, Nc) -> Dict[str, Any]:
@@ -111,7 +126,8 @@
                          lu=lu, uu=uu, reg_x=float(reg_x), reg_u=float(reg_u), Nc=Nc, cone=cone,
                          smooth_alpha=float(settings.get("smooth_alpha", math.nan)), solver_verbose=bool(settings.get("verbose", False)),
                          slew=slew, slew_reg0=slew_reg0, slew0=slew_reg0 if um1 is not None else None, um1=um1,
-                         soc_kw=_stage_cone(soc, settings, T, M, N, xdim, udim, Nc), model=model, params=params if model is not None else None)
+                         soc_kw=_stage_cone(soc, settings, T, M, N, xdim, udim, Nc), model=model, params=params if model is not None else None,
+                         stage_inv=stage_invariant_mask(Qa, Ra, lu, uu))
 
 
 def keepout_static(p: DeviceProblem, K: int) -> Dict[str, torch.Tensor]:
```

Measured after the change: 2984 SCP iterations/s. Within noise of the previous version (-0.1%).
